# iPERDance/iPERCore

Hardware: AMD Instinct MI355X
Metric: synthesized frames/sec at 512x512 (run_imitator) (higher is better)
Workload: dtype f32; 1 GPU; run_imitator 512x512 single src/ref pair, 300-frame reference clip frame-sharded over 1 GPU(s), AttLWB-SPADE generator fp32 (BASELINE configs[1] at N = 1, configs[2] at N = 8); poses=imitate, image_size=512, frame_batch=300, frame_batch_requested=384, world_size=1, parallelism=frame-shard x1, batches_in_flight=1, weights=random-init (seeded) of the real architecture, 36,276,992 params

## Files before the change

### include/lwg_hip.h

```cpp
#ifndef LWG_HIP_H
#define LWG_HIP_H

#include <stddef.h>
#include <stdint.h>

#ifdef __cplusplus
extern "C" {
#endif

typedef void* lwg_stream_t;

#define LWG_ABI_VERSION 10
int lwg_abi_version(void);

#define LWG_MAX_TAPS 52
enum { LWG_EPI_NONE = 0, LWG_EPI_RESIDUAL = 1, LWG_EPI_SPADE = 2 };
enum { LWG_ACTIVATION_NONE = 0, LWG_ACTIVATION_RELU = 1, LWG_ACTIVATION_TANH = 2, LWG_ACTIVATION_SIGMOID = 3 };
#define LWG_ACTIVATION_RELU_MASK 5
enum { LWG_DT_F32 = 0, LWG_DT_BF16 = 1,
       LWG_DT_F32_Q4 = 2 };

typedef struct LwgConvArgs {
    const float* x0;
    const float* x1;
    int C0, C1;
    int B, H, W;
    int OH, OW;
    int M;
    int stride;
    int ntaps;
    int cshift;
    const float* w;
    int N;
    const float* bias;
    float* y;
    int YH, YW, YC, ycoff;
    int omul, ooy, oox;
    int epi;
    int act;
    const float* res;
    const float* xn;
    const float* mean;
    const float* rstd;
    int xdt;
    int ydt;
    signed char dy[LWG_MAX_TAPS];
    signed char dx[LWG_MAX_TAPS];
} LwgConvArgs;

int lwg_conv2d_nhwc_f32(const LwgConvArgs* args, lwg_stream_t stream);
size_t lwg_conv2d_ws_floats(const LwgConvArgs* args);
int lwg_conv2d_nhwc_f32_ws(const LwgConvArgs* args, float* ws, lwg_stream_t stream);
int lwg_conv_slice_count(const LwgConvArgs* args);

int lwg_conv2d_nhwc_bf16(const LwgConvArgs* args, lwg_stream_t stream);
int lwg_conv2d_winograd_f32(const LwgConvArgs* args, lwg_stream_t stream);
size_t lwg_conv2d_winograd_ws_floats(const LwgConvArgs* args);
int lwg_conv2d_winograd_f32_ws(const LwgConvArgs* args, float* ws, lwg_stream_t stream);
int lwg_conv2d_winograd_plan(const LwgConvArgs* args, int with_ws, long long* blocks, int* slices, int* nbv, int* workgroups);
int lwg_winograd_panel_f32(const float* wpanel, float* upk, int Cin, int N, const int* tap9, lwg_stream_t stream);
typedef struct LwgWinoDesc {
    const float* wpanel;
    float* upk;
    int Cin, N, first_block;
    int tap9[9];
} LwgWinoDesc;
int lwg_winograd_panels_f32(const LwgWinoDesc* descs_dev, int ndesc, int total_blocks, lwg_stream_t stream);
int lwg_conv2d_winograd4_f32(const LwgConvArgs* args, lwg_stream_t stream);
typedef struct LwgConvLists {
    const int* heavy;
    const int* light;
    const int* counts;
    const float* cal;
} LwgConvLists;
int lwg_conv2d_winograd4_list_f32(const LwgConvArgs* args, const LwgConvLists* lists, lwg_stream_t stream);
int lwg_conv2d_winograd4_list_applies(const LwgConvArgs* args);
int lwg_spade_skip_lists_f32(const float* T, int B, int ns, int h, int w, int d, int* marks, int* heavy, int* light, int* counts, lwg_stream_t stream);
int lwg_conv2d_winograd4_fine_f32(const LwgConvArgs* args, const LwgConvLists* lists, lwg_stream_t stream);
int lwg_spade_skip_fine_lists_f32(const float* T, int B, int ns, int h, int w, int d, int* marks, int* heavy, int* light, int* counts, int* fmarks,
                                  int* fheavy, int* flight, int* fcounts, lwg_stream_t stream);
int lwg_winograd4_panel_f32(const float* wpanel, float* upk, int Cin, int N, const int* tap9, lwg_stream_t stream);
int lwg_winograd4_panels_f32(const LwgWinoDesc* descs_dev, int ndesc, int total_blocks, lwg_stream_t stream);
int lwg_conv2d_winograd4_f32_ws(const LwgConvArgs* args, float* ws, lwg_stream_t stream);
int lwg_conv2d_winograd4_plan(const LwgConvArgs* args, int with_ws, long long* blocks, int* slices, int* nbv, int* workgroups);
size_t lwg_conv2d_winograd4_ws_floats(const LwgConvArgs* args);
int lwg_conv2d_nhwc_bf16_hr(const LwgConvArgs* args, lwg_stream_t stream);
int lwg_conv2d_nhwc_bf16_hr_list(const LwgConvArgs* args, const LwgConvLists* lists, lwg_stream_t stream);
int lwg_conv2d_nhwc_bf16_hr_list_applies(const LwgConvArgs* args);
int lwg_conv2d_nhwc_bf16_hr_acc(const LwgConvArgs* args, lwg_stream_t stream);
int lwg_conv2d_winograd_bf16(const LwgConvArgs* args, lwg_stream_t stream);
int lwg_conv2d_nhwc_c8_bf16(const LwgConvArgs* args, lwg_stream_t stream);
int lwg_conv_transpose4_nhwc_bf16(const LwgConvArgs* args, lwg_stream_t stream);
int lwg_conv_transpose4_nhwc_f32(const LwgConvArgs* args, lwg_stream_t stream);
int lwg_conv_transpose4_is_one_grid(const LwgConvArgs* args);
int lwg_conv_transpose4_winograd_f32(const LwgConvArgs* args, lwg_stream_t stream);

int lwg_conv_transpose4_winograd24_f32(const LwgConvArgs* args, lwg_stream_t stream);

int lwg_conv2d_nhwc_f32_split(const LwgConvArgs* args, lwg_stream_t stream);

size_t lwg_conv2d_wgrad_ws_floats(int Ktot, int N, int M);
int lwg_conv2d_wgrad_nhwc_f32(const LwgConvArgs* args, const float* dy, float* dw, float* ws, lwg_stream_t stream);
int lwg_conv2d_wgrad_unpacked_f32(const LwgConvArgs* args, const float* dy, float* ws, float* dw, int D0, int D1, int KH, int KW,
                                  int transposed, const int* kidx, int cin, int nout, float* db, lwg_stream_t stream);
int lwg_colsum_nhwc_f32(const float* x, size_t rows, int C, float* out, float* ws, lwg_stream_t stream);
size_t lwg_conv2d_wgrad_winograd_ws_floats(const LwgConvArgs* args);
int lwg_conv2d_wgrad_winograd_f32(const LwgConvArgs* args, const float* dy, float* ws, float* dw, int cin, int nout, lwg_stream_t stream);

int lwg_act_bwd_f32(const float* dy, const float* y, size_t n, int act, float* out, lwg_stream_t stream);
int lwg_norm_fwd_nhwc_f32(const float* x, const float* mean, const float* rstd, const float* gamma, const float* beta, int gstride,
                          int B, int HW, int C, int act, float* y, lwg_stream_t stream);
int lwg_norm_bwd_nhwc_f32(const float* dy, const float* y, const float* x, const float* mean, const float* rstd,
                          const float* gamma, int gstride, int B, int HW, int C, int act, int nsplit, float* dx, float* dgamma,
                          float* dbeta, float* ws, lwg_stream_t stream);
int lwg_adam_step_f32(float* p, const float* g, float* m, float* v, size_t n, float lr, float beta1, float beta2, float eps, int t,
                      lwg_stream_t stream);
int lwg_adam_step_dev_f32(float* p, const float* g, float* m, float* v, size_t n, float lr, float beta1, float beta2, float eps,
                          int* t_dev, lwg_stream_t stream);
int lwg_pack_panel_f32(const float* w, int D0, int D1, int KH, int KW, int transposed, const int* kidx, int ntaps, int cin,
                       int cin_pad, int nout, int n_pad, float* out, lwg_stream_t stream);
int lwg_unpack_wgrad_f32(const float* dwk, int D0, int D1, int KH, int KW, int transposed, const int* kidx, int ntaps, int cin,
                         int cin_pad, int nout, int n_pad, float* dw, lwg_stream_t stream);
typedef struct LwgPackDesc {
    const float* w;
    float* out;
    int D1, KHW, transposed, ntaps, cin, cin_pad, nout, n_pad, Kp, first_block;
    int kidx[LWG_MAX_TAPS];
} LwgPackDesc;
int lwg_pack_panels_f32(const LwgPackDesc* descs_dev, int ndesc, int total_blocks, lwg_stream_t stream);
int lwg_maxpool2_fwd_nhwc_f32(const float* x, float* y, int B, int H, int W, int C, lwg_stream_t stream);
int lwg_maxpool2_bwd_nhwc_f32(const float* x, const float* dy, float* dx, int B, int H, int W, int C, lwg_stream_t stream);
int lwg_crop_resize_bilinear_f32(const float* x, const long long* box, float* y, float* valid, int N, int C, int H, int W, int OH, int OW,
                                 lwg_stream_t stream);
int lwg_crop_resize_bilinear_bwd_f32(const float* dy, const long long* box, float* dx, int N, int C, int H, int W, int OH, int OW, lwg_stream_t stream);
int lwg_prelu_f32(const float* x, const float* slope, const float* res, size_t rows, int C, float* y, lwg_stream_t stream);
int lwg_prelu_bwd_f32(const float* x, const float* slope, const float* dy, size_t rows, int C, float* dx, lwg_stream_t stream);

int lwg_instnorm_stats_nhwc_f32(const float* x, int B, int HW, int C, float eps, float* mean, float* rstd,
                                float* ws, int nsplit, lwg_stream_t stream);
int lwg_instnorm_stats_nhwc_bf16(const void* x, int B, int HW, int C, float eps, float* mean, float* rstd, float* ws, int nsplit,
                                 lwg_stream_t stream);
int lwg_instnorm_apply_nhwc_f32(const float* x, const float* mean, const float* rstd, const float* res,
                                float* y, int B, int HW, int C, int act, lwg_stream_t stream);

int lwg_flow_resize_f32(const float* T, int n, int S, int h, int w, float* out, lwg_stream_t stream);
int lwg_lwb_attention_f32(const float* q, const float* Ks, const float* Vs, const float* bk, const float* bv,
                          const float* T, float* out, int B, int ns, int h, int w, int C, int S,
                          int src_batched, lwg_stream_t stream);
int lwg_lwb_attention_bf16(const void* q, const void* Ks, const void* Vs, const float* bk, const float* bv, const float* T, void* out,
                           int B, int ns, int h, int w, int C, int S, int src_batched, lwg_stream_t stream);
int lwg_lwb_attention_x_records(int h, int w, int C, int element_size);
int lwg_lwb_attention_x_f32(const float* x, const float* Kq, const float* kappa, const float* Vs, const float* bv, const float* T,
                            float* out, float* stats, int B, int ns, int h, int w, int C, int src_batched, lwg_stream_t stream);
int lwg_lwb_attention_x_bf16(const void* x, const void* Kq, const float* kappa, const void* Vs, const float* bv, const float* T,
                             void* out, float* stats, int B, int ns, int h, int w, int C, int src_batched, lwg_stream_t stream);
size_t lwg_instnorm_finalize_ws_floats(int B, int C, int nrec);
int lwg_instnorm_finalize_f32(float* ws, int B, int C, int nrec, float eps, float* mean, float* rstd, lwg_stream_t stream);
int lwg_lwb_attention_bwd_f32(const float* q, const float* Ks, const float* Vs, const float* bk, const float* bv,
                              const float* T, const float* dout, float* dq, float* dKs, float* dVs, int B, int ns,
                              int h, int w, int C, int S, int src_batched, lwg_stream_t stream);
int lwg_lwb_attention_kv_f32(const float* q, const float* kv, const float* bk, const float* bv, const float* T, float* out,
                             int B, int ns, int h, int w, int C, int S, int src_batched, lwg_stream_t stream);
int lwg_lwb_attention_kv_bwd_f32(const float* q, const float* kv, const float* bk, const float* bv, const float* T,
                                 const float* dout, float* dq, float* dkv, int B, int ns, int h, int w, int C, int S,
                                 int src_batched, lwg_stream_t stream);
int lwg_lwb_fuse_f32(const float* tsf_x, const float* src_x, const float* gate, const float* T, float* out, int B, int ns,
                     int h, int w, int C, int S, int src_batched, float scale_w, float scale_o, lwg_stream_t stream);
int lwg_lwb_fuse_bf16(const void* tsf_x, const void* src_x, const void* gate, const float* T, void* out, int B, int ns, int h, int w,
                      int C, int S, int src_batched, float scale_w, float scale_o, lwg_stream_t stream);
int lwg_lwb_fuse_bwd_f32(const float* src_x, const float* gate, const float* T, const float* dout, float* d_tsf, float* d_src,
                         float* d_gate, int B, int ns, int h, int w, int C, int S, int src_batched, float scale_w, float scale_o,
                         lwg_stream_t stream);

size_t lwg_rasterize_ws_bytes(int B, int nf, int S);
int lwg_project_faces_f32(const float* verts, const float* cam, const int32_t* faces, int B, int nv, int nf,
                          float eye_dist, float* faces_v, float* f2pts, lwg_stream_t stream);
int lwg_rasterize_fim_wim_f32(const float* faces_v, int B, int nf, int S, float near, float far, int32_t* fim,
                              float* wim, void* ws, lwg_stream_t stream);
int lwg_texture_sample_f32(const int32_t* fim, const float* wim, const float* faces_v, const float* textures, int B, int nf,
                           int S, int T, int tex_batched, float eps, const float* bg_color3_host, float* rgb, lwg_stream_t stream);

int lwg_flow_compose_f32(const int32_t* fim, const float* wim, int B, int S, const float* map_fn, int nf,
                         const float* f_uvs2img, const float* uv_img4, int Hu, int Wu, const float* src_f2pts,
                         int ns, float* tsf_inputs, float* Tst, float* cond_nchw, float* Tuv, lwg_stream_t stream);
int lwg_bc_transform_f32(const float* f2pts, const int32_t* fim, const float* wim, int B, int S, int nf, float* T,
                         lwg_stream_t stream);
int lwg_encode_fim_f32(const int32_t* fim, const float* map_fn, int B, int S, int nf, int D, float* out,
                       lwg_stream_t stream);

size_t lwg_smpl_lbs_ws_floats(int B, int nv, int nj);
int lwg_smpl_lbs_f32(const float* pose, int pose_stride, const float* beta, int beta_stride, int nbeta,
                     const float* cam, int cam_stride, const float* v_template, const float* offsets, int off_batched,
                     const float* shapedirs, const float* posedirs, const float* J_regressor, const int32_t* parents,
                     const float* lbs_weights, const int32_t* links, int nlinks, int B, int nv, int nj, float* verts,
                     float* j3d, float* j2d, float* ws, lwg_stream_t stream);

int lwg_head_compose_f32(const float* x, const float* wpk, const float* bg, size_t bg_bstride, int B, int S, int C,
                         float* pred, float* mask, float* img, lwg_stream_t stream);
int lwg_head_compose_q4_f32(const float* x, const float* wpk, const float* bg, size_t bg_bstride, int B, int S, int C,
                            float* pred, float* mask, float* img, lwg_stream_t stream);
int lwg_thin_conv_f32(const float* x, const float* wpk, int B, int S, int C, int ks, float* y, lwg_stream_t stream);
int lwg_head_compose_bf16(const void* x, const void* wb, const float* bg, size_t bg_bstride, int B, int S, int C, float* pred,
                          float* mask, float* img, lwg_stream_t stream);
int lwg_up4_head_compose_bf16(const LwgConvArgs* args, const void* whead, const float* bg, size_t bg_bstride, float* pred, float* mask, float* img,
                              lwg_stream_t stream);
int lwg_frames_to_u8(const float* pred, int B, int S, int bgr, uint8_t* out, lwg_stream_t stream);
int lwg_nchw_to_nhwc_f32(const float* src, float* dst, int B, int C, int Cp, int P, lwg_stream_t stream);
int lwg_nhwc_to_nchw_f32(const float* src, float* dst, int B, int C, int Cs, int P, lwg_stream_t stream);

int lwg_morph_f32(const float* in, float* out, int n, int H, int W, int ks, int mode, float* ws, lwg_stream_t stream);
int lwg_canny_f32(const float* sil, int n, int H, int W, const float* gauss9, const float* sobelx9, float low, float high,
                  float* edges, float* ws, lwg_stream_t stream);
int lwg_boundary_fill_f32(const float* src, const float* confidant, const float* outpad, const float* edges, int n, int H,
                          int W, float* out, int32_t* top3, int32_t* ws, lwg_stream_t stream);
int lwg_grid_sample_nchw_f32(const float* img, size_t img_bstride, const float* grid, int n, int C, int H, int W, int Ho,
                             int Wo, float* out, lwg_stream_t stream);
int lwg_uv_merge_f32(const float* src_warp, const float* vis, int ns, int H, int W, float* out, lwg_stream_t stream);
int lwg_uv_merge_parts_f32(const float* uv_imgs, const float* vis, int n, int H, int W, float* out, lwg_stream_t stream);
int lwg_pack_inputs_f32(const float* a, int Ca, const float* b, int Cb, const float* mask, int n, int H, int W, int Cp,
                        float* out, lwg_stream_t stream);

int lwg_device_cu_count(void);

#ifdef __cplusplus
}
#endif
#endif
```

### ipercore_amd/_lib.py

```python
import ctypes
import os
import re

_HERE = os.path.dirname(os.path.abspath(__file__))
LIB_PATH = os.path.join(_HERE, "liblwg_hip.so")
HEADER_PATH = os.path.join(os.path.dirname(_HERE), "include", "lwg_hip.h")

LWG_MAX_TAPS = 52
EPI_NONE, EPI_RESIDUAL, EPI_SPADE = 0, 1, 2
ACT_NONE, ACT_RELU, ACT_TANH, ACT_SIGMOID, ACT_LRELU = 0, 1, 2, 3, 4
ACT_RELU_MASK = 5
DT_F32, DT_BF16, DT_F32_Q4 = 0, 1, 2

c_f = ctypes.c_void_p
c_i = ctypes.c_int


class LwgConvArgs(ctypes.Structure):
    _fields_ = [
        ("x0", c_f), ("x1", c_f),
        ("C0", c_i), ("C1", c_i),
        ("B", c_i), ("H", c_i), ("W", c_i),
        ("OH", c_i), ("OW", c_i),
        ("M", c_i), ("stride", c_i), ("ntaps", c_i), ("cshift", c_i),
        ("w", c_f), ("N", c_i), ("bias", c_f),
        ("y", c_f), ("YH", c_i), ("YW", c_i), ("YC", c_i), ("ycoff", c_i),
        ("omul", c_i), ("ooy", c_i), ("oox", c_i),
        ("epi", c_i), ("act", c_i),
        ("res", c_f), ("xn", c_f), ("mean", c_f), ("rstd", c_f),
        ("xdt", c_i), ("ydt", c_i),
        ("dy", ctypes.c_byte * LWG_MAX_TAPS), ("dx", ctypes.c_byte * LWG_MAX_TAPS),
    ]


class LwgWinoDesc(ctypes.Structure):
    _fields_ = [("wpanel", ctypes.c_void_p), ("upk", ctypes.c_void_p), ("Cin", c_i), ("N", c_i), ("first_block", c_i), ("tap9", c_i * 9)]


class LwgConvLists(ctypes.Structure):
    _fields_ = [("heavy", c_f), ("light", c_f), ("counts", c_f), ("cal", c_f)]


class LwgPackDesc(ctypes.Structure):
    _fields_ = [("w", c_f), ("out", c_f)] + [(n, c_i) for n in ("D1", "KHW", "transposed", "ntaps", "cin", "cin_pad", "nout", "n_pad", "Kp",
                                                               "first_block")] + [("kidx", c_i * LWG_MAX_TAPS)]


_SIGS = {
    "lwg_abi_version": (c_i, []),
    "lwg_device_cu_count": (c_i, []),
    "lwg_conv2d_nhwc_f32": (c_i, [ctypes.POINTER(LwgConvArgs), c_f]),
    "lwg_conv2d_ws_floats": (ctypes.c_size_t, [ctypes.POINTER(LwgConvArgs)]),
    "lwg_conv2d_nhwc_f32_ws": (c_i, [ctypes.POINTER(LwgConvArgs), c_f, c_f]),
    "lwg_conv2d_nhwc_bf16": (c_i, [ctypes.POINTER(LwgConvArgs), c_f]),
    "lwg_conv2d_winograd_f32": (c_i, [ctypes.POINTER(LwgConvArgs), c_f]),
    "lwg_conv2d_winograd_ws_floats": (ctypes.c_size_t, [ctypes.POINTER(LwgConvArgs)]),
    "lwg_conv2d_winograd_f32_ws": (c_i, [ctypes.POINTER(LwgConvArgs), c_f, c_f]),
    "lwg_conv2d_winograd_plan": (c_i, [ctypes.POINTER(LwgConvArgs), c_i, ctypes.POINTER(ctypes.c_longlong), ctypes.POINTER(c_i), ctypes.POINTER(c_i),
                                       ctypes.POINTER(c_i)]),
    "lwg_winograd_panel_f32": (c_i, [c_f, c_f, c_i, c_i, ctypes.POINTER(c_i), c_f]),
    "lwg_winograd_panels_f32": (c_i, [c_f, c_i, c_i, c_f]),
    "lwg_conv2d_winograd4_f32": (c_i, [ctypes.POINTER(LwgConvArgs), c_f]),
    "lwg_conv2d_winograd4_list_f32": (c_i, [ctypes.POINTER(LwgConvArgs), ctypes.POINTER(LwgConvLists), c_f]),
    "lwg_conv2d_winograd4_list_applies": (c_i, [ctypes.POINTER(LwgConvArgs)]),
    "lwg_spade_skip_lists_f32": (c_i, [c_f, c_i, c_i, c_i, c_i, c_i, c_f, c_f, c_f, c_f, c_f]),
    "lwg_conv2d_winograd4_fine_f32": (c_i, [ctypes.POINTER(LwgConvArgs), ctypes.POINTER(LwgConvLists), c_f]),
    "lwg_spade_skip_fine_lists_f32": (c_i, [c_f, c_i, c_i, c_i, c_i, c_i, c_f, c_f, c_f, c_f, c_f, c_f, c_f, c_f, c_f]),
    "lwg_winograd4_panel_f32": (c_i, [c_f, c_f, c_i, c_i, ctypes.POINTER(c_i), c_f]),
    "lwg_winograd4_panels_f32": (c_i, [c_f, c_i, c_i, c_f]),
    "lwg_conv2d_winograd4_f32_ws": (c_i, [ctypes.POINTER(LwgConvArgs), c_f, c_f]),
    "lwg_conv2d_winograd4_plan": (c_i, [ctypes.POINTER(LwgConvArgs), c_i, ctypes.POINTER(ctypes.c_longlong), ctypes.POINTER(c_i), ctypes.POINTER(c_i),
                                        ctypes.POINTER(c_i)]),
    "lwg_conv2d_winograd4_ws_floats": (ctypes.c_size_t, [ctypes.POINTER(LwgConvArgs)]),
    "lwg_conv2d_nhwc_bf16_hr": (c_i, [ctypes.POINTER(LwgConvArgs), c_f]),
    "lwg_conv2d_nhwc_bf16_hr_list": (c_i, [ctypes.POINTER(LwgConvArgs), ctypes.POINTER(LwgConvLists), c_f]),
    "lwg_conv2d_nhwc_bf16_hr_list_applies": (c_i, [ctypes.POINTER(LwgConvArgs)]),
    "lwg_conv2d_nhwc_bf16_hr_acc": (c_i, [ctypes.POINTER(LwgConvArgs), c_f]),
    "lwg_conv2d_winograd_bf16": (c_i, [ctypes.POINTER(LwgConvArgs), c_f]),
    "lwg_conv2d_nhwc_c8_bf16": (c_i, [ctypes.POINTER(LwgConvArgs), c_f]),
    "lwg_conv_transpose4_nhwc_bf16": (c_i, [ctypes.POINTER(LwgConvArgs), c_f]),
    "lwg_conv_transpose4_nhwc_f32": (c_i, [ctypes.POINTER(LwgConvArgs), c_f]),
    "lwg_conv_transpose4_winograd_f32": (c_i, [ctypes.POINTER(LwgConvArgs), c_f]),
    "lwg_conv_transpose4_winograd24_f32": (c_i, [ctypes.POINTER(LwgConvArgs), c_f]),
    "lwg_conv_transpose4_is_one_grid": (c_i, [ctypes.POINTER(LwgConvArgs)]),
    "lwg_conv_slice_count": (c_i, [ctypes.POINTER(LwgConvArgs)]),
    "lwg_conv2d_nhwc_f32_split": (c_i, [ctypes.POINTER(LwgConvArgs), c_f]),
    "lwg_conv2d_wgrad_ws_floats": (ctypes.c_size_t, [c_i, c_i, c_i]),
    "lwg_conv2d_wgrad_nhwc_f32": (c_i, [ctypes.POINTER(LwgConvArgs), c_f, c_f, c_f, c_f]),
    "lwg_conv2d_wgrad_unpacked_f32": (c_i, [ctypes.POINTER(LwgConvArgs), c_f, c_f, c_f] + [c_i] * 5 + [ctypes.POINTER(ctypes.c_int), c_i, c_i, c_f, c_f]),
    "lwg_colsum_nhwc_f32": (c_i, [c_f, ctypes.c_size_t, c_i, c_f, c_f, c_f]),
    "lwg_conv2d_wgrad_winograd_ws_floats": (ctypes.c_size_t, [ctypes.POINTER(LwgConvArgs)]),
    "lwg_conv2d_wgrad_winograd_f32": (c_i, [ctypes.POINTER(LwgConvArgs), c_f, c_f, c_f, c_i, c_i, c_f]),
    "lwg_act_bwd_f32": (c_i, [c_f, c_f, ctypes.c_size_t, c_i, c_f, c_f]),
    "lwg_norm_fwd_nhwc_f32": (c_i, [c_f, c_f, c_f, c_f, c_f, c_i, c_i, c_i, c_i, c_i, c_f, c_f]),
    "lwg_norm_bwd_nhwc_f32": (c_i, [c_f, c_f, c_f, c_f, c_f, c_f, c_i, c_i, c_i, c_i, c_i, c_i, c_f, c_f, c_f, c_f, c_f]),
    "lwg_adam_step_f32": (c_i, [c_f, c_f, c_f, c_f, ctypes.c_size_t, ctypes.c_float, ctypes.c_float, ctypes.c_float, ctypes.c_float, c_i, c_f]),
    "lwg_adam_step_dev_f32": (c_i, [c_f, c_f, c_f, c_f, ctypes.c_size_t, ctypes.c_float, ctypes.c_float, ctypes.c_float, ctypes.c_float, c_f, c_f]),
    "lwg_pack_panel_f32": (c_i, [c_f] + [c_i] * 5 + [ctypes.POINTER(ctypes.c_int)] + [c_i] * 5 + [c_f, c_f]),
    "lwg_pack_panels_f32": (c_i, [c_f, c_i, c_i, c_f]),
    "lwg_unpack_wgrad_f32": (c_i, [c_f] + [c_i] * 5 + [ctypes.POINTER(ctypes.c_int)] + [c_i] * 5 + [c_f, c_f]),
    "lwg_maxpool2_fwd_nhwc_f32": (c_i, [c_f, c_f, c_i, c_i, c_i, c_i, c_f]),
    "lwg_maxpool2_bwd_nhwc_f32": (c_i, [c_f, c_f, c_f, c_i, c_i, c_i, c_i, c_f]),
    "lwg_crop_resize_bilinear_f32": (c_i, [c_f, c_f, c_f, c_f, c_i, c_i, c_i, c_i, c_i, c_i, c_f]),
    "lwg_crop_resize_bilinear_bwd_f32": (c_i, [c_f, c_f, c_f, c_i, c_i, c_i, c_i, c_i, c_i, c_f]),
    "lwg_prelu_f32": (c_i, [c_f, c_f, c_f, ctypes.c_size_t, c_i, c_f, c_f]),
    "lwg_prelu_bwd_f32": (c_i, [c_f, c_f, c_f, ctypes.c_size_t, c_i, c_f, c_f]),
    "lwg_instnorm_stats_nhwc_f32": (c_i, [c_f, c_i, c_i, c_i, ctypes.c_float, c_f, c_f, c_f, c_i, c_f]),
    "lwg_instnorm_apply_nhwc_f32": (c_i, [c_f, c_f, c_f, c_f, c_f, c_i, c_i, c_i, c_i, c_f]),
    "lwg_lwb_attention_f32": (c_i, [c_f, c_f, c_f, c_f, c_f, c_f, c_f, c_i, c_i, c_i, c_i, c_i, c_i, c_i, c_f]),
    "lwg_lwb_attention_bf16": (c_i, [c_f, c_f, c_f, c_f, c_f, c_f, c_f, c_i, c_i, c_i, c_i, c_i, c_i, c_i, c_f]),
    "lwg_instnorm_stats_nhwc_bf16": (c_i, [c_f, c_i, c_i, c_i, ctypes.c_float, c_f, c_f, c_f, c_i, c_f]),
    "lwg_head_compose_bf16": (c_i, [c_f, c_f, c_f, ctypes.c_size_t, c_i, c_i, c_i, c_f, c_f, c_f, c_f]),
    "lwg_up4_head_compose_bf16": (c_i, [ctypes.POINTER(LwgConvArgs), c_f, c_f, ctypes.c_size_t, c_f, c_f, c_f, c_f]),
    "lwg_flow_resize_f32": (c_i, [c_f, c_i, c_i, c_i, c_i, c_f, c_f]),
    "lwg_lwb_fuse_f32": (c_i, [c_f] * 5 + [c_i] * 7 + [ctypes.c_float, ctypes.c_float, c_f]),
    "lwg_lwb_fuse_bf16": (c_i, [c_f] * 5 + [c_i] * 7 + [ctypes.c_float, ctypes.c_float, c_f]),
    "lwg_lwb_fuse_bwd_f32": (c_i, [c_f] * 7 + [c_i] * 7 + [ctypes.c_float, ctypes.c_float, c_f]),
    "lwg_lwb_attention_x_f32": (c_i, [c_f] * 8 + [c_i] * 6 + [c_f]),
    "lwg_lwb_attention_x_bf16": (c_i, [c_f] * 8 + [c_i] * 6 + [c_f]),
    "lwg_lwb_attention_x_records": (c_i, [c_i, c_i, c_i, c_i]),
    "lwg_instnorm_finalize_ws_floats": (ctypes.c_size_t, [c_i, c_i, c_i]),
    "lwg_instnorm_finalize_f32": (c_i, [c_f, c_i, c_i, c_i, ctypes.c_float, c_f, c_f, c_f]),
    "lwg_lwb_attention_bwd_f32": (c_i, [c_f] * 10 + [c_i] * 7 + [c_f]),
    "lwg_lwb_attention_kv_f32": (c_i, [c_f] * 6 + [c_i] * 7 + [c_f]),
    "lwg_lwb_attention_kv_bwd_f32": (c_i, [c_f] * 8 + [c_i] * 7 + [c_f]),
    "lwg_rasterize_ws_bytes": (ctypes.c_size_t, [c_i, c_i, c_i]),
    "lwg_project_faces_f32": (c_i, [c_f, c_f, c_f, c_i, c_i, c_i, ctypes.c_float, c_f, c_f, c_f]),
    "lwg_rasterize_fim_wim_f32": (c_i, [c_f, c_i, c_i, c_i, ctypes.c_float, ctypes.c_float, c_f, c_f, c_f, c_f]),
    "lwg_texture_sample_f32": (c_i, [c_f, c_f, c_f, c_f, c_i, c_i, c_i, c_i, c_i, ctypes.c_float, ctypes.POINTER(ctypes.c_float), c_f, c_f]),
    "lwg_flow_compose_f32": (c_i, [c_f, c_f, c_i, c_i, c_f, c_i, c_f, c_f, c_i, c_i, c_f, c_i, c_f, c_f, c_f, c_f, c_f]),
    "lwg_bc_transform_f32": (c_i, [c_f, c_f, c_f, c_i, c_i, c_i, c_f, c_f]),
    "lwg_encode_fim_f32": (c_i, [c_f, c_f, c_i, c_i, c_i, c_i, c_f, c_f]),
    "lwg_smpl_lbs_ws_floats": (ctypes.c_size_t, [c_i, c_i, c_i]),
    "lwg_smpl_lbs_f32": (c_i, [c_f, c_i, c_f, c_i, c_i, c_f, c_i, c_f, c_f, c_i, c_f, c_f, c_f, c_f, c_f, c_f, c_i, c_i, c_i,
                               c_i, c_f, c_f, c_f, c_f, c_f]),
    "lwg_head_compose_f32": (c_i, [c_f, c_f, c_f, ctypes.c_size_t, c_i, c_i, c_i, c_f, c_f, c_f, c_f]),
    "lwg_head_compose_q4_f32": (c_i, [c_f, c_f, c_f, ctypes.c_size_t, c_i, c_i, c_i, c_f, c_f, c_f, c_f]),
    "lwg_thin_conv_f32": (c_i, [c_f, c_f, c_i, c_i, c_i, c_i, c_f, c_f]),
    "lwg_nchw_to_nhwc_f32": (c_i, [c_f, c_f, c_i, c_i, c_i, c_i, c_f]),
    "lwg_nhwc_to_nchw_f32": (c_i, [c_f, c_f, c_i, c_i, c_i, c_i, c_f]),
    "lwg_frames_to_u8": (c_i, [c_f, c_i, c_i, c_i, c_f, c_f]),
    "lwg_morph_f32": (c_i, [c_f, c_f, c_i, c_i, c_i, c_i, c_i, c_f, c_f]),
    "lwg_canny_f32": (c_i, [c_f, c_i, c_i, c_i, ctypes.POINTER(ctypes.c_float), ctypes.POINTER(ctypes.c_float),
                            ctypes.c_float, ctypes.c_float, c_f, c_f, c_f]),
    "lwg_boundary_fill_f32": (c_i, [c_f, c_f, c_f, c_f, c_i, c_i, c_i, c_f, c_f, c_f, c_f]),
    "lwg_grid_sample_nchw_f32": (c_i, [c_f, ctypes.c_size_t, c_f, c_i, c_i, c_i, c_i, c_i, c_i, c_f, c_f]),
    "lwg_uv_merge_f32": (c_i, [c_f, c_f, c_i, c_i, c_i, c_f, c_f]),
    "lwg_uv_merge_parts_f32": (c_i, [c_f, c_f, c_i, c_i, c_i, c_f, c_f]),
    "lwg_pack_inputs_f32": (c_i, [c_f, c_i, c_f, c_i, c_f, c_i, c_i, c_i, c_i, c_f, c_f]),
}

_lib = None


def header_symbols():
    with open(HEADER_PATH) as fp:
        src = re.sub(r"/\*.*?\*/", "", fp.read(), flags=re.S)
    return sorted(set(re.findall(r"\b(lwg_[a-z0-9_]+)\s*\(", src)))


def lib():
    global _lib
    if _lib is None:
        if not os.path.exists(LIB_PATH):
            raise RuntimeError(
                f"{LIB_PATH} not found: the HIP kernels are not built (run `python -c 'import __graft_entry__ as g; "
                "g.build()'` or `make -C ipercore_amd/csrc`).  There is no CPU fallback.")
        import torch
        handle = ctypes.CDLL(LIB_PATH)
        for name, (res, args) in _SIGS.items():
            fn = getattr(handle, name)
            fn.restype = res
            fn.argtypes = args
        if handle.lwg_abi_version() != 10:
            raise RuntimeError("liblwg_hip.so ABI version mismatch")
        _lib = handle
    return _lib


def check(err, what):
    if err != 0:
        raise RuntimeError(f"{what} failed with hipError_t {err}")
```

### ipercore_amd/csrc/conv_winograd4.hip

```cpp
#include <hip/hip_runtime.h>
#include "lwg_common.h"
#include "lwg_conv_wino.h"

#define W4_THREADS 512
#define W4_PBX 8
#define W4_PBY 4
#define W4_NB 64
#define W4_KS 8
#define W4_HW 34
#define W4_HH 18
#ifndef W4_RS
#define W4_RS 40
#endif
#define W4_PLANE (18 * W4_RS + 4)
#define W4_RAW (W4_KS * W4_PLANE)
#define W4_VS (36 * W4_KS * 32)
#define W4_NEL (W4_HW * W4_HH * 2)
#define W4_NQ 3
#define W4_DUMP_OFF (2 * W4_RAW + 2 * W4_VS)
#define W4_DUMP (W4_THREADS + 3 * W4_PLANE)
#define W4_LOOP (W4_DUMP_OFF + W4_DUMP)
#define W4_MSR 68
#define W4_NPL 28
#define W4_MS (W4_NPL * 16 * W4_MSR)
#define W4_BIAS_OFF (W4_LOOP > W4_MS ? W4_LOOP : W4_MS)
#define W4F_SLOT(s) (((s) / CW4F_NSX) * CW4F_HH * W4_RS + ((s) % CW4F_NSX) * (W4_RS / CW4F_NSX))
#define W4F_PLANE (CW4F_NS / CW4F_NSX * CW4F_HH * W4_RS + 4)
static_assert(W4_RS / CW4F_NSX >= CW4F_HW && (W4_RS / CW4F_NSX) % 4 == 0 && W4F_PLANE >= W4_PLANE, "two sub-tile halo rows per LDS row");
#define W4F_LOOP (2 * W4_KS * W4F_PLANE + 2 * W4_VS + W4_THREADS + 3 * W4F_PLANE)
#define W4F_BIAS_OFF (W4F_LOOP > W4_MS ? W4F_LOOP : W4_MS)
static_assert(CW4F_SX == 16 && CW4F_SY == 8 && CW4F_NS * CW4F_ROUNDS * 64 == W4_NQ * W4_THREADS, "sub-tile halo: four slots x six wave rounds = the staged elements");
#ifndef LWG_W4_XCD
#define LWG_W4_XCD 1
#endif
#ifndef LWG_W4_CHUNK
#define LWG_W4_CHUNK 1
#endif
#ifndef LWG_W4_RDMAP
#define LWG_W4_RDMAP 1
#endif
#ifndef LWG_W4_SMALL
#define LWG_W4_SMALL 1
#endif
#define W4SB() __builtin_amdgcn_sched_barrier(0)

#ifdef LWG_W4_TS
#define W4TS(i) do { if (tid == 0 && lab_bi == 1) reinterpret_cast<unsigned long long*>(const_cast<float*>(a.res))[(size_t)blockIdx.x * 16 + (i)] = __builtin_readcyclecounter(); } while (0)
#define W4TSA(i) do { if (tid == 0) reinterpret_cast<unsigned long long*>(const_cast<float*>(a.res))[(size_t)blockIdx.x * 16 + (i)] = __builtin_readcyclecounter(); } while (0)
#else
#define W4TS(i) do { } while (0)
#define W4TSA(i) do { } while (0)
#endif

#ifndef W4_NT
#define W4_NT 0
#endif
#ifndef W4_NT_LD
#define W4_NT_LD W4_NT
#endif
#ifndef W4_NT_RES
#define W4_NT_RES 0
#endif
#ifndef W4_NT_ST
#define W4_NT_ST 2
#endif

__device__ __forceinline__ void w4_bt6(const float (&r)[6], float (&v)[6]) {
    const float a = __builtin_fmaf(-4.f, r[2], r[4]), b = __builtin_fmaf(-4.f, r[1], r[3]);
    const float c = r[4] - r[2], e = r[3] - r[1];
    v[0] = __builtin_fmaf(-5.f, r[2], __builtin_fmaf(4.f, r[0], r[4]));
    v[1] = a + b;
    v[2] = a - b;
    v[3] = __builtin_fmaf(2.f, e, c);
    v[4] = __builtin_fmaf(-2.f, e, c);
    v[5] = __builtin_fmaf(-5.f, r[3], __builtin_fmaf(4.f, r[1], r[5]));
}

__device__ __forceinline__ float w4_spade_mod(float x, float mu, float rs, float gam, float bet) { return (x - mu) * rs * (1.f + gam) + bet; }
template <int NR>
__device__ __forceinline__ void w4_act16(int act, floatx4 (&o)[NR]) {
    lwg_act_dispatch(act, [&](auto ACTC) {
        constexpr int EA = decltype(ACTC)::value;
#pragma unroll
        for (int i = 0; i < NR; ++i)
#pragma unroll
            for (int c = 0; c < 4; ++c) o[i][c] = lwg_act_c<EA>(o[i][c], act);
    });
}

template <int EPI, bool TWO, bool SM, bool LIST, bool FINE = false, bool SPLIT = false>
__device__ __forceinline__ void w4_body(const LwgConvArgs& a, const LwgConvLists& sk) {
    static_assert(!FINE || (LIST && !SM && !TWO && LWG_W4_RDMAP), "the sub-tile form: a list-driven 8-wave launch");
    static_assert(!SPLIT || (SM && !LIST && EPI == LWG_EPI_NONE), "the split form: 4-wave blocks, plain epilogue");
    constexpr int RS = W4_RS;
    constexpr int PLANE = FINE ? W4F_PLANE : W4_PLANE;
    constexpr int RAW = W4_KS * PLANE;
    constexpr int DUMP_OFF = 2 * RAW + 2 * W4_VS;
    constexpr int BIAS_OFF = FINE ? W4F_BIAS_OFF : W4_BIAS_OFF;
    constexpr bool SMS = SM && EPI == LWG_EPI_SPADE;
    constexpr int NVP = SM && !SMS ? 2 : 1;
    constexpr int NTH = SM ? 256 : W4_THREADS;
    constexpr int NQ = SM ? 5 : W4_NQ;
    constexpr int NBV = SM ? 32 : W4_NB;
    constexpr int MSR = SM ? 36 : W4_MSR;
    constexpr int NHF = SM ? 2 : 1;
    extern __shared__ __attribute__((aligned(16))) float smem[];
    const int wid = __builtin_amdgcn_readfirstlane(threadIdx.x >> 6);
    const float* __restrict__ bias = a.bias;
    const int H = a.H, W = a.W, Cin = a.C0 + a.C1, N = a.N;
    float* __restrict__ y = SPLIT ? a.y + cw4_slab_offset((int)blockIdx.z, a.M, N) : a.y;
    float* const raw0 = smem;
    float* const Ms = smem;
    const int tid = threadIdx.x, lane = tid & 63;
    const CwGrid g = cw_grid(a.B, H, W, N, 4 * W4_PBX, 4 * W4_PBY, NBV);
    const CwOrder o = cw_order(cw4_order_kind(LWG_W4_XCD, LWG_W4_CHUNK, SM, gridDim.x, N / NBV, Cin, N, g.tiles, g.total), gridDim.x, blockIdx.x, N / NBV, g);
    int blk = blockIdx.x;
    const int nall = FINE ? cw4f_in_image_total(a.B, H, W) : g.tiles;
    const int nht = LIST ? min(max(__builtin_amdgcn_readfirstlane(sk.counts[0]), 0), nall) : 0;
    const int nhe = (FINE ? cw4f_groups(nht) : nht) * (N / NBV);
    const bool lst = FINE ? true : LIST ? nht < nall : false;
    const bool run = lst ? blk < nhe : true;
    const int nst = Cin / W4_KS;
    const int sbeg = SPLIT ? cw4_slice_begin((int)blockIdx.z, a.cshift) : 0;
    const int send = SPLIT ? cw4_slice_end((int)blockIdx.z, a.cshift, nst) : nst;
    const __amdgpu_buffer_rsrc_t ru = __builtin_amdgcn_make_buffer_rsrc(const_cast<float*>(a.w), 0, (int)(144u * (unsigned)Cin * (unsigned)N), 0x00020000);
    const int q = wid & 3, ct = SM ? 0 : wid >> 2;
    const int half = SM ? 0 : wid >> 2;
    floatx16 acc[9];
    CwBlock<NQ, TWO> bk;
    unsigned uvoff, uvoffc;
    int fs0 = 0, fs1 = 0;
    auto setup = [&](int id) {
        int cb, t;
        if constexpr (FINE) {
            int tids = tid;
            asm volatile("" : "+v"(tids));
            int fsub[CW4F_NS], slot;
            cw_list_entry(id, N / NBV, slot, cb);
#pragma unroll
            for (int k = 0; k < CW4F_NS; ++k) {
                const int ix = cw4f_slot_index(slot, k, nht);
                fsub[k] = ix < 0 ? -1 : min(max(__builtin_amdgcn_readfirstlane(sk.heavy[ix]), 0), CW4F_NS * g.tiles - 1);
            }
            bk.n0 = cw_n0(cb, NBV);
            const int hs = wid >> 1, u = hs == 0 ? fsub[0] : hs == 1 ? fsub[1] : hs == 2 ? fsub[2] : fsub[3];
            int b, x0, y0;
            cw4f_corner(g, max(u, 0), b, x0, y0);
            bk.rx0 = cw_image_rsrc(a.x0, __builtin_amdgcn_readfirstlane(b), H, W, a.C0, 4u);
#pragma unroll
            for (int k = 0; k < NQ; ++k) {
                int s, j;
                cw4f_halo_elem(tids + NTH * k, s, j);
                bk.voff0[k] = cw4f_halo_voff(u >= 0, j, x0, y0, H, W, a.C0);
            }
            fs0 = (wid >> 2) ? fsub[1] : fsub[0], fs1 = (wid >> 2) ? fsub[CW4F_NSX + 1] : fsub[CW4F_NSX];
        } else if constexpr (LIST) {
            if (lst) {
                int slot;
                cw_list_entry(id, N / NBV, slot, cb);
                t = min(max(__builtin_amdgcn_readfirstlane(sk.heavy[slot]), 0), g.tiles - 1);
            } else {
                cw_block(o, id, cb, t);
            }
        } else {
            cw_block(o, id, cb, t);
        }
        if constexpr (!FINE) {
        bk.locate(a, g, t, 4 * W4_PBX, 4 * W4_PBY, SMS ? cw4_n0_spade_small(cb) : cw_n0(cb, NBV));
        int tids = tid;
        asm volatile("" : "+v"(tids));
        bk.halo(a, tids, NTH, W4_HW, W4_NEL);
        }
        const int col = SMS ? bk.n0 + (((lane & 31) >> 4) << 5) + (lane & 15) : bk.n0 + ct * 32 + (lane & 31);
        uvoff = (unsigned)(((lane >> 5) * 9 * N + 4 * col) * 4);
        uvoffc = (unsigned)(((lane >> 5) * 9 * N + 8 * N + col) * 4);
    };
    if (run) setup(blk);
    int wst[NQ];
#pragma unroll
    for (int k = 0; k < NQ; ++k) {
        const int i = tid + NTH * k;
        if constexpr (FINE) {
            int s, j, hy, hx, hq;
            cw4f_halo_elem(i, s, j);
            cw4f_halo_place(j, hy, hx, hq);
            wst[k] = j < CW4F_NEL ? 4 * hq * PLANE + W4F_SLOT(s) + hy * RS + hx : DUMP_OFF + tid;
        } else {
        const int pix = i >> 1, hq = i & 1, hy = pix / W4_HW, hx = pix - hy * W4_HW;
        wst[k] = i < W4_NEL ? 4 * hq * PLANE + hy * RS + hx : DUMP_OFF + tid;
        }
    }
    floatx4 rreg[NQ];
    auto rld1 = [&](int st, int k) -> floatx4 {
#ifdef W4_LAB_HFIX
        const int c = 0 * st;
#else
        const int c = st * W4_KS;
#endif
        return bk.template rld1<W4_NT_LD>(a, c, k);
    };
    auto rst1 = [&](int buf, int k, floatx4 v) { cw_rst1(raw0 + buf * RAW + wst[k], PLANE, v); };
    floatx4 ufa[4], ufb[4];
    float ufc[4];
    const unsigned ukk = (unsigned)N * 72u;
    const unsigned uq = (unsigned)q * (unsigned)nst * 4u * ukk;
    const unsigned ubo = (unsigned)N * 16u;
    auto uldpart = [&](int set, int st, int kk, int part) {
#ifdef W4_LAB_UFIX
        const unsigned so = uq + 0u * (unsigned)(st + kk);
#else
        const unsigned so = uq + (unsigned)(st * 4 + kk) * ukk;
#endif
        if (part == 0) ufa[set] = cw_buf_load(ru, uvoff, so);
        else if (part == 1) ufb[set] = cw_buf_load(ru, uvoff, so + ubo);
        else ufc[set] = __builtin_bit_cast(float, __builtin_amdgcn_raw_buffer_load_b32(ru, (int)uvoffc, (int)so, 0));
    };
    auto uldset = [&](int set, int st, int kk) {
#ifdef W4_LAB_UFIX
        const unsigned so = uq + 0u * (unsigned)(st + kk);
#else
        const unsigned so = uq + (unsigned)(st * 4 + kk) * ukk;
#endif
        ufa[set] = cw_buf_load(ru, uvoff, so);
        ufb[set] = cw_buf_load(ru, uvoff, so + ubo);
        ufc[set] = __builtin_bit_cast(float, __builtin_amdgcn_raw_buffer_load_b32(ru, (int)uvoffc, (int)so, 0));
    };
    const int patch = tid & 31, tc = (tid >> 5) & 7;
    const int pty = patch >> 3, ptx = patch & 7;
    int pby = pty, pbx = ptx, pslot = 0;
    if constexpr (FINE) {
        cw4f_patch_in_slot(pty, ptx, pby, pbx);
        pslot = W4F_SLOT(cw4f_slot_of_patch(pty, ptx));
    }
    unsigned dbs = (unsigned)(tc * PLANE + pslot + (4 * pby) * RS + 4 * pbx) >> 2;
    asm volatile("" : "+v"(dbs));
    dbs <<= 2;
    unsigned dbx[NHF], vbx[NHF], vbt[NHF];
    float alpha[NHF], beta[NHF], nbeta[NHF];
#pragma unroll
    for (int hi = 0; hi < NHF; ++hi) {
        const int hf = SM ? hi : half;
        dbx[hi] = (unsigned)(tc * PLANE + pslot + (4 * pby + hf) * RS + 4 * pbx) >> 2;
        asm volatile("" : "+v"(dbx[hi]));
        dbx[hi] <<= 2;
        vbx[hi] = (unsigned)(2 * RAW + (hf ? 30 : 0) * W4_KS * 32 + tc * 32 + patch);
        vbt[hi] = (unsigned)(2 * RAW + (hf ? 18 : 6) * W4_KS * 32 + tc * 32 + patch);
        asm volatile("" : "+v"(vbx[hi]));
        asm volatile("" : "+v"(vbt[hi]));
        alpha[hi] = hf ? -1.f : -4.f;
        beta[hi] = hf ? 2.f : 1.f;
        nbeta[hi] = -beta[hi];
    }
    unsigned fbs[2];
    fbs[0] = (unsigned)(2 * RAW + (6 * q) * W4_KS * 32 + lane);
    fbs[1] = (unsigned)(2 * RAW + (6 * (4 + (q >> 1)) + 3 * (q & 1)) * W4_KS * 32 + lane);
    asm volatile("" : "+v"(fbs[0]));
    asm volatile("" : "+v"(fbs[1]));
    float fb[9];
    auto frag1 = [&](int buf, int kk, int j) -> float {
        return smem[fbs[j < 6 ? 0 : 1] + buf * W4_VS + ((j < 6 ? j : j - 6) * W4_KS + 2 * kk) * 32];
    };
    auto rd6 = [&](unsigned base, int buf, int r, float (&d)[6]) {
        const floatx4 v4 = *reinterpret_cast<const floatx4*>(smem + base + buf * RAW + r * RS);
        const float2 v2 = *reinterpret_cast<const float2*>(smem + base + buf * RAW + r * RS + 4);
        d[0] = v4[0]; d[1] = v4[1]; d[2] = v4[2]; d[3] = v4[3]; d[4] = v2.x; d[5] = v2.y;
    };
    auto vst6 = [&](unsigned base, int buf, int i, const float (&v)[6]) {
        float* dst = smem + base + buf * W4_VS + (6 * i) * W4_KS * 32;
#pragma unroll
        for (int nu = 0; nu < 6; ++nu) dst[nu * W4_KS * 32] = v[nu];
    };
    auto transform_full = [&](int buf) {
#pragma unroll
        for (int hi = 0; hi < NHF; ++hi) {
            float X[6], P[6], Q[6], v[6];
            {
                float dR[3][6];
                rd6(dbx[hi], buf, 0, dR[0]); rd6(dbx[hi], buf, 2, dR[1]); rd6(dbx[hi], buf, 4, dR[2]);
#pragma unroll
                for (int j = 0; j < 6; ++j) X[j] = __builtin_fmaf(-5.f, dR[1][j], __builtin_fmaf(4.f, dR[0][j], dR[2][j]));
            }
            {
                float dR[2][6];
                rd6(dbs, buf, 2, dR[0]); rd6(dbs, buf, 4, dR[1]);
#pragma unroll
                for (int j = 0; j < 6; ++j) P[j] = __builtin_fmaf(alpha[hi], dR[0][j], dR[1][j]);
                rd6(dbs, buf, 1, dR[0]); rd6(dbs, buf, 3, dR[1]);
#pragma unroll
                for (int j = 0; j < 6; ++j) Q[j] = __builtin_fmaf(alpha[hi], dR[0][j], dR[1][j]);
            }
            w4_bt6(X, v); vst6(vbx[hi], buf, 0, v);
            float T[6];
#pragma unroll
            for (int j = 0; j < 6; ++j) T[j] = __builtin_fmaf(beta[hi], Q[j], P[j]);
            w4_bt6(T, v); vst6(vbt[hi], buf, 0, v);
#pragma unroll
            for (int j = 0; j < 6; ++j) T[j] = __builtin_fmaf(nbeta[hi], Q[j], P[j]);
            w4_bt6(T, v); vst6(vbt[hi], buf, 1, v);
        }
    };
    auto iteration = [&](int s, auto SET, auto NXT) {
        constexpr int set = decltype(SET)::value;
        constexpr bool nxt = decltype(NXT)::value != 0;
        const int s3 = s + 3 < send ? s + 3 : send - 1;
        float X[6], P[6], Q[6], dR[3][6];
        auto mf = [&](int kk, int j, bool refill) {
            acc[j] = __builtin_amdgcn_mfma_f32_32x32x2f32(j < 4 ? ufa[kk][j & 3] : j < 8 ? ufb[kk][j & 3] : ufc[kk], fb[j], acc[j], 0, 0, 0);
#ifndef W4_KO_FRAG
            if (refill && (j & 1)) {
                fb[j - 1] = kk < 3 ? frag1(set, kk + 1, j - 1) : frag1(set ^ 1, 0, j - 1);
                fb[j] = kk < 3 ? frag1(set, kk + 1, j) : frag1(set ^ 1, 0, j);
            } else if (refill && j == 8) {
                fb[8] = kk < 3 ? frag1(set, kk + 1, 8) : frag1(set ^ 1, 0, 8);
            }
#endif
            W4SB();
        };
        auto ul = [&](int kk, int part) {
#ifndef W4_KO_ULD
            if (kk < 2) uldpart(kk + 2, s, kk + 2, part);
            else if (nxt) uldpart(kk - 2, s + 1, kk - 2, part);
#endif
            W4SB();
        };
        auto halo = [&](int k) {
#ifdef W4_KO_HALO
            return;
#endif
            if (nxt) { rst1(set, k, rreg[k]); rreg[k] = rld1(s3, k); }
            W4SB();
        };
#ifdef W4_KO_TR
        constexpr bool trn = false;
#else
        constexpr bool trn = nxt;
#endif
        auto tr = [&](int hi, int step) {
            if (trn) {
                if (step < 3) rd6(dbx[hi], set ^ 1, 2 * step, dR[step]);
                else if (step < 5) {
#pragma unroll
                    for (int j = 3 * (step - 3); j < 3 * (step - 3) + 3; ++j) X[j] = __builtin_fmaf(-5.f, dR[1][j], __builtin_fmaf(4.f, dR[0][j], dR[2][j]));
                } else if (step < 7) rd6(dbs, set ^ 1, 2 * (step - 5) + 2, dR[step - 5]);
                else if (step == 7) {
                    float v[6];
                    w4_bt6(X, v);
                    vst6(vbx[hi], set ^ 1, 0, v);
                } else if (step == 8) {
#pragma unroll
                    for (int j = 0; j < 6; ++j) P[j] = __builtin_fmaf(alpha[hi], dR[0][j], dR[1][j]);
                } else if (step < 11) rd6(dbs, set ^ 1, 2 * (step - 9) + 1, dR[step - 9]);
                else if (step == 11) {
#pragma unroll
                    for (int j = 0; j < 6; ++j) Q[j] = __builtin_fmaf(alpha[hi], dR[0][j], dR[1][j]);
                } else {
                    float T[6], v[6];
#pragma unroll
                    for (int j = 0; j < 6; ++j) T[j] = __builtin_fmaf(step == 12 ? beta[hi] : nbeta[hi], Q[j], P[j]);
                    w4_bt6(T, v);
                    vst6(vbt[hi], set ^ 1, step - 12, v);
                }
            }
            W4SB();
        };
        if constexpr (!SM) {
            mf(0, 0, true); ul(0, 0);
            mf(0, 1, true); halo(0);
            mf(0, 2, true); ul(0, 1); tr(0, 0);
            mf(0, 3, true); halo(1); tr(0, 1);
            mf(0, 4, true); ul(0, 2); tr(0, 2);
            mf(0, 5, true); halo(2);
            mf(0, 6, true); tr(0, 3);
            mf(0, 7, true); tr(0, 4);
            mf(0, 8, true); tr(0, 5);
            mf(1, 0, true); ul(1, 0); tr(0, 6);
            mf(1, 1, true); tr(0, 7);
            mf(1, 2, true); ul(1, 1); tr(0, 8); tr(0, 9);
            mf(1, 3, true); tr(0, 10);
            mf(1, 4, true); ul(1, 2);
            mf(1, 5, true); tr(0, 11);
            mf(1, 6, true); tr(0, 12);
            mf(1, 7, true);
            mf(1, 8, true); tr(0, 13);
            mf(2, 0, true); ul(2, 0);
            mf(2, 1, true);
            mf(2, 2, true); ul(2, 1);
            mf(2, 3, true);
            mf(2, 4, true); ul(2, 2);
            mf(2, 5, true); mf(2, 6, true); mf(2, 7, true); mf(2, 8, true);
        } else {
            mf(0, 0, true); ul(0, 0); halo(0);
            mf(0, 1, true); tr(0, 0);
            mf(0, 2, true); ul(0, 1); tr(0, 1);
            mf(0, 3, true); halo(1); tr(0, 2);
            mf(0, 4, true); ul(0, 2); tr(0, 3);
            mf(0, 5, true); halo(2); tr(0, 4);
            mf(0, 6, true); tr(0, 5);
            mf(0, 7, true); halo(3); tr(0, 6);
            mf(0, 8, true); tr(0, 7);
            mf(1, 0, true); ul(1, 0); tr(0, 8); tr(0, 9);
            mf(1, 1, true); halo(4); tr(0, 10);
            mf(1, 2, true); ul(1, 1); tr(0, 11);
            mf(1, 3, true); tr(0, 12);
            mf(1, 4, true); ul(1, 2); tr(0, 13);
            mf(1, 5, true); tr(1, 0);
            mf(1, 6, true); tr(1, 1);
            mf(1, 7, true); tr(1, 2);
            mf(1, 8, true); tr(1, 3);
            mf(2, 0, true); ul(2, 0); tr(1, 4);
            mf(2, 1, true); tr(1, 5);
            mf(2, 2, true); ul(2, 1); tr(1, 6);
            mf(2, 3, true); tr(1, 7);
            mf(2, 4, true); ul(2, 2); tr(1, 8); tr(1, 9);
            mf(2, 5, true); tr(1, 10);
            mf(2, 6, true); tr(1, 11);
            mf(2, 7, true); tr(1, 12);
            mf(2, 8, true); tr(1, 13);
        }
        __syncthreads();
        W4SB();
        mf(3, 0, nxt); ul(3, 0);
        mf(3, 1, nxt);
        mf(3, 2, nxt); ul(3, 1);
        mf(3, 3, nxt);
        mf(3, 4, nxt); ul(3, 2);
        mf(3, 5, nxt); mf(3, 6, nxt); mf(3, 7, nxt); mf(3, 8, nxt);
    };

    floatx4 r0[NQ], r1[NQ];
    float bq;
    auto issue_loads = [&]() {
        bq = bias ? bias[SMS ? bk.n0 + (((tid & 31) >> 4) << 5) + (tid & 15) : bk.n0 + (tid & (NBV - 1))] : 0.f;
#pragma unroll
        for (int k = 0; k < NQ; ++k) {
            r0[k] = rld1(sbeg, k);
            r1[k] = rld1(sbeg + 1, k);
        }
        uldset(0, sbeg, 0);
        uldset(1, sbeg, 1);
#pragma unroll
        for (int k = 0; k < NQ; ++k) rreg[k] = rld1(send - sbeg > 2 ? sbeg + 2 : sbeg + 1, k);
    };
    if (run) issue_loads();
#ifdef LWG_W4_TS
    int lab_bi = 0;
#endif
    W4TSA(11);
    if (run) for (;;) {
    W4TS(0);
#pragma unroll
    for (int k = 0; k < NQ; ++k) {
        rst1(0, k, r0[k]);
        rst1(1, k, r1[k]);
    }
    if (tid < NBV) smem[BIAS_OFF + tid] = bq;
    __syncthreads();
    transform_full(0);
    __syncthreads();
#pragma unroll
    for (int j = 0; j < 9; ++j) fb[j] = frag1(0, 0, j);
#pragma unroll
    for (int j = 0; j < 9; ++j)
#pragma unroll
        for (int r = 0; r < 16; ++r) acc[j][r] = 0.f;
    if (q == 1) {
#pragma unroll
        for (int g = 0; g < 4; ++g) {
            const floatx4 b4 = *reinterpret_cast<const floatx4*>(smem + BIAS_OFF + ct * 32 + 8 * g + 4 * (lane >> 5));
#pragma unroll
            for (int k = 0; k < 4; ++k) acc[1][4 * g + k] = b4[k];
        }
    }
    W4TS(1);
    {
        int s = sbeg;
        for (; s + 2 < send; s += 2) {
            iteration(s, IntC<0>(), IntC<1>());
            iteration(s + 1, IntC<1>(), IntC<1>());
        }
        iteration(s, IntC<0>(), IntC<1>());
        iteration(s + 1, IntC<1>(), IntC<0>());
    }
    W4TS(2);
    int eb = FINE ? 0 : bk.b, ex0 = FINE ? 0 : bk.x0, ey0 = FINE ? 0 : bk.y0;
    const int en0 = bk.n0;
    const int es0 = fs0, es1 = fs1;
#pragma unroll
    for (int r = 0; r < 16; ++r) {
        const float m0 = acc[0][r], m1 = acc[1][r], m2 = acc[2][r], m3 = acc[3][r], m4 = acc[4][r], m5 = acc[5][r];
        const float s12 = m1 + m2, d12 = m1 - m2, s34 = m3 + m4, d34 = m3 - m4;
        acc[0][r] = (m0 + s12) + s34;
        acc[1][r] = __builtin_fmaf(2.f, d34, d12);
        acc[2][r] = __builtin_fmaf(4.f, s34, s12);
        acc[3][r] = __builtin_fmaf(8.f, d34, d12) + m5;
    }
    if (q & 1) {
#pragma unroll
        for (int r = 0; r < 16; ++r) {
            const float h0 = acc[6][r], h1 = acc[7][r];
            acc[6][r] = h0 + h1;
            acc[7][r] = h0 - h1;
        }
    } else {
#pragma unroll
        for (int r = 0; r < 16; ++r) {
            const float h0 = acc[6][r], h1 = acc[7][r], h2 = acc[8][r];
            acc[6][r] = (h0 + h1) + h2;
            acc[7][r] = h1 - h2;
            acc[8][r] = h1 + h2;
        }
    }
    W4TS(4);
    int tide = tid;
    asm volatile("" : "+v"(tide));
    const int lanee = tide & 63;
    const int rb = wid & 3;
    const unsigned l5 = (unsigned)lanee & 31u, gsel = (0x0FF0F00Fu >> l5) & 1u;
    const int gidx = __builtin_popcount((gsel ? 0x0FF0F00Fu : 0xF00F0FF0u) & ((1u << l5) - 1u));
    const int p16 = LWG_W4_RDMAP && !SM ? (wid >> 2) * 4 + 2 * (lanee >> 5) + (gsel ? 0 : 1) + 8 * (gidx >> 3) : (wid >> 2) * 8 + (lanee >> 3);
    const int n4 = SMS ? (lanee & 3) * 4 : LWG_W4_RDMAP && !SM ? (gidx & 7) * 4 : (lanee & 7) * 4;
    const int cbase = SMS ? (en0 >> 6) * 32 + ((en0 >> 4) & 1) * 16 : en0 >> 1;
    floatx4 mu, rs;
    typedef unsigned int w4_u4 __attribute__((ext_vector_type(4)));
    const unsigned img_bytes = (unsigned)(H * W) * (unsigned)a.YC * 4u;
    const float* const esrc = EPI == LWG_EPI_SPADE ? a.xn : EPI == LWG_EPI_RESIDUAL ? a.res : a.y;
    __amdgpu_buffer_rsrc_t ry, re;
    auto eframe = [&]() {
        if (EPI == LWG_EPI_SPADE) {
            mu = *reinterpret_cast<const floatx4*>(a.mean + (size_t)eb * a.YC + cbase + n4);
            rs = *reinterpret_cast<const floatx4*>(a.rstd + (size_t)eb * a.YC + cbase + n4);
        }
        ry = __builtin_amdgcn_make_buffer_rsrc(y + (size_t)eb * H * W * a.YC, 0, (int)img_bytes, 0x00020000);
        re = __builtin_amdgcn_make_buffer_rsrc(const_cast<float*>(esrc) + (size_t)eb * H * W * a.YC, 0, (int)img_bytes, 0x00020000);
    };
    if constexpr (!FINE) eframe();
    const int chan = EPI == LWG_EPI_SPADE ? cbase + n4 : a.ycoff + en0 + n4;
    bool more = false;
    int nblk = blk;
#pragma unroll
    for (int ph = 0; ph < 2; ++ph) {
        if (ph == 1) __syncthreads();
        if constexpr (FINE) {
            const int u = ph ? es1 : es0;
            int ub;
            cw4f_corner(g, max(u, 0), ub, ex0, ey0);
            eb = __builtin_amdgcn_readfirstlane(ub);
            if (u < 0) ex0 = W, ey0 = H;
            eframe();
        }
        if (((lanee >> 4) & 1) == ph) {
            float* dst = Ms + (lanee & 15) * MSR + ct * 32 + 4 * (lanee >> 5);
#pragma unroll
            for (int g = 0; g < 4; ++g) {
#pragma unroll
                for (int bb = 0; bb < 4; ++bb)
                    *reinterpret_cast<floatx4*>(dst + (4 * q + bb) * 16 * MSR + 8 * g) = floatx4{acc[bb][4 * g], acc[bb][4 * g + 1], acc[bb][4 * g + 2], acc[bb][4 * g + 3]};
#pragma unroll
                for (int i = 0; i < 3; ++i)
                    *reinterpret_cast<floatx4*>(dst + (16 + 3 * q + i) * 16 * MSR + 8 * g) = floatx4{acc[6 + i][4 * g], acc[6 + i][4 * g + 1], acc[6 + i][4 * g + 2], acc[6 + i][4 * g + 3]};
            }
        }
        unsigned vo[NVP][4];
#pragma unroll
        for (int hp = 0; hp < NVP; ++hp) {
            const int p = ph * 16 + (SMS ? lanee >> 2 : SM ? 8 * hp + (lanee >> 3) : p16);
            const int ox = ex0 + 4 * (FINE ? (p & 7) % (CW4F_SX / 4) : (p & 7)) + rb, oyb = ey0 + 4 * (FINE ? (p >> 3) % (CW4F_SY / 4) : (p >> 3));
#pragma unroll
            for (int i = 0; i < 4; ++i)
                vo[hp][i] = cw4_out_voff(ox, oyb + i, H, W, a.YC, chan);
        }
        floatx4 ext[2][4];
        if (EPI != LWG_EPI_NONE) {
#pragma unroll
            for (int h = 0; h < (EPI == LWG_EPI_SPADE ? 1 : 2); ++h)
#pragma unroll
                for (int i = 0; i < 4; ++i) ext[h][i] = __builtin_bit_cast(floatx4, __builtin_amdgcn_raw_buffer_load_b128(re, (int)cw4_out_group(vo[NVP == 2 ? h : 0][i], h, !SM), 0, W4_NT_RES));
        }
        if (ph == 1) {
            W4TS(8);
            if constexpr (!SPLIT) {
            nblk = blk + (int)gridDim.x;
            if constexpr (FINE) more = nblk < nhe;
            else if constexpr (LIST) more = lst ? nblk < nhe : cw_has_block(o, nblk);
            else more = cw_has_block(o, nblk);
            setup(more ? nblk : blk);
            W4TS(9);
            issue_loads();
            W4TS(10);
            }
        }
        __syncthreads();
        if (ph == 0) W4TS(5); else W4TS(7);
        floatx4 gam[4];
#pragma unroll
        for (int h = 0; h < 2; ++h) {
            const float* base = Ms + (SMS ? lanee >> 2 : SM ? 8 * h + (lanee >> 3) : p16) * MSR + (SMS ? h * 16 : SM ? 0 : h * 32) + n4;
            floatx4 F[6];
#pragma unroll
            for (int xi = 0; xi < 4; ++xi) F[xi] = *reinterpret_cast<const floatx4*>(base + (4 * xi + rb) * 16 * MSR);
            const int ia = rb == 0 ? 0 : rb == 2 ? 2 : 1, ib = (rb & 1) ? 4 : 3;
            const float cb = (float)(1 << rb);
#pragma unroll
            for (int r = 0; r < 2; ++r) {
                const float* hb = base + (16 + 6 * r) * 16 * MSR;
                const floatx4 pa = *reinterpret_cast<const floatx4*>(hb + ia * 16 * MSR);
                const floatx4 pb = *reinterpret_cast<const floatx4*>(hb + ib * 16 * MSR);
                floatx4 f;
#pragma unroll
                for (int c = 0; c < 4; ++c) f[c] = __builtin_fmaf(cb, pb[c], pa[c]);
                if (rb == 3) f += *reinterpret_cast<const floatx4*>(hb + 5 * 16 * MSR);
                F[4 + r] = f;
            }
            floatx4 o[4];
#pragma unroll
            for (int c = 0; c < 4; ++c) {
                const float s12 = F[1][c] + F[2][c], d12 = F[1][c] - F[2][c], s34 = F[3][c] + F[4][c], d34 = F[3][c] - F[4][c];
                o[0][c] = (F[0][c] + s12) + s34;
                o[1][c] = __builtin_fmaf(2.f, d34, d12);
                o[2][c] = __builtin_fmaf(4.f, s34, s12);
                o[3][c] = __builtin_fmaf(8.f, d34, d12) + F[5][c];
            }
            if (EPI == LWG_EPI_SPADE) {
                if (h == 0) {
#pragma unroll
                    for (int i = 0; i < 4; ++i) gam[i] = o[i];
                    continue;
                }
#pragma unroll
                for (int i = 0; i < 4; ++i)
#pragma unroll
                    for (int c = 0; c < 4; ++c) o[i][c] = w4_spade_mod(ext[0][i][c], mu[c], rs[c], gam[i][c], o[i][c]);
            } else if (EPI == LWG_EPI_RESIDUAL) {
                if (a.act == LWG_ACT_RELU_MASK) {
#pragma unroll
                    for (int i = 0; i < 4; ++i)
#pragma unroll
                        for (int c = 0; c < 4; ++c) o[i][c] = ext[h][i][c] > 0.f ? o[i][c] : 0.f;
                } else {
#pragma unroll
                    for (int i = 0; i < 4; ++i) o[i] += ext[h][i];
                }
            }
            w4_act16(a.act, o);
#pragma unroll
            for (int i = 0; i < 4; ++i)
                __builtin_amdgcn_raw_buffer_store_b128(__builtin_bit_cast(w4_u4, o[i]), ry, (int)cw4_out_group(vo[NVP == 2 ? h : 0][i], h, EPI != LWG_EPI_SPADE && !SM), 0, W4_NT_ST);
        }
        if (ph == 0) W4TS(6);
    }
    W4TS(3);
#ifdef LWG_W4_TS
    ++lab_bi;
#endif
    if (!more) break;
    blk = nblk;
    __syncthreads();
    }
    W4TSA(12);
#ifdef LWG_W4_TS
    if (tid == 0) reinterpret_cast<unsigned long long*>(const_cast<float*>(a.res))[(size_t)blockIdx.x * 16 + 13] = (unsigned long long)lab_bi;
#endif
    if constexpr (LIST) {
        typedef unsigned int w4_u4 __attribute__((ext_vector_type(4)));
        constexpr int NQD = EPI == LWG_EPI_SPADE ? 8 : 16;
        constexpr int NPASS = (FINE ? CW4F_SX * CW4F_SY : 512) * NQD / W4_THREADS, NI = NPASS < 4 ? NPASS : 4;
        const int ncb = N / NBV;
        const int nend = nhe + min(max(__builtin_amdgcn_readfirstlane(sk.counts[1]), 0), nall - nht) * ncb;
        const unsigned img_bytes = (unsigned)(H * W) * (unsigned)a.YC * 4u;
        const __amdgpu_buffer_rsrc_t rc = __builtin_amdgcn_make_buffer_rsrc(const_cast<float*>(sk.cal), 0, (int)((unsigned)(H * W) * (unsigned)(EPI == LWG_EPI_SPADE ? N : a.YC) * 4u), 0x00020000);
#pragma unroll 1
        for (int id = cw_list_first_light((int)blockIdx.x, (int)gridDim.x, nhe); id < nend; id += (int)gridDim.x) {
            int slot, cb;
            cw_list_entry(id - nhe, ncb, slot, cb);
            const int t = min(max(__builtin_amdgcn_readfirstlane(sk.light[slot]), 0), (FINE ? CW4F_NS : 1) * g.tiles - 1);
            const int en0 = cw_n0(cb, NBV);
            int eb, ex0, ey0;
            if constexpr (FINE) {
                cw4f_corner(g, t, eb, ex0, ey0);
                eb = __builtin_amdgcn_readfirstlane(eb);
            } else {
                eb = __builtin_amdgcn_readfirstlane(cw_image(g, t));
                cw_corner(g, t - eb * g.bx * g.by, 4 * W4_PBX, 4 * W4_PBY, ex0, ey0);
            }
            const __amdgpu_buffer_rsrc_t ry = __builtin_amdgcn_make_buffer_rsrc(y + (size_t)eb * H * W * a.YC, 0, (int)img_bytes, 0x00020000);
            int px, py, q4;
            cw4_light_elem(tid, 0, W4_THREADS, NQD, px, py, q4);
            if constexpr (EPI == LWG_EPI_SPADE) {
                const __amdgpu_buffer_rsrc_t re = __builtin_amdgcn_make_buffer_rsrc(const_cast<float*>(a.xn) + (size_t)eb * H * W * a.YC, 0, (int)img_bytes, 0x00020000);
                const int cbase = en0 >> 1;
                const floatx4 mu = *reinterpret_cast<const floatx4*>(a.mean + (size_t)eb * a.YC + cbase + 4 * q4);
                const floatx4 rs = *reinterpret_cast<const floatx4*>(a.rstd + (size_t)eb * a.YC + cbase + 4 * q4);
#pragma unroll 1
                for (int it = 0; it < NPASS; it += NI) {
                    unsigned vo[NI];
                    floatx4 o[NI], gam[NI], xv[NI];
#pragma unroll
                    for (int i = 0; i < NI; ++i) {
                        cw4_light_elem(tid, it + i, W4_THREADS, NQD, px, py, q4);
                        if constexpr (FINE) cw4f_light_pixel(px, py);
                        vo[i] = cw4_out_voff(ex0 + px, ey0 + py, H, W, a.YC, cbase + 4 * q4);
                        const unsigned vc = cw4_out_voff(ex0 + px, ey0 + py, H, W, N, en0 + 4 * q4);
                        gam[i] = cw_buf_load(rc, cw4_out_group(vc, 0, true), 0u);
                        o[i] = cw_buf_load(rc, cw4_out_group(vc, 1, true), 0u);
                        xv[i] = cw_buf_load<W4_NT_RES>(re, vo[i], 0u);
                    }
#pragma unroll
                    for (int i = 0; i < NI; ++i)
#pragma unroll
                        for (int c = 0; c < 4; ++c) o[i][c] = w4_spade_mod(xv[i][c], mu[c], rs[c], gam[i][c], o[i][c]);
                    w4_act16(a.act, o);
#pragma unroll
                    for (int i = 0; i < NI; ++i) __builtin_amdgcn_raw_buffer_store_b128(__builtin_bit_cast(w4_u4, o[i]), ry, (int)vo[i], 0, W4_NT_ST);
                }
            } else {
#pragma unroll 1
                for (int it = 0; it < NPASS; it += NI) {
                    unsigned vo[NI];
                    floatx4 o[NI];
#pragma unroll
                    for (int i = 0; i < NI; ++i) {
                        cw4_light_elem(tid, it + i, W4_THREADS, NQD, px, py, q4);
                        if constexpr (FINE) cw4f_light_pixel(px, py);
                        vo[i] = cw4_out_voff(ex0 + px, ey0 + py, H, W, a.YC, a.ycoff + en0 + 4 * q4);
                        o[i] = cw_buf_load(rc, vo[i], 0u);
                    }
#pragma unroll
                    for (int i = 0; i < NI; ++i) __builtin_amdgcn_raw_buffer_store_b128(__builtin_bit_cast(w4_u4, o[i]), ry, (int)vo[i], 0, W4_NT_ST);
                }
            }
        }
    }
}

template <int EPI, bool TWO, bool SM = false>
__global__ __launch_bounds__(SM ? 256 : W4_THREADS, 1) void lwg_conv_winograd4_kernel(const LwgConvArgs a) {
    w4_body<EPI, TWO, SM, false>(a, LwgConvLists{});
}
template <bool TWO>
__global__ __launch_bounds__(256, 1) void lwg_conv_winograd4_split_kernel(const LwgConvArgs a) {
    w4_body<LWG_EPI_NONE, TWO, true, false, false, true>(a, LwgConvLists{});
}
template <int EPI>
__global__ __launch_bounds__(W4_THREADS, 1) void lwg_conv_winograd4_list_kernel(const LwgConvArgs a, const LwgConvLists sk) {
    w4_body<EPI, false, false, true>(a, sk);
}
template <int EPI>
__global__ __launch_bounds__(W4_THREADS, 1) void lwg_conv_winograd4_fine_kernel(const LwgConvArgs a, const LwgConvLists sk) {
    if (__builtin_amdgcn_readfirstlane(sk.counts[0]) >= cw4f_in_image_total(a.B, a.H, a.W)) return;
    w4_body<EPI, false, false, true, true>(a, sk);
}
template <int EPI>
__global__ __launch_bounds__(W4_THREADS, 1) void lwg_conv_winograd4_fine_plain_kernel(const LwgConvArgs a, const LwgConvLists sk) {
    if (__builtin_amdgcn_readfirstlane(sk.counts[0]) < cw4f_in_image_total(a.B, a.H, a.W)) return;
    w4_body<EPI, false, false, false>(a, LwgConvLists{});
}


__global__ __launch_bounds__(256) void lwg_winograd4_panel_kernel(const float* __restrict__ wp, float* __restrict__ U, int Cin, int N, LwgWinoTaps taps) {
    const int n = blockIdx.x * 64 + (threadIdx.x & 63), c = blockIdx.y * 4 + (threadIdx.x >> 6);
    if (n >= N || c >= Cin) return;
    double g[3][3];
#pragma unroll
    for (int r = 0; r < 3; ++r)
#pragma unroll
        for (int s = 0; s < 3; ++s) {
            const int k = ((c >> 5) * 9 + taps.t[3 * r + s]) * 32 + (c & 31);
            g[r][s] = (double)wp[((size_t)(k >> 2) * N + n) * 4 + (k & 3)];
        }
    const double G[6][3] = {{1.0 / 4, 0, 0}, {-1.0 / 6, -1.0 / 6, -1.0 / 6}, {-1.0 / 6, 1.0 / 6, -1.0 / 6}, {1.0 / 24, 1.0 / 12, 1.0 / 6}, {1.0 / 24, -1.0 / 12, 1.0 / 6}, {0, 0, 1}};
    double t[6][3];
#pragma unroll
    for (int i = 0; i < 6; ++i)
#pragma unroll
        for (int s = 0; s < 3; ++s) t[i][s] = G[i][0] * g[0][s] + G[i][1] * g[1][s] + G[i][2] * g[2][s];
    const int s8 = c >> 3, kk = (c & 7) >> 1, kh = c & 1;
#pragma unroll
    for (int qq = 0; qq < 4; ++qq) {
        float* dst = U + ((((size_t)qq * (Cin >> 3) + s8) * 4 + kk) * 2 + kh) * 9 * (size_t)N;
        float o[9];
#pragma unroll
        for (int j = 0; j < 9; ++j) {
            const int xi = j < 6 ? qq : 4 + (qq >> 1), nu = j < 6 ? j : 3 * (qq & 1) + (j - 6);
            o[j] = (float)(t[xi][0] * G[nu][0] + t[xi][1] * G[nu][1] + t[xi][2] * G[nu][2]);
        }
        *reinterpret_cast<floatx4*>(dst + 4 * n) = floatx4{o[0], o[1], o[2], o[3]};
        *reinterpret_cast<floatx4*>(dst + 4 * (size_t)N + 4 * n) = floatx4{o[4], o[5], o[6], o[7]};
        dst[8 * (size_t)N + n] = o[8];
    }
}

__device__ __forceinline__ double w4_panel_sum3(double a0, double b0, double a1, double b1, double a2, double b2) {
#pragma clang fp contract(off)
    const double p = a0 * b0;
    return __builtin_fma(a2, b2, __builtin_fma(a1, b1, p));
}
__device__ __forceinline__ void lwg_winograd4_panels_pair(const float* __restrict__ wp, float* __restrict__ U, int Cin, int N, const int* t9, int c, int n) {
    double g[3][3];
#pragma unroll
    for (int r = 0; r < 3; ++r)
#pragma unroll
        for (int s = 0; s < 3; ++s) {
            const int k = ((c >> 5) * 9 + t9[3 * r + s]) * 32 + (c & 31);
            g[r][s] = (double)wp[((size_t)(k >> 2) * N + n) * 4 + (k & 3)];
        }
    const double G[6][3] = {{1.0 / 4, 0, 0}, {-1.0 / 6, -1.0 / 6, -1.0 / 6}, {-1.0 / 6, 1.0 / 6, -1.0 / 6}, {1.0 / 24, 1.0 / 12, 1.0 / 6}, {1.0 / 24, -1.0 / 12, 1.0 / 6}, {0, 0, 1}};
    double t[6][3];
#pragma unroll
    for (int i = 0; i < 6; ++i)
#pragma unroll
        for (int s = 0; s < 3; ++s) t[i][s] = w4_panel_sum3(G[i][0], g[0][s], G[i][1], g[1][s], G[i][2], g[2][s]);
    const int s8 = c >> 3, kk = (c & 7) >> 1, kh = c & 1;
#pragma unroll
    for (int qq = 0; qq < 4; ++qq) {
        float* dst = U + ((((size_t)qq * (Cin >> 3) + s8) * 4 + kk) * 2 + kh) * 9 * (size_t)N;
        float o[9];
#pragma unroll
        for (int j = 0; j < 9; ++j) {
            const int xi = j < 6 ? qq : 4 + (qq >> 1), nu = j < 6 ? j : 3 * (qq & 1) + (j - 6);
            o[j] = (float)w4_panel_sum3(t[xi][0], G[nu][0], t[xi][1], G[nu][1], t[xi][2], G[nu][2]);
        }
        *reinterpret_cast<floatx4*>(dst + 4 * n) = floatx4{o[0], o[1], o[2], o[3]};
        *reinterpret_cast<floatx4*>(dst + 4 * (size_t)N + 4 * n) = floatx4{o[4], o[5], o[6], o[7]};
        dst[8 * (size_t)N + n] = o[8];
    }
}
__global__ __launch_bounds__(256) void lwg_winograd4_panels_kernel(const LwgWinoDesc* __restrict__ descs, int ndesc) {
    int lo = 0, hi = ndesc - 1;
    while (lo < hi) {
        const int mid = (lo + hi + 1) >> 1;
        if (descs[mid].first_block <= (int)blockIdx.x) lo = mid; else hi = mid - 1;
    }
    const LwgWinoDesc* d = descs + lo;
    const int N = d->N, Cin = d->Cin, nbx = (N + 63) >> 6;
    const int lb = (int)blockIdx.x - d->first_block;
    const int n = (lb % nbx) * 64 + (threadIdx.x & 63), c = (lb / nbx) * 4 + (threadIdx.x >> 6);
    if (n < N && c < Cin) lwg_winograd4_panels_pair(d->wpanel, d->upk, Cin, N, d->tap9, c, n);
}

extern "C" int lwg_winograd4_panels_f32(const LwgWinoDesc* descs_dev, int ndesc, int total_blocks, lwg_stream_t stream_) {
    if (!descs_dev || ndesc < 1 || total_blocks < 1) return (int)hipErrorInvalidValue;
    hipLaunchKernelGGL(lwg_winograd4_panels_kernel, dim3((unsigned)total_blocks), dim3(256), 0, reinterpret_cast<hipStream_t>(stream_), descs_dev, ndesc);
    return (int)hipGetLastError();
}

extern "C" int lwg_winograd4_panel_f32(const float* wpanel, float* upk, int Cin, int N, const int* tap9, lwg_stream_t stream_) {
    LwgWinoTaps taps;
    if (!cw_panel_args_ok(wpanel, upk, Cin, N, tap9, taps)) return (int)hipErrorInvalidValue;
    hipLaunchKernelGGL(lwg_winograd4_panel_kernel, dim3((unsigned)((N + 63) / 64), (unsigned)((Cin + 3) / 4)), dim3(256), 0,
                       reinterpret_cast<hipStream_t>(stream_), wpanel, upk, Cin, N, taps);
    return (int)hipGetLastError();
}

template <int EPI, bool SM>
static int lwg_wino4_go(const LwgConvArgs& a, dim3 grid, size_t lds, hipStream_t stream) {
    return a.C1 > 0 ? cw_launch<lwg_conv_winograd4_kernel<EPI, true, SM>>(grid, SM ? 256 : W4_THREADS, lds, stream, a)
                    : cw_launch<lwg_conv_winograd4_kernel<EPI, false, SM>>(grid, SM ? 256 : W4_THREADS, lds, stream, a);
}

extern "C" int lwg_conv2d_winograd4_f32(const LwgConvArgs* pa, lwg_stream_t stream_) {
    hipStream_t stream = reinterpret_cast<hipStream_t>(stream_);
    if (!pa || !cw_contract_ok(*pa, 144ull, 256ll)) return (int)hipErrorInvalidValue;
    const LwgConvArgs& a = *pa;
    const size_t lds = (size_t)(W4_BIAS_OFF + 64) * 4;
    const int cus = lwg_device_cus();
    long long total = cw_total_blocks(a.B, a.H, a.W, a.N, 4 * W4_PBX, 4 * W4_PBY, W4_NB);
    const bool sm = LWG_W4_SMALL && 2 * total <= cus;
    if (sm) total *= 2;
    const dim3 grid = cw_persistent_grid(total, cus);
    if (a.epi == LWG_EPI_SPADE) return sm ? lwg_wino4_go<LWG_EPI_SPADE, true>(a, grid, lds, stream) : lwg_wino4_go<LWG_EPI_SPADE, false>(a, grid, lds, stream);
    if (a.epi == LWG_EPI_RESIDUAL) return sm ? lwg_wino4_go<LWG_EPI_RESIDUAL, true>(a, grid, lds, stream) : lwg_wino4_go<LWG_EPI_RESIDUAL, false>(a, grid, lds, stream);
    return sm ? lwg_wino4_go<LWG_EPI_NONE, true>(a, grid, lds, stream) : lwg_wino4_go<LWG_EPI_NONE, false>(a, grid, lds, stream);
}

static Cw4Split lwg_wino4_split_plan(const LwgConvArgs& a) {
    const bool mask = a.epi == LWG_EPI_RESIDUAL && a.act == LWG_ACT_RELU_MASK;
    return cw4_split_plan(cw_total_blocks(a.B, a.H, a.W, a.N, 4 * W4_PBX, 4 * W4_PBY, 32), (a.C0 + a.C1) / W4_KS, lwg_device_cus(),
                          LWG_W4_SMALL && (a.epi == LWG_EPI_NONE || mask), cw4_slab_image_ok(a.H, a.W, a.N));
}
extern "C" size_t lwg_conv2d_winograd4_ws_floats(const LwgConvArgs* pa) {
    if (!pa || !cw_contract_ok(*pa, 144ull, 256ll)) return 0;
    return cw4_slab_offset(lwg_wino4_split_plan(*pa).slices, pa->M, pa->N);
}
extern "C" int lwg_conv2d_winograd4_plan(const LwgConvArgs* pa, int with_ws, long long* blocks, int* slices, int* nbv, int* workgroups) {
    if (!pa || !cw_contract_ok(*pa, 144ull, 256ll)) return (int)hipErrorInvalidValue;
    const LwgConvArgs& a = *pa;
    const int sl = with_ws ? lwg_wino4_split_plan(a).slices : 0;
    const int cus = lwg_device_cus();
    const long long b64 = cw_total_blocks(a.B, a.H, a.W, a.N, 4 * W4_PBX, 4 * W4_PBY, W4_NB);
    const int v = sl > 1 || (LWG_W4_SMALL && 2 * b64 <= cus) ? 32 : W4_NB;
    const long long nb = b64 * (W4_NB / v) * (sl > 1 ? sl : 1);
    if (blocks) *blocks = nb;
    if (slices) *slices = sl > 1 ? sl : 0;
    if (nbv) *nbv = v;
    if (workgroups) *workgroups = (int)(sl > 1 ? nb : (nb < cus ? nb : cus));
    return 0;
}
extern "C" int lwg_conv2d_winograd4_f32_ws(const LwgConvArgs* pa, float* ws, lwg_stream_t stream_) {
    if (!pa || !cw_contract_ok(*pa, 144ull, 256ll)) return (int)hipErrorInvalidValue;
    const LwgConvArgs& a = *pa;
    const Cw4Split sp = ws ? lwg_wino4_split_plan(a) : Cw4Split{0, 0};
    if (sp.slices < 2) return lwg_conv2d_winograd4_f32(pa, stream_);
    hipStream_t stream = reinterpret_cast<hipStream_t>(stream_);
    LwgConvArgs part = a;
    part.y = ws;
    part.YC = a.N;
    part.ycoff = 0;
    part.bias = nullptr;
    part.epi = LWG_EPI_NONE;
    part.act = LWG_ACT_NONE;
    part.res = nullptr;
    part.cshift = sp.sps;
    const size_t lds = (size_t)(W4_BIAS_OFF + 64) * 4;
    const dim3 grid((unsigned)cw_total_blocks(a.B, a.H, a.W, a.N, 4 * W4_PBX, 4 * W4_PBY, 32), 1u, (unsigned)sp.slices);
    const int e = a.C1 > 0 ? cw_launch<lwg_conv_winograd4_split_kernel<true>>(grid, 256, lds, stream, part)
                           : cw_launch<lwg_conv_winograd4_split_kernel<false>>(grid, 256, lds, stream, part);
    return e != (int)hipSuccess ? e : (int)lwg_splitk_finish_launch(a, ws, sp.slices, stream);
}

static bool lwg_wino4_list_ok(const LwgConvArgs* pa) {
    return pa && cw_contract_ok(*pa, 144ull, 256ll) && pa->C1 == 0 && (pa->epi == LWG_EPI_NONE || pa->epi == LWG_EPI_SPADE) &&
           cw_contract_calib_ok(*pa) && cw_total_blocks(pa->B, pa->H, pa->W, pa->N, 4 * W4_PBX, 4 * W4_PBY, W4_NB) < (1ll << 30);
}
extern "C" int lwg_conv2d_winograd4_list_applies(const LwgConvArgs* pa) {
    if (!lwg_wino4_list_ok(pa)) return 0;
    return !(LWG_W4_SMALL && 2 * cw_total_blocks(pa->B, pa->H, pa->W, pa->N, 4 * W4_PBX, 4 * W4_PBY, W4_NB) <= lwg_device_cus());
}
extern "C" int lwg_conv2d_winograd4_list_f32(const LwgConvArgs* pa, const LwgConvLists* pl, lwg_stream_t stream_) {
    if (!lwg_wino4_list_ok(pa) || !pl || !pl->heavy || !pl->light || !pl->counts || !pl->cal) return (int)hipErrorInvalidValue;
    if (!lwg_conv2d_winograd4_list_applies(pa)) return lwg_conv2d_winograd4_f32(pa, stream_);
    hipStream_t stream = reinterpret_cast<hipStream_t>(stream_);
    const LwgConvArgs& a = *pa;
    const size_t lds = (size_t)(W4_BIAS_OFF + 64) * 4;
    const dim3 grid = cw_persistent_grid(cw_total_blocks(a.B, a.H, a.W, a.N, 4 * W4_PBX, 4 * W4_PBY, W4_NB), lwg_device_cus());
    return a.epi == LWG_EPI_SPADE ? cw_launch_lists<lwg_conv_winograd4_list_kernel<LWG_EPI_SPADE>>(grid, W4_THREADS, lds, stream, a, *pl)
                                  : cw_launch_lists<lwg_conv_winograd4_list_kernel<LWG_EPI_NONE>>(grid, W4_THREADS, lds, stream, a, *pl);
}

extern "C" int lwg_conv2d_winograd4_fine_f32(const LwgConvArgs* pa, const LwgConvLists* pl, lwg_stream_t stream_) {
    if (!lwg_wino4_list_ok(pa) || !pl || !pl->heavy || !pl->light || !pl->counts || !pl->cal) return (int)hipErrorInvalidValue;
    if (!lwg_conv2d_winograd4_list_applies(pa)) return lwg_conv2d_winograd4_f32(pa, stream_);
    hipStream_t stream = reinterpret_cast<hipStream_t>(stream_);
    const LwgConvArgs& a = *pa;
    const size_t lds = (size_t)(W4F_BIAS_OFF + 64) * 4, ldsp = (size_t)(W4_BIAS_OFF + 64) * 4;
    const dim3 grid = cw_persistent_grid(cw_total_blocks(a.B, a.H, a.W, a.N, 4 * W4_PBX, 4 * W4_PBY, W4_NB), lwg_device_cus());
    const int e = a.epi == LWG_EPI_SPADE ? cw_launch_lists<lwg_conv_winograd4_fine_kernel<LWG_EPI_SPADE>>(grid, W4_THREADS, lds, stream, a, *pl)
                                         : cw_launch_lists<lwg_conv_winograd4_fine_kernel<LWG_EPI_NONE>>(grid, W4_THREADS, lds, stream, a, *pl);
    if (e != 0) return e;
    return a.epi == LWG_EPI_SPADE ? cw_launch_lists<lwg_conv_winograd4_fine_plain_kernel<LWG_EPI_SPADE>>(grid, W4_THREADS, ldsp, stream, a, *pl)
                                  : cw_launch_lists<lwg_conv_winograd4_fine_plain_kernel<LWG_EPI_NONE>>(grid, W4_THREADS, ldsp, stream, a, *pl);
}
```

### ipercore_amd/csrc/lwg_conv_wino.h

```cpp
#pragma once
#include <stddef.h>
#include "lwg_conv_args.h"

#ifdef __HIPCC__
#define CW_FN __host__ __device__ __forceinline__
#else
#define CW_FN static inline
#endif
#ifdef __HIP_DEVICE_COMPILE__
#define CW_UNIFORM(v) __builtin_amdgcn_readfirstlane(v)
#else
#define CW_UNIFORM(v) (v)
#endif
#define CW_OOB 0xC0000000u
#define CW_KS 8
#define CW_NB 64
struct CwGrid { int bx, by, tiles, total; };
CW_FN CwGrid cw_grid(int B, int H, int W, int N, int ex, int ey, int nbv) {
    const int bx = (W + ex - 1) / ex, by = (H + ey - 1) / ey, tiles = bx * by * B;
    return CwGrid{bx, by, tiles, tiles * (N / nbv)};
}
CW_FN long long cw_total_blocks(int B, int H, int W, int N, int ex, int ey, int nbv) {
    return (long long)((W + ex - 1) / ex) * ((H + ey - 1) / ey) * B * (N / nbv);
}

enum { CW_COLMAJOR = 0, CW_CHUNK = 1, CW_XCD = 2 };
struct CwOrder { int kind, nwg, wg, ncb, tiles, total, xg, xr; };

CW_FN int cw4_order_kind(int xcd_sw, int chunk_sw, bool sm, unsigned nwg, int ncb, int Cin, int N, int tiles, int total) {
    const bool xcd = xcd_sw && !sm && (nwg & 7u) == 0 && (ncb == 4 || ncb == 8 || (ncb == 2 && (Cin >= 192 || xcd_sw == 2))) && (int)nwg < total && tiles >= (int)nwg / ncb;
    return xcd ? CW_XCD : chunk_sw == 2 || (chunk_sw == 1 && 144u * (unsigned)Cin * (unsigned)N <= (5u << 20)) ? CW_CHUNK : CW_COLMAJOR;
}
CW_FN CwOrder cw_order(int kind, unsigned nwg, unsigned wg, int ncb, const CwGrid& g) {
    return CwOrder{kind, (int)nwg, (int)wg, ncb, g.tiles, g.total, (int)nwg / ncb, (int)(((wg & 7u) / (unsigned)ncb) * (nwg >> 3) + (wg >> 3))};
}
CW_FN bool cw_has_block(const CwOrder& o, int id) {
    return o.kind == CW_XCD ? (id / o.nwg) * o.xg + o.xr < o.tiles : id < o.total;
}
CW_FN void cw_block(const CwOrder& o, int id, int& cb, int& t) {
    if (o.kind == CW_XCD) {
        cb = (int)((unsigned)o.wg & 7u) & (o.ncb - 1);
        t = CW_UNIFORM((id / o.nwg) * o.xg + o.xr);
    } else if (o.kind == CW_CHUNK) {
        const int G = o.nwg, per = G * o.ncb;
        const int ch = CW_UNIFORM(id / per);
        const int r = id - ch * per, base = ch * G;
        const int nt = o.tiles - base < G ? o.tiles - base : G;
        cb = CW_UNIFORM(r / nt);
        t = CW_UNIFORM(base + r - cb * nt);
    } else {
        cb = CW_UNIFORM(id / o.tiles);
        t = CW_UNIFORM(id - cb * o.tiles);
    }
}
CW_FN int cw_image(const CwGrid& g, int t) { return t / (g.bx * g.by); }
CW_FN void cw_corner(const CwGrid& g, int t_in_image, int ex, int ey, int& x0, int& y0) { x0 = (t_in_image % g.bx) * ex, y0 = (t_in_image / g.bx) * ey; }
CW_FN int cw_n0(int cb, int nbv) { return cb * nbv; }
CW_FN int cw4_n0_spade_small(int cb) { return (cb >> 1) * 64 + (cb & 1) * 16; }
CW_FN int cw_halo_pixel(int i, int hw, int nel, int lgp, int x0, int y0, int H, int W) {
    const int pix = i >> lgp, hy = pix / hw, hx = pix - hy * hw;
    const int gy = y0 - 1 + hy, gx = x0 - 1 + hx;
    return i < nel && gy >= 0 && gy < H && gx >= 0 && gx < W ? gy * W + gx : -1;
}
CW_FN unsigned cw_halo_pixel_voff(int lin, int i, int lgp, int C, int ebytes) {
    return lin >= 0 ? (unsigned)(lin * C + (16 / ebytes) * (i & ((1 << lgp) - 1))) * (unsigned)ebytes : CW_OOB;
}
CW_FN unsigned cw_halo_voff(int i, int hw, int nel, int lgp, int x0, int y0, int H, int W, int C, int ebytes) {
    return cw_halo_pixel_voff(cw_halo_pixel(i, hw, nel, lgp, x0, y0, H, W), i, lgp, C, ebytes);
}
CW_FN bool cw_stage_second(int c, int C0, bool two) { return two && c >= C0; }
CW_FN unsigned cw_stage_soff(int c, int C0, bool two, int ebytes) { return (unsigned)(cw_stage_second(c, C0, two) ? c - C0 : c) * (unsigned)ebytes; }
CW_FN unsigned cw4_out_voff(int ox, int oy, int H, int W, int YC, int chan) {
    return ox < W && oy < H ? (unsigned)((oy * W + ox) * YC + chan) * 4u : CW_OOB;
}
CW_FN unsigned cw4_out_group(unsigned vo, int h, bool grouped) { return vo + (grouped ? 128u * (unsigned)h : 0u); }

struct CwWindow { int x0, y0, x1, y1; };
CW_FN CwWindow cw_block_window(int x0, int y0, int ex, int ey, int d, int H, int W) {
    return CwWindow{x0 - d > 0 ? x0 - d : 0, y0 - d > 0 ? y0 - d : 0, x0 + ex + d < W ? x0 + ex + d : W, y0 + ey + d < H ? y0 + ey + d : H};
}
CW_FN void cw_list_entry(int e, int ncb, int& slot, int& cb) { slot = e / ncb, cb = e - slot * ncb; }
CW_FN int cw_list_first_light(int wg, int nwg, int nhe) { return wg >= nhe ? wg : wg + (nhe - wg + nwg - 1) / nwg * nwg; }
CW_FN void cw4_light_elem(int tid, int it, int nth, int nq, int& px, int& py, int& q4) {
    const int e = it * nth + tid, p = e / nq;
    q4 = e - p * nq, px = p & 31, py = p >> 5;
}

#define CW4F_SX 16
#define CW4F_SY 8
#define CW4F_NSX (32 / CW4F_SX)
#define CW4F_NS (CW4F_NSX * (16 / CW4F_SY))
#define CW4F_HW (CW4F_SX + 2)
#define CW4F_HH (CW4F_SY + 2)
#define CW4F_NEL (CW4F_HW * CW4F_HH * 2)
#define CW4F_ROUNDS ((CW4F_NEL + 63) / 64)
CW_FN int cw4f_slot_of_patch(int pty, int ptx) { return (pty / (CW4F_SY / 4)) * CW4F_NSX + ptx / (CW4F_SX / 4); }
CW_FN void cw4f_patch_in_slot(int pty, int ptx, int& ly, int& lx) { ly = pty % (CW4F_SY / 4), lx = ptx % (CW4F_SX / 4); }
CW_FN void cw4f_corner(const CwGrid& g, int u, int& b, int& x0, int& y0) {
    const int t = u / CW4F_NS, s = u - t * CW4F_NS;
    b = cw_image(g, t);
    cw_corner(g, t - b * g.bx * g.by, 32, 16, x0, y0);
    x0 += (s % CW4F_NSX) * CW4F_SX, y0 += (s / CW4F_NSX) * CW4F_SY;
}
CW_FN bool cw4f_in_image(int x0, int y0, int H, int W) { return x0 < W && y0 < H; }
CW_FN int cw4f_in_image_total(int B, int H, int W) { return B * ((W + CW4F_SX - 1) / CW4F_SX) * ((H + CW4F_SY - 1) / CW4F_SY); }
CW_FN int cw4f_groups(int nh) { return (nh + CW4F_NS - 1) / CW4F_NS; }
CW_FN int cw4f_slot_index(int grp, int k, int nh) { return grp * CW4F_NS + k < nh ? grp * CW4F_NS + k : -1; }
CW_FN unsigned cw4f_reached(int x, int y, int x0, int y0, int d) {
    unsigned m = 0;
    for (int s = 0; s < CW4F_NS; ++s) {
        const int sx = x0 + (s % CW4F_NSX) * CW4F_SX, sy = y0 + (s / CW4F_NSX) * CW4F_SY;
        m |= (x >= sx - d && x < sx + CW4F_SX + d && y >= sy - d && y < sy + CW4F_SY + d ? 1u : 0u) << s;
    }
    return m;
}
CW_FN void cw4f_halo_elem(int i, int& slot, int& j) {
    const int wave = (i >> 6) & 7, k = i >> 9, per = CW4F_ROUNDS / 3, wr = 3 * wave + k;
    slot = wave / per, j = (wr - slot * CW4F_ROUNDS) * 64 + (i & 63);
}
CW_FN void cw4f_halo_place(int j, int& hy, int& hx, int& hq) {
    const int pix = j >> 1;
    hq = j & 1, hy = pix / CW4F_HW, hx = pix - hy * CW4F_HW;
}
CW_FN unsigned cw4f_halo_voff(bool present, int j, int x0, int y0, int H, int W, int C) {
    int hy, hx, hq;
    cw4f_halo_place(j, hy, hx, hq);
    const int gy = y0 - 1 + hy, gx = x0 - 1 + hx;
    return present && j < CW4F_NEL && gy >= 0 && gy < H && gx >= 0 && gx < W ? (unsigned)((gy * W + gx) * C + 4 * hq) * 4u : CW_OOB;
}
CW_FN void cw4f_light_pixel(int& px, int& py) {
    const int p = py * 32 + px;
    py = p / CW4F_SX, px = p - py * CW4F_SX;
}

#define CW4_SPLIT_MIN_STAGES 8
#define CW4_SPLIT_MAX_SLICES 8
struct Cw4Split { int slices, sps; };
CW_FN Cw4Split cw4_split_plan(long long blocks32, int nst, int cus, bool finishable, bool slab_ok) {
    if (!finishable || !slab_ok || blocks32 < 1 || 2 * blocks32 > (long long)cus) return Cw4Split{0, 0};
    int want = (int)((long long)cus / blocks32);
    if (want > CW4_SPLIT_MAX_SLICES) want = CW4_SPLIT_MAX_SLICES;
    int sps = (nst + want - 1) / want;
    if (sps < CW4_SPLIT_MIN_STAGES) sps = CW4_SPLIT_MIN_STAGES;
    sps += sps & 1;
    const int slices = (nst + sps - 1) / sps;
    return slices < 2 ? Cw4Split{0, 0} : Cw4Split{slices, sps};
}
CW_FN int cw4_slice_begin(int slice, int sps) { return slice * sps; }
CW_FN int cw4_slice_end(int slice, int sps, int nst) { return (slice + 1) * sps < nst ? (slice + 1) * sps : nst; }
CW_FN size_t cw4_slab_offset(int slice, int M, int N) { return (size_t)slice * (size_t)M * (size_t)N; }
CW_FN bool cw4_slab_image_ok(int H, int W, int N) { return (unsigned long long)H * W * N * 4ull + 256ull < (unsigned long long)CW_OOB; }

#define CW_NO_OUT_BUFFER (-1ll)
CW_FN bool cw_contract_ok(const LwgConvArgs& a, unsigned long long pair_bytes, long long out_slack) {
    if (!a.x0 || !a.w || !a.y || a.M <= 0 || a.ntaps != 9 || a.stride != 1 || a.omul != 1 || a.C0 <= 0 || (a.C0 % CW_KS) != 0 || a.C1 < 0 ||
        (a.C1 % CW_KS) != 0 || ((a.C0 + a.C1) % (2 * CW_KS)) != 0 || (a.C1 > 0 && !a.x1) || a.N <= 0 || (a.N % CW_NB) != 0 || a.OH != a.H ||
        a.OW != a.W || a.YH != a.H || a.YW != a.W || a.xdt != LWG_DT_F32 || a.ydt != LWG_DT_F32 || (long long)a.M != (long long)a.B * a.H * a.W ||
        a.ycoff < 0 || (a.ycoff % 4) != 0 || (a.YC % 4) != 0 || (a.act == LWG_ACTIVATION_RELU_MASK && a.epi != LWG_EPI_RESIDUAL))
        return false;
    if (a.epi == LWG_EPI_SPADE) {
        if (!a.xn || !a.mean || !a.rstd || !a.bias || a.YC * 2 != a.N || a.ycoff != 0) return false;
    } else {
        if (a.ycoff + a.N > a.YC) return false;
        if (a.epi != LWG_EPI_NONE && (a.epi != LWG_EPI_RESIDUAL || !a.res)) return false;
    }
    const unsigned long long cmax = (unsigned long long)(a.C0 > a.C1 ? a.C0 : a.C1);
    if ((unsigned long long)a.H * a.W * cmax * 4ull >= (unsigned long long)CW_OOB || pair_bytes * (a.C0 + a.C1) * a.N >= 0xffffffffull) return false;
    if (out_slack >= 0 && (unsigned long long)a.H * a.W * a.YC * 4ull + (unsigned long long)out_slack >= (unsigned long long)CW_OOB) return false;
    return true;
}
CW_FN bool cw_contract_calib_ok(const LwgConvArgs& a) {
    return (unsigned long long)a.H * a.W * (unsigned long long)(a.epi == LWG_EPI_SPADE ? a.N : a.YC) * 4ull + 256ull < (unsigned long long)CW_OOB;
}
CW_FN bool cwb_contract_ok(const LwgConvArgs& a) {
    if (!a.x0 || !a.w || !a.y || a.B <= 0 || a.H <= 0 || a.W <= 0 || a.C0 <= 0 || a.C1 < 0 || a.N <= 0 || a.xdt != LWG_DT_BF16 || a.ydt != LWG_DT_BF16 ||
        a.ntaps != 9 || a.stride != 1 || a.omul != 1 || a.ooy != 0 || a.oox != 0 || a.OH != a.H || a.OW != a.W || a.YH != a.H || a.YW != a.W ||
        (long long)a.M != (long long)a.B * a.H * a.W)
        return false;
    for (int t = 0; t < 9; ++t)
        if (a.dy[t] != t / 3 - 1 || a.dx[t] != t % 3 - 1) return false;
    const int Cin = a.C0 + a.C1;
    if (a.N % 64 != 0 || Cin % 64 != 0 || (a.YC & 7) != 0 || (a.ycoff & 7) != 0 || a.ycoff < 0 || (a.C1 != 0 && (a.C0 % 64 != 0 || !a.x1))) return false;
    if (a.act != LWG_ACTIVATION_NONE && a.act != LWG_ACTIVATION_RELU && a.act != LWG_ACTIVATION_TANH && a.act != LWG_ACTIVATION_SIGMOID) return false;
    if ((unsigned long long)a.H * a.W * (unsigned long long)(a.C0 > a.C1 ? a.C0 : a.C1) * 2ull >= (unsigned long long)CW_OOB ||
        32ull * (unsigned long long)Cin * (unsigned long long)a.N >= (unsigned long long)CW_OOB || cw_total_blocks(a.B, a.H, a.W, a.N, 16, 16, 64) >= 0x7fffffffll)
        return false;
    if (a.epi == LWG_EPI_SPADE) return a.xn && a.mean && a.rstd && a.bias && a.YC * 2 == a.N && a.ycoff == 0;
    return a.ycoff + a.N <= a.YC && (a.epi == LWG_EPI_NONE || (a.epi == LWG_EPI_RESIDUAL && a.res));
}

struct LwgWinoTaps { int t[9]; };
CW_FN bool cw_panel_args_ok(const float* wpanel, const float* upk, int Cin, int N, const int* tap9, LwgWinoTaps& taps) {
    if (!wpanel || !upk || !tap9 || Cin <= 0 || (Cin % 32) != 0 || N <= 0) return false;
    for (int i = 0; i < 9; ++i) {
        if (tap9[i] < 0 || tap9[i] > 8) return false;
        taps.t[i] = tap9[i];
    }
    return true;
}

#ifdef __HIPCC__
#include "lwg_common.h"

template <int V> struct IntC { static constexpr int value = V; };
template <int POLICY = 0>
__device__ __forceinline__ floatx4 cw_buf_load(__amdgpu_buffer_rsrc_t r, unsigned voff, unsigned soff) {
    return __builtin_bit_cast(floatx4, __builtin_amdgcn_raw_buffer_load_b128(r, (int)voff, (int)soff, POLICY));
}
__device__ __forceinline__ __amdgpu_buffer_rsrc_t cw_image_rsrc(const void* x, int b, int H, int W, int C, unsigned ebytes) {
    const unsigned img = (unsigned)(H * W);
    return __builtin_amdgcn_make_buffer_rsrc(const_cast<char*>(static_cast<const char*>(x)) + (size_t)b * img * C * ebytes, 0, (int)(img * (unsigned)C * ebytes), 0x00020000);
}

template <int NQ, bool TWO>
struct CwBlock {
    int b, x0, y0, n0;
    __amdgpu_buffer_rsrc_t rx0, rx1;
    unsigned voff0[NQ], voff1[NQ];

    __device__ __forceinline__ void locate(const LwgConvArgs& a, const CwGrid& g, int t, int ex, int ey, int n) {
        b = __builtin_amdgcn_readfirstlane(cw_image(g, t));
        cw_corner(g, t - b * g.bx * g.by, ex, ey, x0, y0);
        n0 = n;
        rx0 = cw_image_rsrc(a.x0, b, a.H, a.W, a.C0, 4u);
        if constexpr (TWO) rx1 = cw_image_rsrc(a.x1, b, a.H, a.W, a.C1, 4u);
    }
    __device__ __forceinline__ void halo(const LwgConvArgs& a, int tid, int nth, int hw, int nel) {
#pragma unroll
        for (int k = 0; k < NQ; ++k) {
            voff0[k] = cw_halo_voff(tid + nth * k, hw, nel, 1, x0, y0, a.H, a.W, a.C0, 4);
            if constexpr (TWO) voff1[k] = cw_halo_voff(tid + nth * k, hw, nel, 1, x0, y0, a.H, a.W, a.C1, 4);
        }
    }
    template <int POLICY = 0>
    __device__ __forceinline__ floatx4 rld1(const LwgConvArgs& a, int c, int k) const {
        if constexpr (!TWO) {
            return cw_buf_load<POLICY>(rx0, voff0[k], cw_stage_soff(c, a.C0, false, 4));
        } else {
            const bool second = cw_stage_second(c, a.C0, true);
            const __amdgpu_buffer_rsrc_t r = second ? rx1 : rx0;
            const unsigned v = second ? voff1[k] : voff0[k];
            return cw_buf_load<POLICY>(r, v, cw_stage_soff(c, a.C0, true, 4));
        }
    }
};
__device__ __forceinline__ void cw_rst1(float* dst, int plane, floatx4 v) {
#pragma unroll
    for (int k = 0; k < 4; ++k) dst[k * plane] = v[k];
}

template <void (*KERNEL)(const LwgConvArgs)>
static inline int cw_launch(dim3 grid, unsigned threads, size_t lds, hipStream_t stream, const LwgConvArgs& a) {
    static unsigned long long done = 0ull;
    if (hipError_t e = lwg_allow_dynamic_lds(reinterpret_cast<const void*>(KERNEL), lds, done); e != hipSuccess) return (int)e;
    hipLaunchKernelGGL(KERNEL, grid, dim3(threads), lds, stream, a);
    return (int)hipGetLastError();
}
template <void (*KERNEL)(const LwgConvArgs, const LwgConvLists)>
static inline int cw_launch_lists(dim3 grid, unsigned threads, size_t lds, hipStream_t stream, const LwgConvArgs& a, const LwgConvLists& l) {
    static unsigned long long done = 0ull;
    if (hipError_t e = lwg_allow_dynamic_lds(reinterpret_cast<const void*>(KERNEL), lds, done); e != hipSuccess) return (int)e;
    hipLaunchKernelGGL(KERNEL, grid, dim3(threads), lds, stream, a, l);
    return (int)hipGetLastError();
}
static inline dim3 cw_persistent_grid(long long total, int cus) { return dim3((unsigned)(LWG_WINO_PERSIST && total > cus ? cus : total)); }
#endif
```

### ipercore_amd/csrc/spade_skip.hip

```cpp
#include <hip/hip_runtime.h>
#include "lwg_common.h"
#include "lwg_conv_wino.h"
#include "lwg_lwb_taps.h"

#define SK_EX 32
#define SK_EY 16

__global__ __launch_bounds__(256) void lwg_spade_skip_mark_kernel(const float2* __restrict__ T, int B, int ns, int h, int w, int d, int* __restrict__ marks) {
    const CwGrid g = cw_grid(B, h, w, CW_NB, SK_EX, SK_EY, CW_NB);
    const int t = blockIdx.x, b = cw_image(g, t);
    int x0, y0;
    cw_corner(g, t - b * g.bx * g.by, SK_EX, SK_EY, x0, y0);
    const CwWindow win = cw_block_window(x0, y0, SK_EX, SK_EY, d, h, w);
    const int ww = win.x1 - win.x0, n = ww * (win.y1 - win.y0);
    bool mine = false;
    for (int s = 0; s < ns; ++s) {
        const float2* Ts = T + ((size_t)b * ns + s) * h * w;
        for (int i = threadIdx.x; i < n; i += 256) {
            const int yy = i / ww, y = win.y0 + yy, x = win.x0 + (i - yy * ww);
            float wt[4];
            int tx0, ty0;
            lwb_taps_of(Ts[(size_t)y * w + x], w, h, wt, tx0, ty0);
            mine |= lwb_tap_in_image(tx0, ty0, w, h);
        }
    }
    const int any = __syncthreads_or(mine ? 1 : 0);
    if (threadIdx.x == 0) marks[t] = any ? 1 : 0;
}

__global__ __launch_bounds__(1024) void lwg_spade_skip_scan_kernel(const int* __restrict__ marks, int n, int* __restrict__ heavy, int* __restrict__ light,
                                                                   int* __restrict__ counts) {
    __shared__ int part[1024];
    const int tid = threadIdx.x, per = (n + 1023) / 1024;
    const int i0 = tid * per < n ? tid * per : n, i1 = i0 + per < n ? i0 + per : n;
    int c = 0;
    for (int i = i0; i < i1; ++i) c += marks[i] != 0;
    part[tid] = c;
    __syncthreads();
    for (int off = 1; off < 1024; off <<= 1) {
        const int v = tid >= off ? part[tid - off] : 0;
        __syncthreads();
        part[tid] += v;
        __syncthreads();
    }
    int hv = part[tid] - c;
    for (int i = i0; i < i1; ++i) {
        if (marks[i] != 0) heavy[hv++] = i;
        else light[i - hv] = i;
    }
    if (tid == 1023) {
        counts[0] = part[1023];
        counts[1] = n - part[1023];
    }
}

__global__ __launch_bounds__(256) void lwg_spade_skip_mark_fine_kernel(const float2* __restrict__ T, int B, int ns, int h, int w, int d, int* __restrict__ marks,
                                                                       int* __restrict__ fmarks) {
    const CwGrid g = cw_grid(B, h, w, CW_NB, SK_EX, SK_EY, CW_NB);
    const int t = blockIdx.x, b = cw_image(g, t);
    int x0, y0;
    cw_corner(g, t - b * g.bx * g.by, SK_EX, SK_EY, x0, y0);
    const CwWindow win = cw_block_window(x0, y0, SK_EX, SK_EY, d, h, w);
    const int ww = win.x1 - win.x0, n = ww * (win.y1 - win.y0);
    unsigned mine = 0;
    for (int s = 0; s < ns; ++s) {
        const float2* Ts = T + ((size_t)b * ns + s) * h * w;
        for (int i = threadIdx.x; i < n; i += 256) {
            const int yy = i / ww, y = win.y0 + yy, x = win.x0 + (i - yy * ww);
            float wt[4];
            int tx0, ty0;
            lwb_taps_of(Ts[(size_t)y * w + x], w, h, wt, tx0, ty0);
            if (lwb_tap_in_image(tx0, ty0, w, h)) mine |= (1u << CW4F_NS) | cw4f_reached(x, y, x0, y0, d);
        }
    }
    unsigned all = 0;
    for (int s = 0; s <= CW4F_NS; ++s) all |= __syncthreads_or((int)((mine >> s) & 1u)) ? 1u << s : 0u;
    if (threadIdx.x < CW4F_NS) {
        const int s = threadIdx.x;
        const bool in = cw4f_in_image(x0 + (s % CW4F_NSX) * CW4F_SX, y0 + (s / CW4F_NSX) * CW4F_SY, h, w);
        fmarks[CW4F_NS * t + s] = in ? (int)((all >> s) & 1u) : 2;
    } else if (threadIdx.x == CW4F_NS) {
        marks[t] = (int)((all >> CW4F_NS) & 1u);
    }
}

struct SkScanJob { const int* marks; int n; int* heavy; int* light; int* counts; };
template <typename F>
__device__ __forceinline__ void sk_for_marks(const int* __restrict__ marks, int i0, int i1, bool vec, F f) {
    int i = i0;
    if (vec)
        for (; i + 4 <= i1; i += 4) {
            const int4 m = *reinterpret_cast<const int4*>(marks + i);
            f(i, m.x), f(i + 1, m.y), f(i + 2, m.z), f(i + 3, m.w);
        }
    for (; i < i1; ++i) f(i, marks[i]);
}
__global__ __launch_bounds__(1024) void lwg_spade_skip_scan2_kernel(SkScanJob j0, SkScanJob j1) {
    __shared__ int ph[1024], pl[1024];
    const SkScanJob j = blockIdx.x == 0 ? j0 : j1;
    const int tid = threadIdx.x, n = j.n, per = ((n + 1023) / 1024 + 3) & ~3;
    const int i0 = tid * per < n ? tid * per : n, i1 = i0 + per < n ? i0 + per : n;
    const bool vec = (reinterpret_cast<size_t>(j.marks) & 15) == 0;
    int ch = 0, cl = 0;
    sk_for_marks(j.marks, i0, i1, vec, [&](int, int m) { ch += m == 1, cl += m == 0; });
    ph[tid] = ch, pl[tid] = cl;
    __syncthreads();
    for (int off = 1; off < 1024; off <<= 1) {
        const int vh = tid >= off ? ph[tid - off] : 0, vl = tid >= off ? pl[tid - off] : 0;
        __syncthreads();
        ph[tid] += vh, pl[tid] += vl;
        __syncthreads();
    }
    int hv = ph[tid] - ch, lt = pl[tid] - cl;
    sk_for_marks(j.marks, i0, i1, vec, [&](int i, int m) {
        if (m == 1) j.heavy[hv++] = i;
        else if (m == 0) j.light[lt++] = i;
    });
    if (tid == 1023) {
        j.counts[0] = ph[1023];
        j.counts[1] = pl[1023];
    }
}

extern "C" int lwg_spade_skip_fine_lists_f32(const float* T, int B, int ns, int h, int w, int d, int* marks, int* heavy, int* light, int* counts,
                                             int* fmarks, int* fheavy, int* flight, int* fcounts, lwg_stream_t stream_) {
    if (!T || !marks || !heavy || !light || !counts || !fmarks || !fheavy || !flight || !fcounts || B <= 0 || ns <= 0 || h <= 0 || w <= 0 || d < 0 || d > 64)
        return (int)hipErrorInvalidValue;
    const long long tiles = cw_total_blocks(B, h, w, CW_NB, SK_EX, SK_EY, CW_NB);
    if (tiles * CW4F_NS >= (1ll << 30) || (long long)h * w >= (1ll << 30)) return (int)hipErrorInvalidValue;
    hipStream_t stream = reinterpret_cast<hipStream_t>(stream_);
    hipLaunchKernelGGL(lwg_spade_skip_mark_fine_kernel, dim3((unsigned)tiles), dim3(256), 0, stream, reinterpret_cast<const float2*>(T), B, ns, h, w, d, marks, fmarks);
    hipLaunchKernelGGL(lwg_spade_skip_scan2_kernel, dim3(2), dim3(1024), 0, stream, SkScanJob{marks, (int)tiles, heavy, light, counts},
                       SkScanJob{fmarks, (int)tiles * CW4F_NS, fheavy, flight, fcounts});
    return (int)hipGetLastError();
}

extern "C" int lwg_spade_skip_lists_f32(const float* T, int B, int ns, int h, int w, int d, int* marks, int* heavy, int* light, int* counts,
                                        lwg_stream_t stream_) {
    if (!T || !marks || !heavy || !light || !counts || B <= 0 || ns <= 0 || h <= 0 || w <= 0 || d < 0 || d > 64) return (int)hipErrorInvalidValue;
    const long long tiles = cw_total_blocks(B, h, w, CW_NB, SK_EX, SK_EY, CW_NB);
    if (tiles >= (1ll << 30) || (long long)h * w >= (1ll << 30)) return (int)hipErrorInvalidValue;
    hipStream_t stream = reinterpret_cast<hipStream_t>(stream_);
    hipLaunchKernelGGL(lwg_spade_skip_mark_kernel, dim3((unsigned)tiles), dim3(256), 0, stream, reinterpret_cast<const float2*>(T), B, ns, h, w, d, marks);
    hipLaunchKernelGGL(lwg_spade_skip_scan_kernel, dim3(1), dim3(1024), 0, stream, marks, (int)tiles, heavy, light, counts);
    return (int)hipGetLastError();
}
```

### ipercore_amd/ops.py

```python
import ctypes

import torch

from . import _lib
from ._lib import ACT_LRELU, ACT_NONE, ACT_RELU, ACT_RELU_MASK, ACT_SIGMOID, ACT_TANH, EPI_NONE, EPI_RESIDUAL, EPI_SPADE

EYE_DIST = 2.7320508075688776


def _ptr(t, dtype=torch.float32):
    if t is None:
        return None
    if not t.is_cuda:
        raise RuntimeError("ipercore_amd ops need CUDA (HIP) tensors: the MI355X path has no CPU fallback")
    if t.dtype != dtype:
        raise TypeError(f"expected {dtype}, got {t.dtype}")
    if not t.is_contiguous():
        raise ValueError("tensor must be contiguous")
    return t.data_ptr()


CONV_PRECISION = "fp32"


# ... 20 lines not shown


def _stream():
    return torch.cuda.current_stream().cuda_stream


class ConvSpec:
    __slots__ = ("w", "bias", "N", "Cin", "ntaps", "dy", "dx", "stride", "cshift", "omul", "ooy", "oox", "algo_kn", "_panels")

    def __init__(self, w, bias, N, Cin, taps, stride=1, omul=1, ooy=0, oox=0, algo_kn=None):
        self.w, self.bias, self.N, self.Cin = w, bias, int(N), int(Cin)
        self.algo_kn = int(algo_kn) if algo_kn is not None else len(taps) * int(Cin) * int(N)
        self.ntaps = len(taps)
        self.dy = [int(t[0]) for t in taps]
        self.dx = [int(t[1]) for t in taps]
        self.stride, self.omul, self.ooy, self.oox = stride, omul, ooy, oox
        self._panels = {}
        self.cshift = 0
        if self.Cin % 32 != 0:
            q = self.Cin // 4
            assert q in (1, 2, 4), "small-Cin path handles Cin in {4, 8, 16}"
            self.cshift = q.bit_length() - 1


def _derived(specs, key, build, bias=False):
    specs = specs if isinstance(specs, (list, tuple)) else (specs,)
    src = [s.w for s in specs] + ([specs[0].bias] if bias else [])
    hit = specs[0]._panels.get(key)
    if hit is None or len(hit[0]) != len(src) or any(a is not b for a, b in zip(hit[0], src)):
        hit = specs[0]._panels[key] = (src, build())
    return hit[1]


def _tap_order9(spec):
    order = [0] * 9
    for t in range(spec.ntaps):
        order[3 * (spec.dy[t] + 1) + spec.dx[t] + 1] = t
    return order


def _spade_columns(N, blk, device):
    j = torch.arange(N, device=device)
    ch, beta = blk * (j // (2 * blk)) + j % blk, (j % (2 * blk)) // blk
    return 64 * (ch // 32) + (ch % 32) + 32 * beta


def _w16v2(spec):
    def build():
        K4, N, _ = spec.w.shape
        cin, nt = spec.Cin, spec.ntaps
        assert cin % 64 == 0 and K4 * 4 == nt * cin, (cin, nt, K4)
        wk = spec.w.permute(0, 2, 1).reshape(cin // 64, 2, nt, 32, N)
        wk = wk.permute(0, 2, 1, 3, 4).reshape(cin // 64 * nt, 64, N)
        rows = wk.permute(0, 2, 1).reshape(cin // 64 * nt, N, 8, 8)
        n = torch.arange(N, device=spec.w.device)
        slot = torch.arange(8, device=spec.w.device)
        src = slot[None, :] ^ ((n[:, None] >> 1) & 7)
        rows = torch.gather(rows, 2, src[None, :, :, None].expand(rows.shape[0], N, 8, 8))
        return rows.reshape(cin // 64 * nt, N, 64).contiguous().to(torch.bfloat16)
    return _derived(spec, "w16v2", build)


def _hr_eligible(spec, x0, y, out_hw):
    if not BF16_HR or spec.stride != 1 or spec.ntaps not in (9, 4) or spec.N % 64 != 0 or spec.Cin % 64 != 0:
        return False
    if any(abs(d) > 1 for d in spec.dy) or any(abs(d) > 1 for d in spec.dx):
        return False
    OH, OW = ((y.shape[1], y.shape[2]) if spec.omul == 1 else (y.shape[1] // spec.omul, y.shape[2] // spec.omul)) if out_hw is None else out_hw
    return (OH, OW) == (x0.shape[1], x0.shape[2])


def _hr_tap_order(spec):
    return sorted(range(spec.ntaps), key=lambda t: (spec.dy[t], spec.dx[t]))


def _w16hr(spec, spade):
    def build():
        K4, N, _ = spec.w.shape
        cin, nt = spec.Cin, spec.ntaps
        wk = spec.w.permute(0, 2, 1).reshape(cin // 64, 2, nt, 32, N).permute(0, 2, 1, 3, 4).reshape(cin // 64, nt, 64, N)
        wk = wk[:, _hr_tap_order(spec)].reshape(cin // 64 * nt, 64, N)
        bias = spec.bias
        if spade:
            old = _spade_columns(N, 16, spec.w.device)
            wk = wk[:, :, old]
            bias = None if bias is None else bias[old].contiguous()
        return wk.reshape(cin // 64 * nt, 4, 16, N).permute(0, 1, 3, 2).contiguous().to(torch.bfloat16), bias
    return _derived(spec, ("w16hr", bool(spade)), build, bias=True)


BF16_WINO_MIN_CIN = 64
_WINO_G = ((1.0, 0.0, 0.0), (0.5, 0.5, 0.5), (0.5, -0.5, 0.5), (0.0, 0.0, 1.0))


def _bf16_wino_eligible(spec, x0, y, x1, epi, act, out_hw, ycoff=0):
    if spec.ntaps != 9 or spec.stride != 1 or spec.omul != 1 or spec.N % 64 != 0 or spec.Cin % 64 != 0 or spec.Cin < BF16_WINO_MIN_CIN:
        return False
    if (y.shape[1], y.shape[2]) != (x0.shape[1], x0.shape[2]) or (out_hw is not None and tuple(out_hw) != (x0.shape[1], x0.shape[2])):
        return False
    if sorted(zip(spec.dy, spec.dx)) != _WINO_TAPS or epi not in (EPI_NONE, EPI_RESIDUAL, EPI_SPADE):
        return False
    if act not in (ACT_NONE, ACT_RELU, ACT_TANH, ACT_SIGMOID) or y.dtype != torch.bfloat16:
        return False
    if x1 is not None and (x1.dtype != torch.bfloat16 or x0.shape[3] % 64 != 0):
        return False
    if epi == EPI_SPADE:
        return y.shape[3] * 2 == spec.N and ycoff == 0
    return y.shape[3] % 8 == 0 and ycoff % 8 == 0 and ycoff + spec.N <= y.shape[3]


def wwino16_index(ks, p, n, e, N):
    return ((ks * 16 + p) * N + n) * 16 + e


def wwino16_spade_column(j):
    return 4 * (j // 8) + j % 4, (j % 8) // 4


def _wwino16(spec, spade):
    def build():
        K4, N, _ = spec.w.shape
        cin, nt = spec.Cin, spec.ntaps
        assert nt == 9 and cin % 64 == 0 and N % 64 == 0 and K4 * 4 == nt * cin, (cin, nt, K4, N)
        dev = spec.w.device
        wk = spec.w.permute(0, 2, 1).reshape(cin // 32, nt, 32, N).permute(1, 0, 2, 3).reshape(nt, cin, N)
        w33 = wk[_tap_order9(spec)].reshape(3, 3, cin, N).to(torch.float64)
        G = torch.tensor(_WINO_G, dtype=torch.float64, device=dev)
        U = torch.einsum("ar,rscn,bs->abcn", G, w33, G)
        bias = spec.bias
        if spade:
            old = _spade_columns(N, 4, dev)
            U = U[:, :, :, old]
            bias = None if bias is None else bias[old].contiguous()
        return U.reshape(16, cin // 16, 16, N).permute(1, 0, 3, 2).contiguous().to(torch.bfloat16), bias
    return _derived(spec, ("wwino16", bool(spade)), build, bias=True)


BF16_HR = True
BF16_PW = True
BF16_C8 = True


def _pw_eligible(spec, x0, y, x1, epi, out_hw):
    if not BF16_PW or spec.ntaps != 1 or spec.stride != 1 or spec.omul != 1 or x1 is not None or epi != EPI_NONE:
        return False
    if spec.dy[0] != 0 or spec.dx[0] != 0 or spec.N != spec.Cin or spec.N not in (64, 128, 256):
        return False
    OH, OW = (y.shape[1], y.shape[2]) if out_hw is None else out_hw
    return (OH, OW) == (x0.shape[1], x0.shape[2])


def _w16c8(spec):
    def build():
        K4, N, _ = spec.w.shape
        nks = (spec.ntaps + 1) // 2
        wk = spec.w.permute(0, 2, 1).reshape(K4 * 4, N)
        if wk.shape[0] < nks * 16:
            wk = torch.cat([wk, wk.new_zeros(nks * 16 - wk.shape[0], N)], dim=0)
        return wk[:nks * 16].reshape(nks, 16, N).permute(0, 2, 1).contiguous().to(torch.bfloat16)
    return _derived(spec, "w16c8", build)


def _w16x3(spec):
    def build():
        K4, N, _ = spec.w.shape
        wk = spec.w.permute(0, 2, 1).reshape(K4 * 4, N)
        hi = wk.to(torch.bfloat16)
        r1 = wk - hi.float()
        mid = r1.to(torch.bfloat16)
        lo = (r1 - mid.float()).to(torch.bfloat16)
        return torch.stack([hi, mid, lo]).view(3, K4 // 2, 8, N).permute(0, 1, 3, 2).contiguous()
    return _derived(spec, "w16x3", build)


_WINO_TAPS = sorted((dy, dx) for dy in (-1, 0, 1) for dx in (-1, 0, 1))


def _wino_eligible(spec, x0, y, x1, epi, act, out_hw, q4, ycoff=0):
    if q4 or x0.dtype != torch.float32 or y.dtype != torch.float32 or epi not in (EPI_NONE, EPI_RESIDUAL, EPI_SPADE) or \
            (act == ACT_RELU_MASK and epi != EPI_RESIDUAL):
        return False
    if x1 is not None and (x1.dtype != torch.float32 or x0.shape[3] % 8 != 0 or x1.shape[3] % 8 != 0):
        return False
    if spec.ntaps != 9 or spec.stride != 1 or spec.omul != 1 or spec.Cin % 32 != 0 or spec.N % 64 != 0:
        return False
    if epi == EPI_SPADE and (y.shape[3] * 2 != spec.N or ycoff != 0):
        return False
    if sorted(zip(spec.dy, spec.dx)) != _WINO_TAPS:
        return False
    hw = (y.shape[1], y.shape[2]) if out_hw is None else tuple(out_hw)
    return hw == (x0.shape[1], x0.shape[2]) == (y.shape[1], y.shape[2])


WINO_MIN_GRID = 128
WINO_SPLITK = True


def _wino_plan(a, spec, y, splitk):
    if not splitk:
        return 0
    blocks, slices, nbv = ctypes.c_longlong(0), ctypes.c_int(0), ctypes.c_int(0)
    if _lib.lib().lwg_conv2d_winograd_plan(a, 1 if WINO_SPLITK else 0, ctypes.byref(blocks), ctypes.byref(slices), ctypes.byref(nbv), None) != 0:
        return None
    units32 = blocks.value * (nbv.value // 32)
    return slices.value * a.M * spec.N if units32 >= WINO_MIN_GRID else None


def _wwino(spec):
    def build():
        cin, N, tap9 = _wino_panel_source(spec)
        if PANEL_CACHE is not None:
            U = PANEL_CACHE.winograd(spec, list(tap9))
            if U is not None:
                return U
        U = torch.empty(16, cin // 8, 2, N, 4, device=spec.w.device, dtype=torch.float32)
        _lib.check(_lib.lib().lwg_winograd_panel_f32(_ptr(spec.w), _ptr(U), cin, N, tap9, _stream()), "lwg_winograd_panel_f32")
        return U
    return _derived(spec, "wwino", build)


def _wino_panel_source(spec):
    K4, N, _ = spec.w.shape
    cin, nt = spec.Cin, spec.ntaps
    assert nt == 9 and cin % 32 == 0 and K4 * 4 == nt * cin, (cin, nt, K4)
    if not spec.w.is_cuda:
        raise RuntimeError("ipercore_amd ops need CUDA (HIP) tensors: the MI355X path has no CPU fallback")
    return cin, N, (ctypes.c_int * 9)(*_tap_order9(spec))


WINO4 = True
WINO4_MIN_CIN = 64


TRAIN_CONV_TILES = "2x2"


class train_conv_tiles(object):

    def __init__(self, mode):
        assert mode in ("2x2", "4x4")
        self.mode = mode

    def __enter__(self):
        global TRAIN_CONV_TILES
        self.prev = TRAIN_CONV_TILES
        TRAIN_CONV_TILES = self.mode

    def __exit__(self, *exc):
        global TRAIN_CONV_TILES
        TRAIN_CONV_TILES = self.prev


def _wino4_use(spec, splitk):
    return WINO4 and _MODE_WINO4 and spec.Cin >= WINO4_MIN_CIN and (not splitk or TRAIN_CONV_TILES == "4x4")


WINO4_TRAIN_MIN_GRID = 129
WINO4_TRAIN_MIN_SLICE_CIN = 128
WINO4_TRAIN_WHOLE = True
WINO4_TRAIN_SPLITK = True


def _wino4_plan(a):
    blocks, slices, nbv = ctypes.c_longlong(0), ctypes.c_int(0), ctypes.c_int(0)
    if _lib.lib().lwg_conv2d_winograd4_plan(a, 1, ctypes.byref(blocks), ctypes.byref(slices), ctypes.byref(nbv), None) != 0:
        return None
    if not (WINO4_TRAIN_SPLITK if slices.value else WINO4_TRAIN_WHOLE) or blocks.value * (nbv.value // 32) < WINO4_TRAIN_MIN_GRID:
        return None
    if slices.value and a.C0 + a.C1 < WINO4_TRAIN_MIN_SLICE_CIN * slices.value:
        return None
    return slices.value * a.M * a.N


def _wino_route(a, spec, y, splitk):
    if _wino4_use(spec, splitk):
        n4 = _wino4_plan(a) if splitk else 0
        if n4 is not None:
            return True, n4
    n = _wino_plan(a, spec, y, splitk)
    return None if n is None else (False, n)


def _wwino4(spec):
    def build():
        cin, N, tap9 = _wino_panel_source(spec)
        if PANEL_CACHE is not None:
            U = PANEL_CACHE.winograd4(spec, list(tap9))
            if U is not None:
                return U
        U = torch.empty(4, cin // 8, 4, 2, 9 * N, device=spec.w.device, dtype=torch.float32)
        _lib.check(_lib.lib().lwg_winograd4_panel_f32(_ptr(spec.w), _ptr(U), cin, N, tap9, _stream()), "lwg_winograd4_panel_f32")
        return U
    return _derived(spec, "wwino4", build)


SPADE_SKIP = True
SPADE_SKIP_D = (1, 5)
SPADE_SKIP_BF16 = False
SPADE_SKIP_D_BF16 = (1, 2)


SPADE_SKIP_FINE = True

_LISTS_APPLY = {}


class SkipLists(tuple):
    fine = None


def spade_skip_fine_apply(x0):
    return SPADE_SKIP_FINE


def spade_skip_lists(flow, d):
    B, ns, h, w, two = flow.shape
    assert two == 2 and flow.dtype == torch.float32
    tiles = B * ((h + 15) // 16) * ((w + 31) // 32)
    buf = torch.empty(15 * tiles + 4, device=flow.device, dtype=torch.int32)
    fmarks, fheavy, flight = buf[:4 * tiles], buf[4 * tiles:8 * tiles], buf[8 * tiles:12 * tiles]
    bb = buf[12 * tiles:]
    marks, heavy, light, counts, fcounts = bb[:tiles], bb[tiles:2 * tiles], bb[2 * tiles:3 * tiles], bb[3 * tiles:3 * tiles + 2], bb[3 * tiles + 2:]
    i32 = torch.int32
    _lib.check(_lib.lib().lwg_spade_skip_fine_lists_f32(_ptr(flow), B, ns, h, w, int(d), _ptr(marks, i32), _ptr(heavy, i32), _ptr(light, i32),
                                                        _ptr(counts, i32), _ptr(fmarks, i32), _ptr(fheavy, i32), _ptr(flight, i32), _ptr(fcounts, i32),
                                                        _stream()), "lwg_spade_skip_fine_lists_f32")
    out = SkipLists((heavy, light, counts))
    out.fine = (fheavy, flight, fcounts)
    return out


def conv2d_lists_apply(x0, spec, y, epi=EPI_NONE, act=ACT_NONE, xn=None, mean=None, rstd=None):
    if x0.dtype == torch.bfloat16 or y.dtype == torch.bfloat16:
        if not SPADE_SKIP or not SPADE_SKIP_BF16 or CONV_PRECISION != "bf16" or not x0.is_cuda or x0.dtype != y.dtype or not _hr_eligible(spec, x0, y, None):
            return False
        key = ("bf16", x0.shape, y.shape, spec.Cin, spec.N, spec.ntaps, epi, act)
        if key not in _LISTS_APPLY:
            _LISTS_APPLY[key] = bool(_lib.lib().lwg_conv2d_nhwc_bf16_hr_list_applies(_hr_args(conv_args(x0, spec, y, None, epi, act, None, xn, mean, rstd), spec, epi)))
        return _LISTS_APPLY[key]
    if not SPADE_SKIP or CONV_PRECISION != "winograd" or not x0.is_cuda or x0.dtype != torch.float32 or not _wino4_use(spec, False) or \
            not _wino_eligible(spec, x0, y, None, epi, act, None, False):
        return False
    key = (x0.shape, y.shape, spec.Cin, spec.N, epi, act)
    if key not in _LISTS_APPLY:
        a = conv_args(x0, spec, y, None, epi, act, None, xn, mean, rstd)
        a.w = _ptr(_wwino4(spec))
        _LISTS_APPLY[key] = bool(_lib.lib().lwg_conv2d_winograd4_list_applies(a))
    return _LISTS_APPLY[key]


def conv_args(x0, spec, y, x1=None, epi=EPI_NONE, act=ACT_NONE, res=None, xn=None, mean=None, rstd=None,
              out_hw=None, ycoff=0, q4=False):
    B, H, W, C0 = x0.shape
    C1 = 0 if x1 is None else x1.shape[3]
    assert C0 + C1 == spec.Cin, (C0, C1, spec.Cin)
    if q4:
        YB, YCq, YH, YW, four = y.shape
        assert four == 4 and y.dtype == torch.float32 and x0.dtype == torch.float32 and epi == EPI_NONE and y.is_contiguous()
        YC = 4 * YCq
    else:
        YB, YH, YW, YC = y.shape
    if out_hw is None:
        OH, OW = (YH, YW) if spec.omul == 1 else (YH // spec.omul, YW // spec.omul)
    else:
        OH, OW = out_hw
    a = _lib.LwgConvArgs()
    xdt, ydt = x0.dtype, y.dtype
    a.xdt = _lib.DT_BF16 if xdt == torch.bfloat16 else _lib.DT_F32
    a.ydt = _lib.DT_F32_Q4 if q4 else (_lib.DT_BF16 if ydt == torch.bfloat16 else _lib.DT_F32)
    a.x0, a.x1 = _ptr(x0, xdt), _ptr(x1, xdt)
    a.C0, a.C1 = C0, C1
    a.B, a.H, a.W = B, H, W
    a.OH, a.OW, a.M = OH, OW, B * OH * OW
    a.stride, a.ntaps, a.cshift = spec.stride, spec.ntaps, spec.cshift
    a.w, a.N, a.bias = _ptr(spec.w), spec.N, _ptr(spec.bias)
    a.y, a.YH, a.YW, a.YC, a.ycoff = _ptr(y, ydt), YH, YW, YC, ycoff
    a.omul, a.ooy, a.oox = spec.omul, spec.ooy, spec.oox
    a.epi, a.act = epi, act
    a.res, a.xn, a.mean, a.rstd = _ptr(res, ydt), _ptr(xn, ydt), _ptr(mean), _ptr(rstd)
    for i in range(spec.ntaps):
        a.dy[i] = spec.dy[i]
        a.dx[i] = spec.dx[i]
    return a


def _hr_args(a, spec, epi):
    panel, bias = _w16hr(spec, epi == EPI_SPADE)
    a.w, a.bias = _ptr(panel, torch.bfloat16), _ptr(bias)
    for i, t in enumerate(_hr_tap_order(spec)):
        a.dy[i], a.dx[i] = spec.dy[t], spec.dx[t]
    return a


def conv2d_acc_frame(x0, spec, spade=True):
    B, H, W, _ = x0.shape
    y = torch.empty(B, H, W, spec.N, device=x0.device, dtype=torch.float32)
    a = conv_args(x0, spec, y)
    a.ydt = _lib.DT_F32
    _hr_args(a, spec, EPI_SPADE if spade else EPI_NONE)
    _lib.check(_lib.lib().lwg_conv2d_nhwc_bf16_hr_acc(a, _stream()), "lwg_conv2d_nhwc_bf16_hr_acc")
    return y


def _hook_end(a, spec, epi, kind, slices=True, extra=0):
    n = (max(1, int(_lib.lib().lwg_conv_slice_count(a))) if slices else 1) + extra
    CONV_HOOK(False, a.M, spec, epi, {"kernels": n, "kind": kind})


def conv2d(x0, spec, y, x1=None, epi=EPI_NONE, act=ACT_NONE, res=None, xn=None, mean=None, rstd=None,
           out_hw=None, ycoff=0, splitk=False, q4=False, lists=None):
    a = conv_args(x0, spec, y, x1, epi, act, res, xn, mean, rstd, out_hw, ycoff, q4)
    if q4 and (splitk or CONV_PRECISION not in ("fp32", "winograd") or x0.dtype != torch.float32):
        raise ValueError("channel-quad-plane outputs: fp32 activations on the fp32 MFMA path, no split-K")
    if CONV_HOOK is not None:
        CONV_HOOK(True, a.M, spec, epi, None)
    if lists is not None and not (x0.dtype == torch.float32 and y.dtype == torch.float32 and CONV_PRECISION == "winograd" and _wino4_use(spec, splitk)) and \
            not (x0.dtype == torch.bfloat16 and y.dtype == torch.bfloat16 and CONV_PRECISION == "bf16" and x1 is None and spec.ntaps == 9 and
                 _hr_eligible(spec, x0, y, out_hw)):
        raise ValueError("lists: the F(4x4, 3x3) launches of the \"winograd\" mode and the 3 x 3 launches of the \"bf16\" mode only (conv2d_lists_apply)")
    kind, sliced, extra = "direct", True, 0
    if x0.dtype == torch.bfloat16:
        kind = "bf16"
        if y.dtype != torch.bfloat16 or spec.Cin % 64 != 0:
            raise ValueError("bf16 convolutions need bf16 outputs and Cin % 64 == 0")
        if CONV_PRECISION == "bf16_winograd" and _bf16_wino_eligible(spec, x0, y, x1, epi, act, out_hw, ycoff):
            kind, sliced = "bf16_winograd", False
            panel, bias = _wwino16(spec, epi == EPI_SPADE)
            a.w, a.bias = _ptr(panel, torch.bfloat16), _ptr(bias)
            for i, (dy, dx) in enumerate(_WINO_TAPS):
                a.dy[i], a.dx[i] = dy, dx
            _lib.check(_lib.lib().lwg_conv2d_winograd_bf16(a, _stream()), "lwg_conv2d_winograd_bf16")
        elif _hr_eligible(spec, x0, y, out_hw) or _pw_eligible(spec, x0, y, x1, epi, out_hw):
            _hr_args(a, spec, epi)
            if lists is not None:
                sliced = False
                if len(lists) == 2 and isinstance(lists[0], SkipLists):
                    lists = tuple(lists[0].fine) + (lists[1],)
                i32 = torch.int32
                nsub = x0.shape[0] * ((x0.shape[1] + 7) // 8) * ((x0.shape[2] + 15) // 16)
                if min(lists[0].numel(), lists[1].numel()) < nsub or lists[2].numel() < 2 or \
                        lists[3].numel() != x0.shape[1] * x0.shape[2] * (spec.N if epi == EPI_SPADE else y.shape[3]):
                    raise ValueError("lists: the sub-tile lists of this frame batch and ONE calibration frame at its feature size")
                ld = _lib.LwgConvLists(_ptr(lists[0], i32), _ptr(lists[1], i32), _ptr(lists[2], i32),
                                       _ptr(lists[3], torch.float32 if epi == EPI_SPADE else torch.bfloat16))
                _lib.check(_lib.lib().lwg_conv2d_nhwc_bf16_hr_list(a, ctypes.byref(ld), _stream()), "lwg_conv2d_nhwc_bf16_hr_list")
            else:
                _lib.check(_lib.lib().lwg_conv2d_nhwc_bf16_hr(a, _stream()), "lwg_conv2d_nhwc_bf16_hr")
        else:
            a.w = _ptr(_w16v2(spec), torch.bfloat16)
            _lib.check(_lib.lib().lwg_conv2d_nhwc_bf16(a, _stream()), "lwg_conv2d_nhwc_bf16")
    elif y.dtype == torch.bfloat16:
        if BF16_C8 and spec.Cin == 8 and spec.N == 64 and spec.ntaps <= 10 and x1 is None and epi == EPI_NONE and spec.omul == 1:
            a.w = _ptr(_w16c8(spec), torch.bfloat16)
            _lib.check(_lib.lib().lwg_conv2d_nhwc_c8_bf16(a, _stream()), "lwg_conv2d_nhwc_c8_bf16")
        else:
            _lib.check(_lib.lib().lwg_conv2d_nhwc_f32(a, _stream()), "lwg_conv2d_nhwc_f32")
    elif CONV_PRECISION == "winograd" and _wino_eligible(spec, x0, y, x1, epi, act, out_hw, q4, ycoff) and \
            (route := _wino_route(a, spec, y, splitk)) is not None:
        kind, sliced = "winograd", False
        four, nws = route
        if four:
            a.w = _ptr(_wwino4(spec))
            kind = "winograd4"
            if lists is not None:
                i32 = torch.int32
                fine = len(lists) == 2 and isinstance(lists[0], SkipLists)
                if fine:
                    sl, cal = lists
                    fine = sl.fine is not None and spade_skip_fine_apply(x0)
                    lists = tuple(sl.fine if fine else sl) + (cal,)
                ld = _lib.LwgConvLists(_ptr(lists[0], i32), _ptr(lists[1], i32), _ptr(lists[2], i32), _ptr(lists[3]))
                if fine:
                    _lib.check(_lib.lib().lwg_conv2d_winograd4_fine_f32(a, ctypes.byref(ld), _stream()), "lwg_conv2d_winograd4_fine_f32")
                else:
                    _lib.check(_lib.lib().lwg_conv2d_winograd4_list_f32(a, ctypes.byref(ld), _stream()), "lwg_conv2d_winograd4_list_f32")
            elif nws:
                ws, extra = torch.empty(nws, device=x0.device, dtype=torch.float32), 1
                _lib.check(_lib.lib().lwg_conv2d_winograd4_f32_ws(a, _ptr(ws), _stream()), "lwg_conv2d_winograd4_f32_ws")
            else:
                _lib.check(_lib.lib().lwg_conv2d_winograd4_f32(a, _stream()), "lwg_conv2d_winograd4_f32")
        elif nws:
            a.w = _ptr(_wwino(spec))
            ws, extra = torch.empty(nws, device=x0.device, dtype=torch.float32), 1
            _lib.check(_lib.lib().lwg_conv2d_winograd_f32_ws(a, _ptr(ws), _stream()), "lwg_conv2d_winograd_f32_ws")
        else:
            a.w = _ptr(_wwino(spec))
            _lib.check(_lib.lib().lwg_conv2d_winograd_f32(a, _stream()), "lwg_conv2d_winograd_f32")
    elif CONV_PRECISION == "split" and spec.Cin % 32 == 0:
        a.w = _ptr(_w16x3(spec), torch.bfloat16)
        kind = "split"
        _lib.check(_lib.lib().lwg_conv2d_nhwc_f32_split(a, _stream()), "lwg_conv2d_nhwc_f32_split")
    else:
        nws = _lib.lib().lwg_conv2d_ws_floats(a) if splitk else 0
        if nws:
            ws = torch.empty(nws, device=x0.device, dtype=torch.float32)
            _lib.check(_lib.lib().lwg_conv2d_nhwc_f32_ws(a, _ptr(ws), _stream()), "lwg_conv2d_nhwc_f32_ws")
        else:
            _lib.check(_lib.lib().lwg_conv2d_nhwc_f32(a, _stream()), "lwg_conv2d_nhwc_f32")
    if CONV_HOOK is not None:
        _hook_end(a, spec, epi, kind, sliced, extra)
    return y


WINO_UP4 = True
F32_UP4 = True
BF16_UP4 = True


def _parity_specs_ok(specs):
    s0 = specs[0]
    return (len(specs) == 4 and all(s.ntaps == 4 and s.omul == 2 and s.stride == 1 and (s.ooy, s.oox) == (i >> 1, i & 1) and s.N == s0.N and s.Cin == s0.Cin
                                    and [(dy - (i >> 1), dx - (i & 1)) for dy, dx in zip(s.dy, s.dx)] == list(zip(s0.dy, s0.dx)) for i, s in enumerate(specs)))


def _wwino_t(specs):
    def build():
        Cin, N = specs[0].Cin, specs[0].N
        G = torch.tensor([[1.0, 0.0], [1.0, 1.0], [0.0, 1.0]], dtype=torch.float64, device=specs[0].w.device)
        parts = []
        for par, g in enumerate(_parity_subkernels(specs)):
            u = torch.einsum("ar,rqcn,bq->abcn", G, g, G)
            if par >> 1:
                u[0] = -u[0]
            if par & 1:
                u[:, 0] = -u[:, 0]
            parts.append(u.reshape(9, Cin, N))
        U9 = torch.stack(parts).float()
        U = torch.cat([U9[:, 0:4].permute(0, 2, 3, 1).reshape(4, Cin, 4 * N), U9[:, 4:8].permute(0, 2, 3, 1).reshape(4, Cin, 4 * N), U9[:, 8]], dim=2)
        return U.view(4, Cin // 8, 4, 2, 9 * N).contiguous()
    return _derived(specs, "wwino_t", build)


def _parity_subkernels(specs):
    Cin, N = specs[0].Cin, specs[0].N
    out = []
    for par, sp in enumerate(specs):
        py, px = par >> 1, par & 1
        W = sp.w.double().permute(0, 2, 1).reshape(4 * Cin, N)
        W = W.view(Cin // 32, 4, 32, N).permute(1, 0, 2, 3).reshape(4, Cin, N)
        g = torch.zeros(2, 2, Cin, N, dtype=torch.float64, device=W.device)
        for t, (dy, dx) in enumerate(zip(sp.dy, sp.dx)):
            g[dy - (py - 1), dx - (px - 1)] = W[t]
        out.append(g)
    return out


_G_X24 = ((1.0, 0.0), (0.5, 0.5), (-1.0 / 6.0, 1.0 / 6.0), (-8.0 / 3.0, -4.0 / 3.0), (0.0, 0.5))


def _wwino_t24(specs):
    def build():
        Cin, N = specs[0].Cin, specs[0].N
        Gy = torch.tensor([[1.0, 0.0], [1.0, 1.0], [0.0, 1.0]], dtype=torch.float64, device=specs[0].w.device)
        Gx = torch.tensor(_G_X24, dtype=torch.float64, device=specs[0].w.device)
        parts = []
        for par, g in enumerate(_parity_subkernels(specs)):
            u = torch.einsum("ar,rqcn,bq->abcn", Gy, g, Gx)
            if par >> 1:
                u[0] = -u[0]
            parts.append(torch.cat([u[:, :3].reshape(9, Cin, N), u[:, 3:].reshape(6, Cin, N)]))
        U15 = torch.stack(parts).float()
        quad = lambda lo, hi: U15[:, lo:hi].permute(0, 2, 3, 1).reshape(4, Cin, (hi - lo) * N)
        U = torch.cat([quad(0, 4), quad(4, 8), U15[:, 8], quad(9, 13), U15[:, 13], U15[:, 14]], dim=2)
        return U.view(4, Cin // 8, 4, 2, 15 * N).contiguous()
    return _derived(specs, "wwino_t24", build)


WINO_UP4_24 = True
WINO_UP4_24_MIN_HW = 64 * 64


def _up4_24(x):
    return WINO_UP4_24 and x.shape[1] * x.shape[2] >= WINO_UP4_24_MIN_HW


class _FusedTransposeSpec(object):

    def __init__(self, s0, panel):
        self.N, self.Cin, self.ntaps, self.stride, self.omul = 4 * s0.N, s0.Cin, 16, 1, 2
        self.algo_kn, self.w = 4 * s0.algo_kn, panel


def _fused_transpose_launch(a, s0, panel, entry, kind, sliced=True, extra=(), kernels=None):
    a.w = _ptr(panel, panel.dtype)
    if CONV_HOOK is not None:
        whole = _FusedTransposeSpec(s0, panel)
        CONV_HOOK(True, a.M, whole, EPI_NONE, None)
    _lib.check(getattr(_lib.lib(), entry)(a, *extra, _stream()), entry)
    if CONV_HOOK is not None:
        if kernels is None:
            _hook_end(a, whole, EPI_NONE, kind, sliced)
        else:
            CONV_HOOK(False, a.M, whole, EPI_NONE, {"kernels": kernels, "kind": kind})


def _w16up(specs):
    return _derived(specs, "w16up", lambda: torch.stack([_w16hr(s, False)[0] for s in specs]).contiguous())


def _w32up(specs):
    return _derived(specs, "w32up", lambda: torch.stack([s.w.reshape(-1) for s in specs]).contiguous())


def conv_transpose2d(x, specs, y, act=ACT_NONE, splitk=False, out_hw=None, q4=False):
    s0 = specs[0]
    if (BF16_UP4 and BF16_HR and x.dtype == torch.bfloat16 and y.dtype == torch.bfloat16 and len(specs) == 4 and s0.Cin in (64, 128)
            and s0.N % 64 == 0 and all(s.ntaps == 4 and s.omul == 2 and (s.ooy, s.oox) == (i >> 1, i & 1) for i, s in enumerate(specs))):
        _fused_transpose_launch(conv_args(x, s0, y, act=act), s0, _w16up(specs), "lwg_conv_transpose4_nhwc_bf16", "up4")
        return y
    if (WINO_UP4 and CONV_PRECISION == "winograd" and not splitk and out_hw is None and x.is_cuda and x.dtype == torch.float32 and y.dtype == torch.float32
            and s0.Cin % 32 == 0 and s0.N % 32 == 0 and _parity_specs_ok(specs)):
        a = conv_args(x, s0, y, act=act, q4=q4)
        if _up4_24(x):
            _fused_transpose_launch(a, s0, _wwino_t24(specs), "lwg_conv_transpose4_winograd24_f32", "winograd_up4", False)
        else:
            _fused_transpose_launch(a, s0, _wwino_t(specs), "lwg_conv_transpose4_winograd_f32", "winograd_up4", False)
        return y
    if (F32_UP4 and x.is_cuda and x.dtype == torch.float32 and y.dtype == torch.float32 and CONV_PRECISION in ("fp32", "winograd") and s0.Cin % 32 == 0
            and _parity_specs_ok(specs)):
        a = conv_args(x, s0, y, act=act, q4=q4)
        if _lib.lib().lwg_conv_transpose4_is_one_grid(a):
            _fused_transpose_launch(a, s0, _w32up(specs), "lwg_conv_transpose4_nhwc_f32", "up4")
            return y
    for s in specs:
        conv2d(x, s, y, act=act, splitk=splitk, out_hw=None if out_hw is None else out_hw(s), q4=q4)
    return y


def instnorm_stats(x, mean, rstd, ws, eps=1e-5, nsplit=None):
    B, H, W, C = x.shape
    HW = H * W
    if nsplit is None:
        nsplit = max(1, min(64, HW // 64))
    assert ws.numel() >= B * C * nsplit * 3
    if x.dtype == torch.bfloat16:
        _lib.check(_lib.lib().lwg_instnorm_stats_nhwc_bf16(_ptr(x, torch.bfloat16), B, HW, C, eps, _ptr(mean), _ptr(rstd), _ptr(ws), nsplit,
                                                            _stream()), "lwg_instnorm_stats_nhwc_bf16")
        return
    _lib.check(_lib.lib().lwg_instnorm_stats_nhwc_f32(_ptr(x), B, HW, C, eps, _ptr(mean), _ptr(rstd), _ptr(ws), nsplit,
                                                       _stream()), "lwg_instnorm_stats_nhwc_f32")


def instnorm_apply(x, mean, rstd, y, act=ACT_NONE, res=None):
    B, H, W, C = x.shape
    _lib.check(_lib.lib().lwg_instnorm_apply_nhwc_f32(_ptr(x), _ptr(mean), _ptr(rstd), _ptr(res), _ptr(y), B, H * W, C, act,
                                                       _stream()), "lwg_instnorm_apply_nhwc_f32")
    return y


def flow_resize(T, h, w):
    B, ns, S = T.shape[0], T.shape[1], T.shape[2]
    T = T.contiguous()
    out = torch.empty(B, ns, h, w, 2, device=T.device, dtype=torch.float32)
    _lib.check(_lib.lib().lwg_flow_resize_f32(_ptr(T), B * ns, S, h, w, _ptr(out), _stream()), "lwg_flow_resize_f32")
    return out


def lwb_attention(q, Ks, Vs, bk, bv, T, out, src_batched=False):
    B, h, w, C = q.shape
    ns = T.shape[1]
    S = T.shape[2]
    assert T.shape[0] == B and Ks.shape[0] == (B * ns if src_batched else ns) and tuple(Ks.shape[1:]) == (h, w, C)
    if q.dtype == torch.bfloat16:
        bf = torch.bfloat16
        _lib.check(_lib.lib().lwg_lwb_attention_bf16(_ptr(q, bf), _ptr(Ks, bf), _ptr(Vs, bf), _ptr(bk), _ptr(bv), _ptr(T), _ptr(out, bf), B, ns, h,
                                                      w, C, S, 1 if src_batched else 0, _stream()), "lwg_lwb_attention_bf16")
        return out
    _lib.check(_lib.lib().lwg_lwb_attention_f32(_ptr(q), _ptr(Ks), _ptr(Vs), _ptr(bk), _ptr(bv), _ptr(T), _ptr(out), B, ns, h,
                                                 w, C, S, 1 if src_batched else 0, _stream()), "lwg_lwb_attention_f32")
    return out


def attn_records(h, w, C, dtype=torch.float32):
    n = _lib.lib().lwg_lwb_attention_x_records(int(h), int(w), int(C), 2 if dtype == torch.bfloat16 else 4)
    if n <= 0:
        raise ValueError(f"lwb_attention_x: unsupported (h, w, C, dtype) = {(h, w, C, dtype)}")
    return n


def lwb_attention_x(x, Kq, kappa, Vs, bv, T, out, stats=None, src_batched=False):
    B, h, w, C = x.shape
    ns = T.shape[1]
    nsrc = B * ns if src_batched else ns
    assert tuple(T.shape) == (B, ns, h, w, 2), (tuple(T.shape), (B, ns, h, w, 2))
    assert tuple(Kq.shape) == (nsrc, h, w, C) and tuple(Vs.shape) == (nsrc, h, w, C) and tuple(kappa.shape) == (nsrc, h, w)
    assert Kq.dtype == x.dtype and Vs.dtype == x.dtype and out.dtype == x.dtype and kappa.dtype == torch.float32
    assert stats is None or stats.numel() >= B * attn_records(h, w, C, x.dtype) * C * 3
    if x.dtype == torch.bfloat16:
        bf = torch.bfloat16
        _lib.check(_lib.lib().lwg_lwb_attention_x_bf16(_ptr(x, bf), _ptr(Kq, bf), _ptr(kappa), _ptr(Vs, bf), _ptr(bv), _ptr(T), _ptr(out, bf),
                                                        _ptr(stats), B, ns, h, w, C, 1 if src_batched else 0, _stream()), "lwg_lwb_attention_x_bf16")
        return out
    _lib.check(_lib.lib().lwg_lwb_attention_x_f32(_ptr(x), _ptr(Kq), _ptr(kappa), _ptr(Vs), _ptr(bv), _ptr(T), _ptr(out), _ptr(stats), B, ns, h, w,
                                                   C, 1 if src_batched else 0, _stream()), "lwg_lwb_attention_x_f32")
    return out


def instnorm_finalize_ws(B, C, nrec):
    return int(_lib.lib().lwg_instnorm_finalize_ws_floats(int(B), int(C), int(nrec)))


def instnorm_finalize(ws, B, C, nrec, mean, rstd, eps=1e-5):
    assert ws.numel() >= instnorm_finalize_ws(B, C, nrec)
    _lib.check(_lib.lib().lwg_instnorm_finalize_f32(_ptr(ws), B, C, nrec, float(eps), _ptr(mean), _ptr(rstd), _stream()), "lwg_instnorm_finalize_f32")


def lwb_fuse(tsf_x, src_x, T, out, gate=None, scale_w=1.0, scale_o=1.0, src_batched=False):
    B, h, w, C = tsf_x.shape
    ns, S = T.shape[1], T.shape[2]
    assert T.shape[0] == B and src_x.shape[0] == (B * ns if src_batched else ns) and tuple(src_x.shape[1:]) == (h, w, C)
    assert src_x.dtype == tsf_x.dtype and out.dtype == tsf_x.dtype and (gate is None or gate.dtype == tsf_x.dtype)
    assert T.dtype == torch.float32
    if tsf_x.dtype == torch.bfloat16:
        bf = torch.bfloat16
        _lib.check(_lib.lib().lwg_lwb_fuse_bf16(_ptr(tsf_x, bf), _ptr(src_x, bf), _ptr(gate, bf), _ptr(T), _ptr(out, bf), B, ns, h, w, C, S,
                                                1 if src_batched else 0, float(scale_w), float(scale_o), _stream()), "lwg_lwb_fuse_bf16")
        return out
    _lib.check(_lib.lib().lwg_lwb_fuse_f32(_ptr(tsf_x), _ptr(src_x), _ptr(gate), _ptr(T), _ptr(out), B, ns, h, w, C, S,
                                           1 if src_batched else 0, float(scale_w), float(scale_o), _stream()), "lwg_lwb_fuse_f32")
    return out


def lwb_fuse_bwd(src_x, gate, T, dout, src_batched=False, scale_w=1.0, scale_o=1.0):
    B, h, w, C = dout.shape
    ns, S = T.shape[1], T.shape[2]
    assert T.shape[0] == B and src_x.shape[0] == (B * ns if src_batched else ns) and tuple(src_x.shape[1:]) == (h, w, C)
    assert gate is None or gate.shape == dout.shape
    dout = dout.contiguous()
    d_tsf = torch.empty_like(dout)
    d_src = torch.zeros_like(src_x)
    d_gate = None if gate is None else torch.empty_like(dout)
    _lib.check(_lib.lib().lwg_lwb_fuse_bwd_f32(_ptr(src_x), _ptr(gate), _ptr(T), _ptr(dout), _ptr(d_tsf), _ptr(d_src), _ptr(d_gate), B, ns, h, w, C,
                                               S, 1 if src_batched else 0, float(scale_w), float(scale_o), _stream()), "lwg_lwb_fuse_bwd_f32")
    return d_tsf, d_src, d_gate


def lwb_attention_bwd(q, Ks, Vs, bk, bv, T, dout, src_batched=False):
    B, h, w, C = q.shape
    ns, S = T.shape[1], T.shape[2]
    dout = dout.contiguous()
    dq = torch.empty_like(q)
    dKs = torch.zeros_like(Ks)
    dVs = torch.zeros_like(Vs)
    _lib.check(_lib.lib().lwg_lwb_attention_bwd_f32(_ptr(q), _ptr(Ks), _ptr(Vs), _ptr(bk), _ptr(bv), _ptr(T), _ptr(dout), _ptr(dq),
                                                     _ptr(dKs), _ptr(dVs), B, ns, h, w, C, S, 1 if src_batched else 0, _stream()),
               "lwg_lwb_attention_bwd_f32")
    return dq, dKs, dVs


def lwb_attention_kv(q, kv, bk, bv, T, out, src_batched=False):
    B, h, w, C = q.shape
    ns, S = T.shape[1], T.shape[2]
    assert T.shape[0] == B and kv.shape[0] == (B * ns if src_batched else ns) and tuple(kv.shape[1:]) == (h, w, 2 * C)
    _lib.check(_lib.lib().lwg_lwb_attention_kv_f32(_ptr(q), _ptr(kv), _ptr(bk), _ptr(bv), _ptr(T), _ptr(out), B, ns, h, w, C, S,
                                                    1 if src_batched else 0, _stream()), "lwg_lwb_attention_kv_f32")
    return out


def lwb_attention_kv_bwd(q, kv, bk, bv, T, dout, src_batched=False):
    B, h, w, C = q.shape
    ns, S = T.shape[1], T.shape[2]
    dout = dout.contiguous()
    dq = torch.empty_like(q)
    dkv = torch.zeros_like(kv)
    _lib.check(_lib.lib().lwg_lwb_attention_kv_bwd_f32(_ptr(q), _ptr(kv), _ptr(bk), _ptr(bv), _ptr(T), _ptr(dout), _ptr(dq), _ptr(dkv),
                                                        B, ns, h, w, C, S, 1 if src_batched else 0, _stream()), "lwg_lwb_attention_kv_bwd_f32")
    return dq, dkv


def project_faces(verts, cam, faces, want_faces_v=True, want_f2pts=True):
    B, nv, _ = verts.shape
    nf = faces.shape[0]
    fv = torch.empty(B, nf, 3, 3, device=verts.device, dtype=torch.float32) if want_faces_v else None
    f2 = torch.empty(B, nf, 3, 2, device=verts.device, dtype=torch.float32) if want_f2pts else None
    cam = cam.contiguous()
# ... 622 lines not shown
```

Baseline: 1362 frames/s.

## Add 8x8 sub-tile SPADE skip lists and Winograd4 kernel variant

Adds a finer 8x8-pixel sub-tile granularity to the SPADE skip machinery. A new mark kernel computes tile, 16x8 and 8x8 marks in one pass, and a three-job scan builds all three lists. The Winograd4 body gains a Q8 template path that gathers up to eight 8x8 heavy sub-tiles per block, with its own halo staging and epilogue corner handling. The goal is to skip more of the conv work on regions the warp flow never reaches, at the cost of extra halo loads, a second plain-kernel launch and more list-building work. It is gated by size thresholds (H*W at most 64x64, and a minimum count of tiles times channel blocks).

```diff
diff --git a/include/lwg_hip.h b/include/lwg_hip.h
--- a/include/lwg_hip.h
+++ b/include/lwg_hip.h
@@ -79,6 +79,9 @@
 int lwg_conv2d_winograd4_fine_f32(const LwgConvArgs* args, const LwgConvLists* lists, lwg_stream_t stream);
 int lwg_spade_skip_fine_lists_f32(const float* T, int B, int ns, int h, int w, int d, int* marks, int* heavy, int* light, int* counts, int* fmarks,
                                   int* fheavy, int* flight, int* fcounts, lwg_stream_t stream);
+int lwg_conv2d_winograd4_q8_f32(const LwgConvArgs* args, const LwgConvLists* lists, lwg_stream_t stream);
+int lwg_spade_skip_q8_lists_f32(const float* T, int B, int ns, int h, int w, int d, int* marks, int* heavy, int* light, int* counts, int* fmarks,
+                                int* fheavy, int* flight, int* fcounts, int* qmarks, int* qheavy, int* qlight, int* qcounts, lwg_stream_t stream);
 int lwg_winograd4_panel_f32(const float* wpanel, float* upk, int Cin, int N, const int* tap9, lwg_stream_t stream);
 int lwg_winograd4_panels_f32(const LwgWinoDesc* descs_dev, int ndesc, int total_blocks, lwg_stream_t stream);
 int lwg_conv2d_winograd4_f32_ws(const LwgConvArgs* args, float* ws, lwg_stream_t stream);
diff --git a/ipercore_amd/_lib.py b/ipercore_amd/_lib.py
--- a/ipercore_amd/_lib.py
+++ b/ipercore_amd/_lib.py
@@ -66,6 +66,8 @@
     "lwg_spade_skip_lists_f32": (c_i, [c_f, c_i, c_i, c_i, c_i, c_i, c_f, c_f, c_f, c_f, c_f]),
     "lwg_conv2d_winograd4_fine_f32": (c_i, [ctypes.POINTER(LwgConvArgs), ctypes.POINTER(LwgConvLists), c_f]),
     "lwg_spade_skip_fine_lists_f32": (c_i, [c_f, c_i, c_i, c_i, c_i, c_i, c_f, c_f, c_f, c_f, c_f, c_f, c_f, c_f, c_f]),
+    "lwg_conv2d_winograd4_q8_f32": (c_i, [ctypes.POINTER(LwgConvArgs), ctypes.POINTER(LwgConvLists), c_f]),
+    "lwg_spade_skip_q8_lists_f32": (c_i, [c_f, c_i, c_i, c_i, c_i, c_i, c_f, c_f, c_f, c_f, c_f, c_f, c_f, c_f, c_f, c_f, c_f, c_f, c_f]),
     "lwg_winograd4_panel_f32": (c_i, [c_f, c_f, c_i, c_i, ctypes.POINTER(c_i), c_f]),
     "lwg_winograd4_panels_f32": (c_i, [c_f, c_i, c_i, c_f]),
     "lwg_conv2d_winograd4_f32_ws": (c_i, [ctypes.POINTER(LwgConvArgs), c_f, c_f]),
diff --git a/ipercore_amd/csrc/conv_winograd4.hip b/ipercore_amd/csrc/conv_winograd4.hip
--- a/ipercore_amd/csrc/conv_winograd4.hip
+++ b/ipercore_amd/csrc/conv_winograd4.hip
@@ -30,6 +30,10 @@
 #define W4F_LOOP (2 * W4_KS * W4F_PLANE + 2 * W4_VS + W4_THREADS + 3 * W4F_PLANE)
 #define W4F_BIAS_OFF (W4F_LOOP > W4_MS ? W4F_LOOP : W4_MS)
 static_assert(CW4F_SX == 16 && CW4F_SY == 8 && CW4F_NS * CW4F_ROUNDS * 64 == W4_NQ * W4_THREADS, "sub-tile halo: four slots x six wave rounds = the staged elements");
+#define W4Q_NQ CW4Q_ROUNDS
+#define W4Q_LOOP (2 * W4_KS * CW4Q_PLANE + 2 * W4_VS + W4_THREADS + 3 * CW4Q_PLANE)
+#define W4Q_BIAS_OFF (W4Q_LOOP > W4_MS ? W4Q_LOOP : W4_MS)
+static_assert(CW4Q_NS == 8 && W4Q_NQ == 4 && CW4Q_RS % 4 == 0 && CW4Q_RS >= 16 + CW4Q_HW && (W4Q_BIAS_OFF + 64) * 4 <= 160 * 1024, "8 x 8 sub-tile halo: one slot per wave, inside the LDS");
 #ifndef LWG_W4_XCD
 #define LWG_W4_XCD 1
 #endif
@@ -88,19 +92,20 @@
     });
 }
 
-template <int EPI, bool TWO, bool SM, bool LIST, bool FINE = false, bool SPLIT = false>
+template <int EPI, bool TWO, bool SM, bool LIST, bool FINE = false, bool SPLIT = false, bool Q8 = false>
 __device__ __forceinline__ void w4_body(const LwgConvArgs& a, const LwgConvLists& sk) {
     static_assert(!FINE || (LIST && !SM && !TWO && LWG_W4_RDMAP), "the sub-tile form: a list-driven 8-wave launch");
+    static_assert(!Q8 || (LIST && !FINE && !SM && !TWO && !SPLIT && LWG_W4_RDMAP), "the 8 x 8 sub-tile form: a list-driven 8-wave launch");
     static_assert(!SPLIT || (SM && !LIST && EPI == LWG_EPI_NONE), "the split form: 4-wave blocks, plain epilogue");
-    constexpr int RS = W4_RS;
-    constexpr int PLANE = FINE ? W4F_PLANE : W4_PLANE;
+    constexpr int RS = Q8 ? CW4Q_RS : W4_RS;
+    constexpr int PLANE = Q8 ? CW4Q_PLANE : FINE ? W4F_PLANE : W4_PLANE;
     constexpr int RAW = W4_KS * PLANE;
     constexpr int DUMP_OFF = 2 * RAW + 2 * W4_VS;
-    constexpr int BIAS_OFF = FINE ? W4F_BIAS_OFF : W4_BIAS_OFF;
+    constexpr int BIAS_OFF = Q8 ? W4Q_BIAS_OFF : FINE ? W4F_BIAS_OFF : W4_BIAS_OFF;
     constexpr bool SMS = SM && EPI == LWG_EPI_SPADE;
     constexpr int NVP = SM && !SMS ? 2 : 1;
     constexpr int NTH = SM ? 256 : W4_THREADS;
-    constexpr int NQ = SM ? 5 : W4_NQ;
+    constexpr int NQ = SM ? 5 : W4_NQ + (Q8 ? W4Q_NQ - W4_NQ : 0);
     constexpr int NBV = SM ? 32 : W4_NB;
     constexpr int MSR = SM ? 36 : W4_MSR;
     constexpr int NHF = SM ? 2 : 1;
@@ -115,10 +120,10 @@
     const CwGrid g = cw_grid(a.B, H, W, N, 4 * W4_PBX, 4 * W4_PBY, NBV);
     const CwOrder o = cw_order(cw4_order_kind(LWG_W4_XCD, LWG_W4_CHUNK, SM, gridDim.x, N / NBV, Cin, N, g.tiles, g.total), gridDim.x, blockIdx.x, N / NBV, g);
     int blk = blockIdx.x;
-    const int nall = FINE ? cw4f_in_image_total(a.B, H, W) : g.tiles;
+    const int nall = Q8 ? cw4q_in_image_total(a.B, H, W) : FINE ? cw4f_in_image_total(a.B, H, W) : g.tiles;
     const int nht = LIST ? min(max(__builtin_amdgcn_readfirstlane(sk.counts[0]), 0), nall) : 0;
-    const int nhe = (FINE ? cw4f_groups(nht) : nht) * (N / NBV);
-    const bool lst = FINE ? true : LIST ? nht < nall : false;
+    const int nhe = (Q8 ? cw4q_groups(nht) : FINE ? cw4f_groups(nht) : nht) * (N / NBV);
+    const bool lst = FINE || Q8 ? true : LIST ? nht < nall : false;
     const bool run = lst ? blk < nhe : true;
     const int nst = Cin / W4_KS;
     const int sbeg = SPLIT ? cw4_slice_begin((int)blockIdx.z, a.cshift) : 0;
@@ -132,7 +137,28 @@
     int fs0 = 0, fs1 = 0;
     auto setup = [&](int id) {
         int cb, t;
-        if constexpr (FINE) {
+        if constexpr (Q8) {
+            int tids = tid;
+            asm volatile("" : "+v"(tids));
+            int slot;
+            cw_list_entry(id, N / NBV, slot, cb);
+            auto sub = [&](int k) {
+                const int ix = cw4q_slot_index(slot, k, nht);
+                return ix < 0 ? -1 : min(max(__builtin_amdgcn_readfirstlane(sk.heavy[ix]), 0), CW4Q_NS * g.tiles - 1);
+            };
+            bk.n0 = cw_n0(cb, NBV);
+            const int u = sub(wid);
+            int b, x0, y0;
+            cw4q_corner(g, max(u, 0), b, x0, y0);
+            bk.rx0 = cw_image_rsrc(a.x0, __builtin_amdgcn_readfirstlane(b), H, W, a.C0, 4u);
+#pragma unroll
+            for (int k = 0; k < NQ; ++k) {
+                int s, j;
+                cw4q_halo_elem(tids + NTH * k, s, j);
+                bk.voff0[k] = cw4q_halo_voff(u >= 0, j, x0, y0, H, W, a.C0);
+            }
+            fs0 = sub(wid >> 1), fs1 = sub(CW4Q_NSX + (wid >> 1));
+        } else if constexpr (FINE) {
             int tids = tid;
             asm volatile("" : "+v"(tids));
             int fsub[CW4F_NS], slot;
@@ -165,7 +191,7 @@
         } else {
             cw_block(o, id, cb, t);
         }
-        if constexpr (!FINE) {
+        if constexpr (!FINE && !Q8) {
         bk.locate(a, g, t, 4 * W4_PBX, 4 * W4_PBY, SMS ? cw4_n0_spade_small(cb) : cw_n0(cb, NBV));
         int tids = tid;
         asm volatile("" : "+v"(tids));
@@ -180,7 +206,12 @@
 #pragma unroll
     for (int k = 0; k < NQ; ++k) {
         const int i = tid + NTH * k;
-        if constexpr (FINE) {
+        if constexpr (Q8) {
+            int s, j, hy, hx, hq;
+            cw4q_halo_elem(i, s, j);
+            cw4q_halo_place(j, hy, hx, hq);
+            wst[k] = j < CW4Q_NEL ? 4 * hq * PLANE + cw4q_lds_slot(s) + hy * RS + hx : DUMP_OFF + tid;
+        } else if constexpr (FINE) {
             int s, j, hy, hx, hq;
             cw4f_halo_elem(i, s, j);
             cw4f_halo_place(j, hy, hx, hq);
@@ -232,6 +263,7 @@
         cw4f_patch_in_slot(pty, ptx, pby, pbx);
         pslot = W4F_SLOT(cw4f_slot_of_patch(pty, ptx));
     }
+    if constexpr (Q8) pby = 0, pbx = 0, pslot = cw4q_lds_patch(pty, ptx);
     unsigned dbs = (unsigned)(tc * PLANE + pslot + (4 * pby) * RS + 4 * pbx) >> 2;
     asm volatile("" : "+v"(dbs));
     dbs <<= 2;
@@ -371,6 +403,7 @@
             mf(0, 4, true); ul(0, 2); tr(0, 2);
             mf(0, 5, true); halo(2);
             mf(0, 6, true); tr(0, 3);
+            if constexpr (Q8) halo(3);
             mf(0, 7, true); tr(0, 4);
             mf(0, 8, true); tr(0, 5);
             mf(1, 0, true); ul(1, 0); tr(0, 6);
@@ -482,7 +515,7 @@
         iteration(s + 1, IntC<1>(), IntC<0>());
     }
     W4TS(2);
-    int eb = FINE ? 0 : bk.b, ex0 = FINE ? 0 : bk.x0, ey0 = FINE ? 0 : bk.y0;
+    int eb = FINE || Q8 ? 0 : bk.b, ex0 = FINE || Q8 ? 0 : bk.x0, ey0 = FINE || Q8 ? 0 : bk.y0;
     const int en0 = bk.n0;
     const int es0 = fs0, es1 = fs1;
 #pragma unroll
@@ -514,10 +547,12 @@
     int tide = tid;
     asm volatile("" : "+v"(tide));
     const int lanee = tide & 63;
-    const int rb = wid & 3;
+    int rb = wid & 3;
+    int p16q = 0;
+    if constexpr (Q8) cw4q_reader(wid, lanee, rb, p16q);
     const unsigned l5 = (unsigned)lanee & 31u, gsel = (0x0FF0F00Fu >> l5) & 1u;
     const int gidx = __builtin_popcount((gsel ? 0x0FF0F00Fu : 0xF00F0FF0u) & ((1u << l5) - 1u));
-    const int p16 = LWG_W4_RDMAP && !SM ? (wid >> 2) * 4 + 2 * (lanee >> 5) + (gsel ? 0 : 1) + 8 * (gidx >> 3) : (wid >> 2) * 8 + (lanee >> 3);
+    const int p16 = Q8 ? p16q : LWG_W4_RDMAP && !SM ? (wid >> 2) * 4 + 2 * (lanee >> 5) + (gsel ? 0 : 1) + 8 * (gidx >> 3) : (wid >> 2) * 8 + (lanee >> 3);
     const int n4 = SMS ? (lanee & 3) * 4 : LWG_W4_RDMAP && !SM ? (gidx & 7) * 4 : (lanee & 7) * 4;
     const int cbase = SMS ? (en0 >> 6) * 32 + ((en0 >> 4) & 1) * 16 : en0 >> 1;
     floatx4 mu, rs;
@@ -533,13 +568,21 @@
         ry = __builtin_amdgcn_make_buffer_rsrc(y + (size_t)eb * H * W * a.YC, 0, (int)img_bytes, 0x00020000);
         re = __builtin_amdgcn_make_buffer_rsrc(const_cast<float*>(esrc) + (size_t)eb * H * W * a.YC, 0, (int)img_bytes, 0x00020000);
     };
-    if constexpr (!FINE) eframe();
+    if constexpr (!FINE && !Q8) eframe();
     const int chan = EPI == LWG_EPI_SPADE ? cbase + n4 : a.ycoff + en0 + n4;
     bool more = false;
     int nblk = blk;
 #pragma unroll
     for (int ph = 0; ph < 2; ++ph) {
         if (ph == 1) __syncthreads();
+        if constexpr (Q8) {
+            const int u = ph ? es1 : es0;
+            int ub;
+            cw4q_corner(g, max(u, 0), ub, ex0, ey0);
+            eb = __builtin_amdgcn_readfirstlane(ub);
+            if (u < 0) ex0 = W, ey0 = H;
+            eframe();
+        }
         if constexpr (FINE) {
             const int u = ph ? es1 : es0;
             int ub;
@@ -564,7 +607,8 @@
 #pragma unroll
         for (int hp = 0; hp < NVP; ++hp) {
             const int p = ph * 16 + (SMS ? lanee >> 2 : SM ? 8 * hp + (lanee >> 3) : p16);
-            const int ox = ex0 + 4 * (FINE ? (p & 7) % (CW4F_SX / 4) : (p & 7)) + rb, oyb = ey0 + 4 * (FINE ? (p >> 3) % (CW4F_SY / 4) : (p >> 3));
+            const int ox = ex0 + 4 * (Q8 ? (p & 7) % (CW4Q_SX / 4) : FINE ? (p & 7) % (CW4F_SX / 4) : (p & 7)) + rb;
+            const int oyb = ey0 + 4 * (Q8 ? (p >> 3) % (CW4Q_SY / 4) : FINE ? (p >> 3) % (CW4F_SY / 4) : (p >> 3));
 #pragma unroll
             for (int i = 0; i < 4; ++i)
                 vo[hp][i] = cw4_out_voff(ox, oyb + i, H, W, a.YC, chan);
@@ -580,7 +624,7 @@
             W4TS(8);
             if constexpr (!SPLIT) {
             nblk = blk + (int)gridDim.x;
-            if constexpr (FINE) more = nblk < nhe;
+            if constexpr (FINE || Q8) more = nblk < nhe;
             else if constexpr (LIST) more = lst ? nblk < nhe : cw_has_block(o, nblk);
             else more = cw_has_block(o, nblk);
             setup(more ? nblk : blk);
@@ -663,7 +707,7 @@
     if constexpr (LIST) {
         typedef unsigned int w4_u4 __attribute__((ext_vector_type(4)));
         constexpr int NQD = EPI == LWG_EPI_SPADE ? 8 : 16;
-        constexpr int NPASS = (FINE ? CW4F_SX * CW4F_SY : 512) * NQD / W4_THREADS, NI = NPASS < 4 ? NPASS : 4;
+        constexpr int NPASS = (Q8 ? CW4Q_SX * CW4Q_SY : FINE ? CW4F_SX * CW4F_SY : 512) * NQD / W4_THREADS, NI = NPASS < 4 ? NPASS : 4;
         const int ncb = N / NBV;
         const int nend = nhe + min(max(__builtin_amdgcn_readfirstlane(sk.counts[1]), 0), nall - nht) * ncb;
         const unsigned img_bytes = (unsigned)(H * W) * (unsigned)a.YC * 4u;
@@ -672,10 +716,13 @@
         for (int id = cw_list_first_light((int)blockIdx.x, (int)gridDim.x, nhe); id < nend; id += (int)gridDim.x) {
             int slot, cb;
             cw_list_entry(id - nhe, ncb, slot, cb);
-            const int t = min(max(__builtin_amdgcn_readfirstlane(sk.light[slot]), 0), (FINE ? CW4F_NS : 1) * g.tiles - 1);
+            const int t = min(max(__builtin_amdgcn_readfirstlane(sk.light[slot]), 0), (Q8 ? CW4Q_NS : FINE ? CW4F_NS : 1) * g.tiles - 1);
             const int en0 = cw_n0(cb, NBV);
             int eb, ex0, ey0;
-            if constexpr (FINE) {
+            if constexpr (Q8) {
+                cw4q_corner(g, t, eb, ex0, ey0);
+                eb = __builtin_amdgcn_readfirstlane(eb);
+            } else if constexpr (FINE) {
                 cw4f_corner(g, t, eb, ex0, ey0);
                 eb = __builtin_amdgcn_readfirstlane(eb);
             } else {
@@ -698,6 +745,7 @@
                     for (int i = 0; i < NI; ++i) {
                         cw4_light_elem(tid, it + i, W4_THREADS, NQD, px, py, q4);
                         if constexpr (FINE) cw4f_light_pixel(px, py);
+                        if constexpr (Q8) cw4q_light_pixel(px, py);
                         vo[i] = cw4_out_voff(ex0 + px, ey0 + py, H, W, a.YC, cbase + 4 * q4);
                         const unsigned vc = cw4_out_voff(ex0 + px, ey0 + py, H, W, N, en0 + 4 * q4);
                         gam[i] = cw_buf_load(rc, cw4_out_group(vc, 0, true), 0u);
@@ -721,6 +769,7 @@
                     for (int i = 0; i < NI; ++i) {
                         cw4_light_elem(tid, it + i, W4_THREADS, NQD, px, py, q4);
                         if constexpr (FINE) cw4f_light_pixel(px, py);
+                        if constexpr (Q8) cw4q_light_pixel(px, py);
                         vo[i] = cw4_out_voff(ex0 + px, ey0 + py, H, W, a.YC, a.ycoff + en0 + 4 * q4);
                         o[i] = cw_buf_load(rc, vo[i], 0u);
                     }
@@ -752,6 +801,17 @@
 template <int EPI>
 __global__ __launch_bounds__(W4_THREADS, 1) void lwg_conv_winograd4_fine_plain_kernel(const LwgConvArgs a, const LwgConvLists sk) {
     if (__builtin_amdgcn_readfirstlane(sk.counts[0]) < cw4f_in_image_total(a.B, a.H, a.W)) return;
+    w4_body<EPI, false, false, false>(a, LwgConvLists{});
+}
+
+template <int EPI>
+__global__ __launch_bounds__(W4_THREADS, 1) void lwg_conv_winograd4_q8_kernel(const LwgConvArgs a, const LwgConvLists sk) {
+    if (__builtin_amdgcn_readfirstlane(sk.counts[0]) >= cw4q_in_image_total(a.B, a.H, a.W)) return;
+    w4_body<EPI, false, false, true, false, false, true>(a, sk);
+}
+template <int EPI>
+__global__ __launch_bounds__(W4_THREADS, 1) void lwg_conv_winograd4_q8_plain_kernel(const LwgConvArgs a, const LwgConvLists sk) {
+    if (__builtin_amdgcn_readfirstlane(sk.counts[0]) < cw4q_in_image_total(a.B, a.H, a.W)) return;
     w4_body<EPI, false, false, false>(a, LwgConvLists{});
 }
 
@@ -949,3 +1009,17 @@
     return a.epi == LWG_EPI_SPADE ? cw_launch_lists<lwg_conv_winograd4_fine_plain_kernel<LWG_EPI_SPADE>>(grid, W4_THREADS, ldsp, stream, a, *pl)
                                   : cw_launch_lists<lwg_conv_winograd4_fine_plain_kernel<LWG_EPI_NONE>>(grid, W4_THREADS, ldsp, stream, a, *pl);
 }
+
+extern "C" int lwg_conv2d_winograd4_q8_f32(const LwgConvArgs* pa, const LwgConvLists* pl, lwg_stream_t stream_) {
+    if (!lwg_wino4_list_ok(pa) || !pl || !pl->heavy || !pl->light || !pl->counts || !pl->cal) return (int)hipErrorInvalidValue;
+    if (!lwg_conv2d_winograd4_list_applies(pa)) return lwg_conv2d_winograd4_f32(pa, stream_);
+    hipStream_t stream = reinterpret_cast<hipStream_t>(stream_);
+    const LwgConvArgs& a = *pa;
+    const size_t lds = (size_t)(W4Q_BIAS_OFF + 64) * 4, ldsp = (size_t)(W4_BIAS_OFF + 64) * 4;
+    const dim3 grid = cw_persistent_grid(cw_total_blocks(a.B, a.H, a.W, a.N, 4 * W4_PBX, 4 * W4_PBY, W4_NB), lwg_device_cus());
+    const int e = a.epi == LWG_EPI_SPADE ? cw_launch_lists<lwg_conv_winograd4_q8_kernel<LWG_EPI_SPADE>>(grid, W4_THREADS, lds, stream, a, *pl)
+                                         : cw_launch_lists<lwg_conv_winograd4_q8_kernel<LWG_EPI_NONE>>(grid, W4_THREADS, lds, stream, a, *pl);
+    if (e != 0) return e;
+    return a.epi == LWG_EPI_SPADE ? cw_launch_lists<lwg_conv_winograd4_q8_plain_kernel<LWG_EPI_SPADE>>(grid, W4_THREADS, ldsp, stream, a, *pl)
+                                  : cw_launch_lists<lwg_conv_winograd4_q8_plain_kernel<LWG_EPI_NONE>>(grid, W4_THREADS, ldsp, stream, a, *pl);
+}
diff --git a/ipercore_amd/csrc/lwg_conv_wino.h b/ipercore_amd/csrc/lwg_conv_wino.h
--- a/ipercore_amd/csrc/lwg_conv_wino.h
+++ b/ipercore_amd/csrc/lwg_conv_wino.h
@@ -133,6 +133,65 @@
     py = p / CW4F_SX, px = p - py * CW4F_SX;
 }
 
+#define CW4Q_SX 8
+#define CW4Q_SY 8
+#define CW4Q_NSX (32 / CW4Q_SX)
+#define CW4Q_NS (CW4Q_NSX * (16 / CW4Q_SY))
+#define CW4Q_HW (CW4Q_SX + 2)
+#define CW4Q_HH (CW4Q_SY + 2)
+#define CW4Q_NEL (CW4Q_HW * CW4Q_HH * 2)
+#define CW4Q_ROUNDS ((CW4Q_NEL + 63) / 64)
+CW_FN int cw4q_slot_of_patch(int pty, int ptx) { return (pty / (CW4Q_SY / 4)) * CW4Q_NSX + ptx / (CW4Q_SX / 4); }
+CW_FN void cw4q_patch_in_slot(int pty, int ptx, int& ly, int& lx) { ly = pty % (CW4Q_SY / 4), lx = ptx % (CW4Q_SX / 4); }
+CW_FN void cw4q_corner(const CwGrid& g, int u, int& b, int& x0, int& y0) {
+    const int t = u / CW4Q_NS, s = u - t * CW4Q_NS;
+    b = cw_image(g, t);
+    cw_corner(g, t - b * g.bx * g.by, 32, 16, x0, y0);
+    x0 += (s % CW4Q_NSX) * CW4Q_SX, y0 += (s / CW4Q_NSX) * CW4Q_SY;
+}
+CW_FN bool cw4q_in_image(int x0, int y0, int H, int W) { return x0 < W && y0 < H; }
+CW_FN int cw4q_in_image_total(int B, int H, int W) { return B * ((W + CW4Q_SX - 1) / CW4Q_SX) * ((H + CW4Q_SY - 1) / CW4Q_SY); }
+CW_FN int cw4q_groups(int nh) { return (nh + CW4Q_NS - 1) / CW4Q_NS; }
+CW_FN int cw4q_slot_index(int grp, int k, int nh) { return grp * CW4Q_NS + k < nh ? grp * CW4Q_NS + k : -1; }
+CW_FN unsigned cw4q_reached(int x, int y, int x0, int y0, int d) {
+    unsigned m = 0;
+    for (int s = 0; s < CW4Q_NS; ++s) {
+        const int sx = x0 + (s % CW4Q_NSX) * CW4Q_SX, sy = y0 + (s / CW4Q_NSX) * CW4Q_SY;
+        m |= (x >= sx - d && x < sx + CW4Q_SX + d && y >= sy - d && y < sy + CW4Q_SY + d ? 1u : 0u) << s;
+    }
+    return m;
+}
+CW_FN unsigned cw4q_marks16(unsigned m8) { return ((m8 | (m8 >> 1)) & 1u) | (((m8 >> 2) | (m8 >> 3)) & 1u) << 1 | (((m8 >> 4) | (m8 >> 5)) & 1u) << 2 | (((m8 >> 6) | (m8 >> 7)) & 1u) << 3; }
+CW_FN void cw4q_halo_elem(int i, int& slot, int& j) { slot = (i >> 6) & 7, j = (i >> 9) * 64 + (i & 63); }
+CW_FN void cw4q_halo_place(int j, int& hy, int& hx, int& hq) {
+    const int pix = j >> 1;
+    hq = j & 1, hy = pix / CW4Q_HW, hx = pix - hy * CW4Q_HW;
+}
+CW_FN unsigned cw4q_halo_voff(bool present, int j, int x0, int y0, int H, int W, int C) {
+    int hy, hx, hq;
+    cw4q_halo_place(j, hy, hx, hq);
+    const int gy = y0 - 1 + hy, gx = x0 - 1 + hx;
+    return present && j < CW4Q_NEL && gy >= 0 && gy < H && gx >= 0 && gx < W ? (unsigned)((gy * W + gx) * C + 4 * hq) * 4u : CW_OOB;
+}
+#define CW4Q_RS 28
+#define CW4Q_PLANE (4 * CW4Q_HH * CW4Q_RS + 24 + 4)
+CW_FN int cw4q_lds_slot(int s) { const int r = s >> 1; return r * (CW4Q_HH * CW4Q_RS) + 4 * r * (r - 1) + (s & 1) * 16; }
+CW_FN int cw4q_lds_patch(int pty, int ptx) {
+    int ly, lx;
+    cw4q_patch_in_slot(pty, ptx, ly, lx);
+    return cw4q_lds_slot(cw4q_slot_of_patch(pty, ptx)) + 4 * ly * CW4Q_RS + 4 * lx;
+}
+CW_FN void cw4q_reader(int wid, int lane, int& rb, int& p16) {
+    const unsigned l5 = (unsigned)lane & 31u, gsel = (0x0FF0F00Fu >> l5) & 1u;
+    const int gidx = __builtin_popcount((gsel ? 0x0FF0F00Fu : 0xF00F0FF0u) & ((1u << l5) - 1u));
+    rb = 2 * (wid & 1) + (lane >> 5);
+    p16 = 2 * (wid >> 1) + (gsel ? 0 : 1) + 8 * (gidx >> 3);
+}
+CW_FN void cw4q_light_pixel(int& px, int& py) {
+    const int p = py * 32 + px;
+    py = p / CW4Q_SX, px = p - py * CW4Q_SX;
+}
+
 #define CW4_SPLIT_MIN_STAGES 8
 #define CW4_SPLIT_MAX_SLICES 8
 struct Cw4Split { int slices, sps; };
diff --git a/ipercore_amd/csrc/spade_skip.hip b/ipercore_amd/csrc/spade_skip.hip
--- a/ipercore_amd/csrc/spade_skip.hip
+++ b/ipercore_amd/csrc/spade_skip.hip
@@ -95,9 +95,8 @@
         }
     for (; i < i1; ++i) f(i, marks[i]);
 }
-__global__ __launch_bounds__(1024) void lwg_spade_skip_scan2_kernel(SkScanJob j0, SkScanJob j1) {
+__device__ __forceinline__ void sk_scan_job(const SkScanJob j) {
     __shared__ int ph[1024], pl[1024];
-    const SkScanJob j = blockIdx.x == 0 ? j0 : j1;
     const int tid = threadIdx.x, n = j.n, per = ((n + 1023) / 1024 + 3) & ~3;
     const int i0 = tid * per < n ? tid * per : n, i1 = i0 + per < n ? i0 + per : n;
     const bool vec = (reinterpret_cast<size_t>(j.marks) & 15) == 0;
@@ -119,6 +118,48 @@
     if (tid == 1023) {
         j.counts[0] = ph[1023];
         j.counts[1] = pl[1023];
+    }
+}
+__global__ __launch_bounds__(1024) void lwg_spade_skip_scan2_kernel(SkScanJob j0, SkScanJob j1) {
+    const SkScanJob j = blockIdx.x == 0 ? j0 : j1;
+    sk_scan_job(j);
+}
+__global__ __launch_bounds__(1024) void lwg_spade_skip_scan3_kernel(SkScanJob j0, SkScanJob j1, SkScanJob j2) {
+    const SkScanJob j = blockIdx.x == 0 ? j0 : blockIdx.x == 1 ? j1 : j2;
+    sk_scan_job(j);
+}
+
+__global__ __launch_bounds__(256) void lwg_spade_skip_mark_q8_kernel(const float2* __restrict__ T, int B, int ns, int h, int w, int d, int* __restrict__ marks,
+                                                                     int* __restrict__ fmarks, int* __restrict__ qmarks) {
+    const CwGrid g = cw_grid(B, h, w, CW_NB, SK_EX, SK_EY, CW_NB);
+    const int t = blockIdx.x, b = cw_image(g, t);
+    int x0, y0;
+    cw_corner(g, t - b * g.bx * g.by, SK_EX, SK_EY, x0, y0);
+    const CwWindow win = cw_block_window(x0, y0, SK_EX, SK_EY, d, h, w);
+    const int ww = win.x1 - win.x0, n = ww * (win.y1 - win.y0);
+    unsigned mine = 0;
+    for (int s = 0; s < ns; ++s) {
+        const float2* Ts = T + ((size_t)b * ns + s) * h * w;
+        for (int i = threadIdx.x; i < n; i += 256) {
+            const int yy = i / ww, y = win.y0 + yy, x = win.x0 + (i - yy * ww);
+            float wt[4];
+            int tx0, ty0;
+            lwb_taps_of(Ts[(size_t)y * w + x], w, h, wt, tx0, ty0);
+            if (lwb_tap_in_image(tx0, ty0, w, h)) mine |= (1u << CW4Q_NS) | cw4q_reached(x, y, x0, y0, d);
+        }
+    }
+    unsigned all = 0;
+    for (int s = 0; s <= CW4Q_NS; ++s) all |= __syncthreads_or((int)((mine >> s) & 1u)) ? 1u << s : 0u;
+    const int s = threadIdx.x;
+    if (s < CW4Q_NS) {
+        const bool in = cw4q_in_image(x0 + (s % CW4Q_NSX) * CW4Q_SX, y0 + (s / CW4Q_NSX) * CW4Q_SY, h, w);
+        qmarks[CW4Q_NS * t + s] = in ? (int)((all >> s) & 1u) : 2;
+    } else if (s < CW4Q_NS + CW4F_NS) {
+        const int f = s - CW4Q_NS;
+        const bool in = cw4f_in_image(x0 + (f % CW4F_NSX) * CW4F_SX, y0 + (f / CW4F_NSX) * CW4F_SY, h, w);
+        fmarks[CW4F_NS * t + f] = in ? (int)((cw4q_marks16(all) >> f) & 1u) : 2;
+    } else if (s == CW4Q_NS + CW4F_NS) {
+        marks[t] = (int)((all >> CW4Q_NS) & 1u);
     }
 }
 
@@ -145,3 +186,19 @@
     hipLaunchKernelGGL(lwg_spade_skip_scan_kernel, dim3(1), dim3(1024), 0, stream, marks, (int)tiles, heavy, light, counts);
     return (int)hipGetLastError();
 }
+
+extern "C" int lwg_spade_skip_q8_lists_f32(const float* T, int B, int ns, int h, int w, int d, int* marks, int* heavy, int* light, int* counts,
+                                           int* fmarks, int* fheavy, int* flight, int* fcounts, int* qmarks, int* qheavy, int* qlight, int* qcounts,
+                                           lwg_stream_t stream_) {
+    if (!T || !marks || !heavy || !light || !counts || !fmarks || !fheavy || !flight || !fcounts || !qmarks || !qheavy || !qlight || !qcounts || B <= 0 ||
+        ns <= 0 || h <= 0 || w <= 0 || d < 0 || d > 64)
+        return (int)hipErrorInvalidValue;
+    const long long tiles = cw_total_blocks(B, h, w, CW_NB, SK_EX, SK_EY, CW_NB);
+    if (tiles * CW4Q_NS >= (1ll << 30) || (long long)h * w >= (1ll << 30)) return (int)hipErrorInvalidValue;
+    hipStream_t stream = reinterpret_cast<hipStream_t>(stream_);
+    hipLaunchKernelGGL(lwg_spade_skip_mark_q8_kernel, dim3((unsigned)tiles), dim3(256), 0, stream, reinterpret_cast<const float2*>(T), B, ns, h, w, d, marks, fmarks,
+                       qmarks);
+    hipLaunchKernelGGL(lwg_spade_skip_scan3_kernel, dim3(3), dim3(1024), 0, stream, SkScanJob{marks, (int)tiles, heavy, light, counts},
+                       SkScanJob{fmarks, (int)tiles * CW4F_NS, fheavy, flight, fcounts}, SkScanJob{qmarks, (int)tiles * CW4Q_NS, qheavy, qlight, qcounts});
+    return (int)hipGetLastError();
+}
diff --git a/ipercore_amd/ops.py b/ipercore_amd/ops.py
--- a/ipercore_amd/ops.py
+++ b/ipercore_amd/ops.py
@@ -346,26 +346,53 @@
 
 SPADE_SKIP_FINE = True
 
+SPADE_SKIP_Q8 = True
+SPADE_SKIP_Q8_MIN = 640
+SPADE_SKIP_Q8_MAX_HW = 64 * 64
+
 _LISTS_APPLY = {}
 
 
 class SkipLists(tuple):
     fine = None
+    fine8 = None
 
 
 def spade_skip_fine_apply(x0):
     return SPADE_SKIP_FINE
+
+
+def spade_skip_q8_apply(x0, ncb):
+    B, H, W = x0.shape[:3]
+    return SPADE_SKIP_FINE and SPADE_SKIP_Q8 and H * W <= SPADE_SKIP_Q8_MAX_HW and B * ((H + 15) // 16) * ((W + 31) // 32) * ncb >= SPADE_SKIP_Q8_MIN
+
+
+def spade_skip_q8_lists_apply(tiles, h, w):
+    return SPADE_SKIP_FINE and SPADE_SKIP_Q8 and CONV_PRECISION == "winograd" and h * w <= SPADE_SKIP_Q8_MAX_HW and tiles * 8 >= SPADE_SKIP_Q8_MIN
 
 
 def spade_skip_lists(flow, d):
     B, ns, h, w, two = flow.shape
     assert two == 2 and flow.dtype == torch.float32
     tiles = B * ((h + 15) // 16) * ((w + 31) // 32)
-    buf = torch.empty(15 * tiles + 4, device=flow.device, dtype=torch.int32)
+    q8 = spade_skip_q8_lists_apply(tiles, h, w)
+    buf = torch.empty((39 if q8 else 15) * tiles + 8, device=flow.device, dtype=torch.int32)
+    if q8:
+        qb, buf = buf[:24 * tiles], buf[24 * tiles:]
+        qmarks, qheavy, qlight = qb[:8 * tiles], qb[8 * tiles:16 * tiles], qb[16 * tiles:]
     fmarks, fheavy, flight = buf[:4 * tiles], buf[4 * tiles:8 * tiles], buf[8 * tiles:12 * tiles]
     bb = buf[12 * tiles:]
-    marks, heavy, light, counts, fcounts = bb[:tiles], bb[tiles:2 * tiles], bb[2 * tiles:3 * tiles], bb[3 * tiles:3 * tiles + 2], bb[3 * tiles + 2:]
+    marks, heavy, light, counts, fcounts = bb[:tiles], bb[tiles:2 * tiles], bb[2 * tiles:3 * tiles], bb[3 * tiles:3 * tiles + 2], bb[3 * tiles + 2:3 * tiles + 4]
     i32 = torch.int32
+    if q8:
+        qcounts = bb[3 * tiles + 4:3 * tiles + 6]
+        _lib.check(_lib.lib().lwg_spade_skip_q8_lists_f32(_ptr(flow), B, ns, h, w, int(d), _ptr(marks, i32), _ptr(heavy, i32), _ptr(light, i32),
+                                                          _ptr(counts, i32), _ptr(fmarks, i32), _ptr(fheavy, i32), _ptr(flight, i32), _ptr(fcounts, i32),
+                                                          _ptr(qmarks, i32), _ptr(qheavy, i32), _ptr(qlight, i32), _ptr(qcounts, i32), _stream()),
+                   "lwg_spade_skip_q8_lists_f32")
+        out = SkipLists((heavy, light, counts))
+        out.fine, out.fine8 = (fheavy, flight, fcounts), (qheavy, qlight, qcounts)
+        return out
     _lib.check(_lib.lib().lwg_spade_skip_fine_lists_f32(_ptr(flow), B, ns, h, w, int(d), _ptr(marks, i32), _ptr(heavy, i32), _ptr(light, i32),
                                                         _ptr(counts, i32), _ptr(fmarks, i32), _ptr(fheavy, i32), _ptr(flight, i32), _ptr(fcounts, i32),
                                                         _stream()), "lwg_spade_skip_fine_lists_f32")
@@ -512,9 +539,14 @@
                 if fine:
                     sl, cal = lists
                     fine = sl.fine is not None and spade_skip_fine_apply(x0)
-                    lists = tuple(sl.fine if fine else sl) + (cal,)
+                    q8 = fine and sl.fine8 is not None and spade_skip_q8_apply(x0, spec.N // 64)
+                    lists = tuple(sl.fine8 if q8 else sl.fine if fine else sl) + (cal,)
+                else:
+                    q8 = False
                 ld = _lib.LwgConvLists(_ptr(lists[0], i32), _ptr(lists[1], i32), _ptr(lists[2], i32), _ptr(lists[3]))
-                if fine:
+                if q8:
+                    _lib.check(_lib.lib().lwg_conv2d_winograd4_q8_f32(a, ctypes.byref(ld), _stream()), "lwg_conv2d_winograd4_q8_f32")
+                elif fine:
                     _lib.check(_lib.lib().lwg_conv2d_winograd4_fine_f32(a, ctypes.byref(ld), _stream()), "lwg_conv2d_winograd4_fine_f32")
                 else:
                     _lib.check(_lib.lib().lwg_conv2d_winograd4_list_f32(a, ctypes.byref(ld), _stream()), "lwg_conv2d_winograd4_list_f32")
```

Result: faster. 1377 frames/s, median of 6 (+1.1%).
